# GitHubOfAndrew/TeAMOFlow

Measured on AMD Instinct MI355X. Metric: train_interactions_per_sec, higher is better.
Workload: dtype f32

## Files before the change

### include/tmf.h

```cpp
#ifndef TMF_H
#define TMF_H

#include <stddef.h>
#include <stdint.h>

#ifdef __cplusplus
extern "C" {
#endif

#define TMF_VERSION 203

#define TMF_OK 0
#define TMF_E_INVALID (-1)
#define TMF_E_LAUNCH (-2)
#define TMF_E_UNSUPPORTED (-3)

#define TMF_EPI_ADAM 0
#define TMF_EPI_GRAD 1

int tmf_version(void);
const char* tmf_last_error(void);

int tmf_padded_ld(int n_components);

int tmf_padded_ld_bf16(int n_components);

typedef struct tmf_adam {
    float alpha, one_minus_b1, one_minus_b2, eps;
} tmf_adam;
tmf_adam tmf_adam_fresh(float lr);

typedef struct tmf_segments {
    const int64_t* rowptr;
    const int32_t* seg_row;
    const int32_t* seg_chunk;
    const int32_t* seg_slab;
    int64_t nseg;
    int32_t chunk;
    int32_t row_mod;
} tmf_segments;

size_t tmf_csr_build_workspace_bytes(int64_t nnz);
int tmf_csr_build(const int64_t* indices, const float* values, int64_t nnz, int32_t n_users, int32_t n_items,
                  int64_t* rowptr_u, int32_t* col_u, float* val_u, int32_t* user_of, void* workspace,
                  size_t workspace_bytes, void* stream);
size_t tmf_stable_order_workspace_bytes(int64_t n);
int tmf_csc_perm(const int32_t* col_u, int64_t nnz, int32_t n_items, int64_t* rowptr_i, int64_t* perm,
                 void* workspace, size_t workspace_bytes, void* stream);
int tmf_stable_order_i32(const int32_t* keys, int64_t n, int64_t n_rows, int64_t* perm, int32_t* sorted_keys,
                         int64_t* rowptr, void* workspace, size_t workspace_bytes, void* stream);

size_t tmf_sort_samples_workspace_bytes(int32_t n_users, int32_t n_samples);
int tmf_sort_samples(const int32_t* R, int32_t n_users, int32_t n_samples, int32_t n_items, int32_t* R_sorted,
                     void* workspace, size_t workspace_bytes, void* stream);
int tmf_slice_offsets(const int32_t* ids, const int64_t* rowptr, int64_t stride, int32_t n_rows, int32_t n_items,
                      int32_t n_slices, int32_t* off, void* stream);
size_t tmf_wmrb_entry_lists_workspace_bytes(int64_t nnz, int32_t n_users, int32_t n_samples);
int tmf_wmrb_entry_lists(const int32_t* user_of, const int32_t* col_u, const float* val_u, int64_t nnz,
                         const int32_t* R_sorted, int32_t n_users, int32_t n_samples, int32_t n_items, int32_t user_chunks,
                         int32_t* ent_row, int32_t* ent_id, int64_t* rowptr_e, void* workspace, size_t workspace_bytes,
                         void* stream);

int tmf_mse_pass_f32(const tmf_segments* seg, const int32_t* other, const float* val,
                     const float* X_old, const float* Y_old, float* X_out, float* slab,
                     float* loss_part, int n_components, int epi, tmf_adam adam, void* stream);

int tmf_wsum_pass_f32(const tmf_segments* seg, const int32_t* ent_row, const int32_t* ent_w,
                      const float* wbuf, const float* T, const float* X_old, float* X_out,
                      float* slab, int n_components, int epi, tmf_adam adam, void* stream);

int tmf_wsum_rows4_rows_per_group(int n_components, int bf16);
size_t tmf_wsum_rows4_workspace_bytes(int32_t n_rows, int32_t n_blocks, int32_t rows_per_launch);
int tmf_wsum_rows4_f32(const int64_t* rowptr, int32_t n_rows, int32_t n_blocks, const int32_t* ent_row, const int32_t* ent_w,
                       const float* wbuf, const float* T, const float* X_old, float* X_out, int n_components, int epi,
                       tmf_adam adam, int32_t rows_per_launch, void* workspace, size_t workspace_bytes, void* stream);

size_t tmf_wsum_rows5_workspace_bytes(int32_t n_vrows, int32_t n_blocks, int32_t rows_per_launch);
int tmf_wsum_rows5_f32(const int64_t* rowptr, int32_t n_rows, int32_t n_blocks, const int32_t* ent_row, const int32_t* ent_w,
                       const float* wbuf, const float* T, const float* X_old, float* X_out, float* slab, const int32_t* vr_item,
                       const int32_t* vr_part, const int32_t* vr_nparts, const int32_t* vr_slot, int32_t n_vrows, int n_components,
                       int epi, tmf_adam adam, int32_t rows_per_launch, void* workspace, size_t workspace_bytes, void* stream);

int tmf_combine_rows_f32(const int32_t* long_rows, const int64_t* slab_beg, int64_t n_long,
                         const float* slab, const float* X_old, float* X_out, int n_components,
                         int epi, tmf_adam adam, void* stream);

int tmf_wmrb_user_pass_f32(const int64_t* rowptr, const int32_t* col, const float* val,
                           const int32_t* R, int32_t n_users, int32_t S, float c,
                           const float* U_old, const float* V_old, float* U_out, float* delta,
                           float* D, float* loss_part, float* pos_part,
                           int n_components, int epi, tmf_adam adam, void* stream);
int tmf_wmrb_user_pass_fits(int32_t n_samples, int n_components);

typedef struct tmf_slice_lists {
    const int32_t* R_sorted;
    const int32_t* slice_off;
    const int64_t* rowptr;
    const int32_t* col;
    const int32_t* pos_off;
    int32_t n_users, n_samples, n_slices;
    int32_t slice_begin, slice_count, item_base;
    int32_t flags;
    int32_t n_items;
} tmf_slice_lists;
#define TMF_SLICE_XCD_MAJOR 1
#define TMF_SLICE_N_ITEMS_STATED 2
int tmf_wmrb_scores3_f32(const tmf_slice_lists* lists, const void* U, const void* V, float* sp, float* p,
                         int n_components, void* stream);
int tmf_wmrb_scores3_bf16(const tmf_slice_lists* lists, const void* U, const void* V, float* sp, float* p,
                          int n_components, void* stream);
int tmf_wmrb_scores5_users_per_workgroup(void);
int tmf_wmrb_scores5_supported(int n_components, int bf16, int64_t n_items);
size_t tmf_wmrb_scores5_workspace_bytes(int64_t n_wg, int32_t n_windows, int wgs_per_launch);
int tmf_wmrb_scores5_f32(const int32_t* ids, const int32_t* outs, const int64_t* wg_ptr, int64_t n_wg, int64_t n_users,
                         int64_t n_items, const void* U, const void* V, float* sp, float* p, int n_components,
                         int wgs_per_launch, const int32_t* wstart, int32_t n_windows, int lag, void* workspace,
                         size_t workspace_bytes, void* stream);
int tmf_wmrb_scores5_bf16(const int32_t* ids, const int32_t* outs, const int64_t* wg_ptr, int64_t n_wg, int64_t n_users,
                          int64_t n_items, const void* U, const void* V, float* sp, float* p, int n_components,
                          int wgs_per_launch, const int32_t* wstart, int32_t n_windows, int lag, void* workspace,
                          size_t workspace_bytes, void* stream);
int tmf_wmrb_scores6_users_per_group(void);
int tmf_wmrb_scores6_supported(int n_components, int bf16, int64_t n_items);
int tmf_wmrb_scores6_f32(const int32_t* ids, const int32_t* outs, const int64_t* chunk_ptr, int64_t n_groups, int32_t n_slices,
                         int64_t n_users, int64_t n_items, const void* U, const void* V, float* sp, float* p, int n_components,
                         void* stream);
int tmf_wmrb_scores6_bf16(const int32_t* ids, const int32_t* outs, const int64_t* chunk_ptr, int64_t n_groups, int32_t n_slices,
                          int64_t n_users, int64_t n_items, const void* U, const void* V, float* sp, float* p, int n_components,
                          void* stream);
int tmf_wmrb_hinge2(const int64_t* rowptr, const float* val, const float* p, const float* sp, int32_t n_users,
                    int32_t n_samples, float c, float* delta, float* D, float* loss_part, void* stream);
int tmf_wmrb_hinge2_ordered(const int64_t* rowptr, const float* val, const float* p, const float* sp, int32_t n_users,
                            int32_t n_samples, float c, float* delta, float* D, float* loss_part, const int32_t* user_order,
                            void* stream);
int tmf_wmrb_gradu3_f32(const tmf_slice_lists* lists, const float* D, const float* delta, const void* V, float* part,
                        int per_slice_launches, int n_components, void* stream);
int tmf_wmrb_gradu3_bf16(const tmf_slice_lists* lists, const float* D, const float* delta, const void* V, float* part,
                         int per_slice_launches, int n_components, void* stream);
int tmf_wmrb_gradu4_supported(int n_components, int bf16);
size_t tmf_wmrb_gradu4_workspace_bytes(int32_t n_users, int32_t n_slices, int32_t users_per_launch);
int tmf_wmrb_gradu4_f32(const tmf_slice_lists* lists, const float* D, const float* delta, const void* V, const void* U_old,
                        void* U_out, int n_components, int epi, tmf_adam adam, int32_t users_per_launch, void* workspace,
                        size_t workspace_bytes, void* stream);
int tmf_wmrb_gradu4_bf16(const tmf_slice_lists* lists, const float* D, const float* delta, const void* V, const void* U_old,
                         void* U_out, int n_components, int epi, tmf_adam adam, int32_t users_per_launch, void* workspace,
                         size_t workspace_bytes, void* stream);
int tmf_wmrb_finish_f32(const float* part, int32_t n_slices, int32_t n_users, const void* U_old, void* U_out,
                        int n_components, int epi, tmf_adam adam, void* stream);
int tmf_wmrb_finish_bf16(const float* part, int32_t n_slices, int32_t n_users, const void* U_old, void* U_out,
                         int n_components, int epi, tmf_adam adam, void* stream);

int tmf_adam_fresh_rows_f32(float* W, const float* G, int64_t n_rows, int n_components,
                            tmf_adam adam, void* stream);

tmf_adam tmf_adam_step(float lr, int step);
int tmf_adam_state_rows_f32(float* W, const float* G, float* M, float* V, int64_t n_rows, int n_components,
                            tmf_adam adam, void* stream);

int tmf_sum_f32(const float* x, int64_t n, double* out, void* stream);

int tmf_gather_rows_cols_f32(const float* X, const int64_t* idx, float* out, int64_t rows,
                             int64_t cols, int64_t k, void* stream);

int tmf_predict_gemm_f32(const float* A, const float* B, float* C, int64_t m, int64_t n, int r,
                         int64_t lda, int64_t ldb, int64_t ldc, void* stream);

size_t tmf_topk_workspace_bytes(int64_t rows, int64_t cols, int k);
int tmf_topk_stable_f32(const float* X, int64_t rows, int64_t cols, int64_t ldx, int k,
                        int clamp_negatives, int32_t* out_idx, float* out_val, void* workspace,
                        size_t workspace_bytes, void* stream);

int tmf_mse_pass_bf16(const tmf_segments* seg, const int32_t* other, const float* val,
                      const void* X_old, const void* Y_old, void* X_out, float* slab,
                      float* loss_part, int n_components, int epi, tmf_adam adam, void* stream);
int tmf_wsum_pass_bf16(const tmf_segments* seg, const int32_t* ent_row, const int32_t* ent_w,
                       const float* wbuf, const void* T, const void* X_old, void* X_out,
                       float* slab, int n_components, int epi, tmf_adam adam, void* stream);
int tmf_wsum_rows4_bf16(const int64_t* rowptr, int32_t n_rows, int32_t n_blocks, const int32_t* ent_row, const int32_t* ent_w,
                        const float* wbuf, const void* T, const void* X_old, void* X_out, int n_components, int epi,
                        tmf_adam adam, int32_t rows_per_launch, void* workspace, size_t workspace_bytes, void* stream);
int tmf_wsum_rows5_bf16(const int64_t* rowptr, int32_t n_rows, int32_t n_blocks, const int32_t* ent_row, const int32_t* ent_w,
                        const float* wbuf, const void* T, const void* X_old, void* X_out, float* slab, const int32_t* vr_item,
                        const int32_t* vr_part, const int32_t* vr_nparts, const int32_t* vr_slot, int32_t n_vrows, int n_components,
                        int epi, tmf_adam adam, int32_t rows_per_launch, void* workspace, size_t workspace_bytes, void* stream);
int tmf_combine_rows_bf16(const int32_t* long_rows, const int64_t* slab_beg, int64_t n_long,
                          const float* slab, const void* X_old, void* X_out, int n_components,
                          int epi, tmf_adam adam, void* stream);
int tmf_wmrb_user_pass_bf16(const int64_t* rowptr, const int32_t* col, const float* val,
                            const int32_t* R, int32_t n_users, int32_t S, float c,
                            const void* U_old, const void* V_old, void* U_out, float* delta,
                            float* D, float* loss_part, float* pos_part,
                            int n_components, int epi, tmf_adam adam, void* stream);
int tmf_adam_fresh_rows_bf16(void* W, const float* G, int64_t n_rows, int n_components,
                             tmf_adam adam, void* stream);

int tmf_predict_topk_f32(const float* A, const float* B, int64_t m, int64_t n, int r, int64_t lda,
                         int64_t ldb, int k, int clamp_negatives, int32_t* out_idx, float* out_val,
                         void* stream);

int tmf_predict_topk_bf16(const void* A, const void* B, int64_t m, int64_t n, int r, int64_t lda,
                          int64_t ldb, int k, int clamp_negatives, int32_t* out_idx, float* out_val,
                          void* stream);

int tmf_predict_topk_split_supported(int r, int k);
size_t tmf_predict_topk_split_workspace_bytes(int64_t n, int r);
int tmf_predict_topk_split_f32(const float* A, const float* B, int64_t m, int64_t n, int r, int64_t lda,
                               int64_t ldb, int k, int clamp_negatives, int32_t* out_idx, float* out_val,
                               void* workspace, size_t workspace_bytes, void* stream);
int tmf_predict_topk_half2_supported(int r, int k);
size_t tmf_predict_topk_half2_workspace_bytes(int64_t n, int r);
int tmf_predict_topk_half2_f32(const float* A, const float* B, int64_t m, int64_t n, int r, int64_t lda,
                               int64_t ldb, int k, int clamp_negatives, int32_t* out_idx, float* out_val,
                               void* workspace, size_t workspace_bytes, void* stream);

typedef struct tmf_exclusion {
    const int64_t* rowptr;
    const int32_t* cols;
    int64_t item_base;
} tmf_exclusion;

int tmf_predict_topk_exclude_f32(const float* A, const float* B, int64_t m, int64_t n, int r, int64_t lda,
                                 int64_t ldb, int k, int clamp_negatives, const tmf_exclusion* exclude,
                                 int32_t* out_idx, float* out_val, void* stream);
int tmf_predict_topk_exclude_bf16(const void* A, const void* B, int64_t m, int64_t n, int r, int64_t lda,
                                  int64_t ldb, int k, int clamp_negatives, const tmf_exclusion* exclude,
                                  int32_t* out_idx, float* out_val, void* stream);
int tmf_predict_topk_split_exclude_f32(const float* A, const float* B, int64_t m, int64_t n, int r, int64_t lda,
                                       int64_t ldb, int k, int clamp_negatives, const tmf_exclusion* exclude,
                                       int32_t* out_idx, float* out_val, void* workspace, size_t workspace_bytes, void* stream);
int tmf_predict_topk_half2_exclude_f32(const float* A, const float* B, int64_t m, int64_t n, int r, int64_t lda,
                                       int64_t ldb, int k, int clamp_negatives, const tmf_exclusion* exclude,
                                       int32_t* out_idx, float* out_val, void* workspace, size_t workspace_bytes, void* stream);
int tmf_topk_stable_exclude_f32(float* X, int64_t rows, int64_t cols, int64_t ldx, int k, int clamp_negatives,
                                const tmf_exclusion* exclude, int32_t* out_idx, float* out_val, void* workspace,
                                size_t workspace_bytes, void* stream);

#define TMF_RANK_ROW_PAIRS 16
typedef struct tmf_rank_rows {
    const int32_t* user;
    const int64_t* begin;
    const int32_t* count;
    int64_t n_rows;
} tmf_rank_rows;

int tmf_pair_scores_f32(const float* A, const float* B, int r, int64_t lda, int64_t ldb, const int32_t* pair_user,
                        const int32_t* pair_item, int64_t n_pairs, float* out, void* stream);
int tmf_pair_scores_split(const float* A, const float* B, int r, int64_t lda, int64_t ldb, const int32_t* pair_user,
                          const int32_t* pair_item, int64_t n_pairs, float* out, void* stream);

int tmf_item_ranks_f32_supported(int r);
int tmf_item_ranks_split_supported(int r);
size_t tmf_item_ranks_split_workspace_bytes(int64_t n, int r);
int tmf_item_ranks_f32(const float* A, const float* B, int64_t n, int r, int64_t lda, int64_t ldb, const tmf_rank_rows* rows,
                       const int32_t* pos_item, const float* pos_score, const tmf_exclusion* exclude, int32_t* out_rank,
                       void* stream);
int tmf_item_ranks_split(const float* A, const float* B, int64_t n, int r, int64_t lda, int64_t ldb, const tmf_rank_rows* rows,
                         const int32_t* pos_item, const float* pos_score, const tmf_exclusion* exclude, int32_t* out_rank,
                         void* workspace, size_t workspace_bytes, void* stream);

int tmf_rank_count_rows_f32(float* X, int64_t rows, int64_t cols, int64_t ldx, int64_t user_base, const tmf_rank_rows* vrows,
                            const int32_t* pos_item, const tmf_exclusion* exclude, int32_t* out_rank, void* stream);

int tmf_dcg_idcg_f32(const int64_t* rowptr, const int32_t* cols, const float* gain, int64_t m, int64_t n_items, const int32_t* top,
                     int64_t ldt, int k, const float* den, const int64_t* n_zero, float* dcg, float* idcg, void* stream);

#ifdef __cplusplus
}
#endif
#endif
```

### teamoflow_amd/_engine.py

```python
import ctypes
import os

import torch

from . import _lib

DEFAULT_CHUNK = 1024
PART_BUDGET = int(os.environ.get('TMF_PART_BUDGET', 8 << 30))


def _excl_cumsum(x):
    out = torch.zeros(x.numel() + 1, dtype=torch.int64, device=x.device)
    torch.cumsum(x, 0, out=out[1:])
    return out


def take_interactions(indices, values, keep, user_offset=0, item_offset=0):
    u = indices[:, 0][keep] - user_offset
    j = indices[:, 1][keep] - item_offset
    return torch.stack([u, j], dim=1), values[keep]


def stable_order(keys, n_rows):
    n = keys.numel()
    if keys.is_cuda and n < 2 ** 31 and n_rows < 2 ** 31:
        lib = _lib.get()
        k32 = keys.to(torch.int32).contiguous()
        perm = torch.empty(n, dtype=torch.int64, device=keys.device)
        rowptr = torch.empty(n_rows + 1, dtype=torch.int64, device=keys.device)
        ws = torch.empty(lib.tmf_stable_order_workspace_bytes(n), dtype=torch.uint8, device=keys.device)
        _lib.check(lib.tmf_stable_order_i32(_lib.ptr(k32), n, n_rows, _lib.ptr(perm), None, _lib.ptr(rowptr), _lib.ptr(ws),
                                            ws.numel(), _lib.stream_ptr()), lib)
        return perm, rowptr
    perm = torch.sort(keys, stable=True)[1]
    return perm, _excl_cumsum(torch.bincount(keys.to(torch.int64), minlength=n_rows))


class SegmentTable:

    def __init__(self, rowptr, chunk=DEFAULT_CHUNK, out_row=None, n_out=None, row_mod=0):
        dev = rowptr.device
        rows = rowptr.numel() - 1
        lens = rowptr[1:] - rowptr[:-1]
        nch = torch.clamp((lens + (chunk - 1)) // chunk, min=1)
        nseg = int(nch.sum())
        seg_first = _excl_cumsum(nch)
        ar = torch.arange(rows, device=dev)
        seg_row = torch.repeat_interleave(ar, nch, output_size=nseg)
        seg_chunk = torch.arange(nseg, device=dev) - seg_first[seg_row]
        if out_row is None:
            multi = nch > 1
            slab_beg = _excl_cumsum(nch * multi)
            seg_slab = torch.where(multi[seg_row], slab_beg[seg_row] + seg_chunk, torch.full_like(seg_chunk, -1))
            long_rows = torch.nonzero(multi).flatten()
            self.n_slab = int(slab_beg[-1])
            self.long_slab_beg = torch.cat([slab_beg[long_rows], slab_beg[-1:]]).contiguous()
        else:
            seg_out = out_row[seg_row]
            order = torch.sort(seg_out, stable=True)[1]
            seg_slab = torch.empty(nseg, dtype=torch.int64, device=dev)
            seg_slab[order] = torch.arange(nseg, device=dev)
            long_rows = torch.arange(n_out, device=dev)
            self.n_slab = nseg
            self.long_slab_beg = _excl_cumsum(torch.bincount(seg_out, minlength=n_out))
        self.rows, self.chunk, self.nseg, self.row_mod = rows, int(chunk), nseg, int(row_mod)
        self.rowptr = rowptr.contiguous()
        self.seg_row = seg_row.to(torch.int32)
        self.seg_chunk = seg_chunk.to(torch.int32)
        self.seg_slab = seg_slab.to(torch.int32)
        self.long_rows = long_rows.to(torch.int32)
        self.n_long = int(long_rows.numel())
        self._c = None

    @classmethod
    def of_rows(cls, rowptr, rows, out_row, n_out, chunk=DEFAULT_CHUNK):
        self = cls.__new__(cls)
        dev = rowptr.device
        lens = rowptr[rows + 1] - rowptr[rows]
        nch = torch.clamp((lens + (chunk - 1)) // chunk, min=1)
        nseg = int(nch.sum())
        seg_first = _excl_cumsum(nch)
        sel = torch.repeat_interleave(torch.arange(rows.numel(), device=dev), nch, output_size=nseg)
        seg_chunk = torch.arange(nseg, device=dev) - seg_first[sel]
        seg_out = out_row[sel]
        order = torch.sort(seg_out, stable=True)[1]
        seg_slab = torch.empty(nseg, dtype=torch.int64, device=dev)
        seg_slab[order] = torch.arange(nseg, device=dev)
        self.n_slab = nseg
        self.long_slab_beg = _excl_cumsum(torch.bincount(seg_out, minlength=n_out))
        self.rows, self.chunk, self.nseg, self.row_mod = int(rows.numel()), int(chunk), nseg, 0
        self.rowptr = rowptr
        self.seg_row = rows[sel].to(torch.int32)
        self.seg_chunk = seg_chunk.to(torch.int32)
        self.seg_slab = seg_slab.to(torch.int32)
        self.long_rows = torch.arange(n_out, device=dev, dtype=torch.int32)
        self.n_long = int(n_out)
        self._c = None
        return self

    def cstruct(self):
        if self._c is None:
            self._c = _lib.Segments(self.rowptr.data_ptr(), self.seg_row.data_ptr(), self.seg_chunk.data_ptr(),
                                    self.seg_slab.data_ptr(), self.nseg, self.chunk, self.row_mod)
        return ctypes.byref(self._c)


class InteractionPlan:

    def __init__(self, indices, values, n_users, n_items, chunk=DEFAULT_CHUNK, user_chunks=1, csc=True):
        dev = indices.device
        u = indices[:, 0].contiguous()
        j = indices[:, 1].contiguous()
        nnz = u.numel()
        if nnz:
            lo_u, hi_u, lo_j, hi_j = int(u.min()), int(u.max()), int(j.min()), int(j.max())
            if lo_u < 0 or hi_u >= n_users or lo_j < 0 or hi_j >= n_items:
                raise IndexError(f'interaction indices outside dense_shape: users [{lo_u}, {hi_u}] of {n_users}, '
                                 f'items [{lo_j}, {hi_j}] of {n_items}')
        values = values.to(torch.float32).contiguous()
        self.nnz, self.n_users, self.n_items = nnz, n_users, n_items
        if indices.is_cuda and nnz < 2 ** 31:
            lib = _lib.get()
            idx64 = indices.to(torch.int64).contiguous()
            self.rowptr_u = torch.empty(n_users + 1, dtype=torch.int64, device=dev)
            self.col_u = torch.empty(nnz, dtype=torch.int32, device=dev)
            self.val_u = torch.empty(nnz, dtype=torch.float32, device=dev)
            self.user_of = torch.empty(nnz, dtype=torch.int32, device=dev)
            ws = torch.empty(lib.tmf_csr_build_workspace_bytes(nnz), dtype=torch.uint8, device=dev)
            _lib.check(lib.tmf_csr_build(_lib.ptr(idx64), _lib.ptr(values), nnz, n_users, n_items, _lib.ptr(self.rowptr_u),
                                         _lib.ptr(self.col_u), _lib.ptr(self.val_u), _lib.ptr(self.user_of), _lib.ptr(ws),
                                         ws.numel(), _lib.stream_ptr()), lib)
            del ws, idx64
        else:
            key = u.to(torch.int64) * n_items + j.to(torch.int64)
            if nnz > 1 and not bool((key[1:] >= key[:-1]).all()):
                perm = torch.sort(key, stable=True)[1]
                u, j, values = u[perm], j[perm], values[perm]
            self.rowptr_u = _excl_cumsum(torch.bincount(u, minlength=n_users))
            self.col_u = j.to(torch.int32)
            self.val_u = values.contiguous()
            self.user_of = u.to(torch.int32)
        self.seg_u = SegmentTable(self.rowptr_u, chunk)
        C = max(1, int(user_chunks))
        self.user_chunks = C
        self.seg_i = self.rowptr_i = self.row_i = self.val_i = None
        if csc:
            if C > 1:
                upc = -(-n_users // C)
                key = (self.user_of.to(torch.int64) // upc) * n_items + self.col_u.to(torch.int64)
            else:
                key = self.col_u
            perm_c, self.rowptr_i = stable_order(key, C * n_items)
            self.row_i = self.user_of[perm_c].contiguous()
            self.val_i = self.val_u[perm_c].contiguous()
            if C > 1:
                out_row = torch.arange(C * n_items, device=dev) % n_items
                self.seg_i = SegmentTable(self.rowptr_i, chunk, out_row=out_row, n_out=n_items, row_mod=n_items)
            else:
                self.seg_i = SegmentTable(self.rowptr_i, chunk)
        self.n_pos = int((self.val_u > 0).sum())

    @property
    def user_ids(self):
        return self.user_of.to(torch.int64)


def _slab_budget():
    env = os.environ.get('TMF_SLAB_BUDGET')
    if env:
        return int(env)
    total = torch.cuda.get_device_properties(torch.cuda.current_device()).total_memory if torch.cuda.is_available() else 32 << 30
    return int(min(64 << 30, total // 4))




def default_user_chunks(n_users, ld, target_bytes=3 << 20, n_items=None):
    env = os.environ.get('TMF_USER_CHUNKS')
    if env:
        return max(1, int(env))
    c = -(-n_users * ld * 4 // target_bytes)
    if n_items:
        c = min(c, max(1, _slab_budget() // (n_items * ld * 4)))
    return int(min(max(c, 1), 256)) if c > 1 else 1


def mse_user_chunks():
    env = os.environ.get('TMF_USER_CHUNKS')
    return max(1, int(env)) if env else 1


def default_item_slices(n_items, ld, n_samples=None, target_bytes=4 << 20, elem_size=4):
    env = os.environ.get('TMF_ITEM_SLICES')
    if env:
        return max(1, int(env))
    if n_items * ld * elem_size <= 2 * target_bytes:
        return 1
    return int(min(-(-n_items * ld * elem_size // target_bytes), 64))


def slices_xcd_major(n_slices):
    env = os.environ.get('TMF_SLICE_XCD')
    if env in ('0', '1'):
        return env == '1'
    return XCD_MAJOR_DEFAULT and n_slices >= 8


XCD_MAJOR_DEFAULT = False
SLICED_MIN_HINGE_TERMS = 1 << 16
SLICED_MIN_SCORES = 1 << 21


def choose_wmrb_user_pass(n_users, n_items, ld, n_samples, n_positives, n_components, elem_size=4):
    ns = default_item_slices(n_items, ld, elem_size=elem_size)
    if ns > 1 or not fused_user_pass_fits(n_samples, n_components) or os.environ.get('TMF_FORCE_SLICED') == '1':
        return ns, True
    if os.environ.get('TMF_ITEM_SLICES') or os.environ.get('TMF_FORCE_FUSED') == '1':
        return ns, False
    if (n_positives / max(n_users, 1)) * n_samples >= SLICED_MIN_HINGE_TERMS and n_users * n_samples >= SLICED_MIN_SCORES:
        groups = -(-n_users // 16)
        return int(max(min(max(round(1400 / groups), 1), 8), -(-n_items * ld * elem_size // (4 << 20)))), True
    return 1, False


def rows4_wanted(n_components, dtype=torch.float32, plan=None, R=None, n_users=None, n_items=None):
    env = os.environ.get('TMF_ROWS4')
    if env == '0':
        return False
    if not _lib.load_library().tmf_wsum_rows4_rows_per_group(int(n_components), int(dtype is torch.bfloat16)):
        return False
    if env == '1':
        return True
    if plan is not None:
        n_users = plan.n_users if n_users is None else n_users
        n_items = plan.n_items if n_items is None else n_items
    if not n_users or not n_items:
        return False
    ld = _lib.padded_ld(n_components, dtype)
    row_bytes = ld * (2 if dtype is torch.bfloat16 else 4)
    blocks_wanted = -(-int(n_users) * row_bytes // ROWS5_BLOCK_BYTES)
    blocks_slab_allows = max(1, _slab_budget() // (int(n_items) * ld * 4))
    return blocks_wanted > 2 * blocks_slab_allows


ROWS5_TARGET_OVER_MEDIAN = 1.15
ROWS5_BLOCK_BYTES = 4 << 20


def rows5_user_chunks(n_users, n_components, dtype=torch.float32):
    env = os.environ.get('TMF_USER_CHUNKS')
    if env:
        return max(1, int(env))
    row_bytes = _lib.padded_ld(n_components, dtype) * (2 if dtype is torch.bfloat16 else 4)
    return int(min(max(1, -(-int(n_users) * row_bytes // ROWS5_BLOCK_BYTES)), 256))


class VirtualRows:

    def __init__(self, rowptr_e, n_blocks, n_rows, target=None):
        dev = rowptr_e.device
        lens = (rowptr_e[1:] - rowptr_e[:-1]).view(n_blocks, n_rows).sum(0)
        mean = float(lens.to(torch.float64).mean()) if n_rows else 0.0
        median = float(lens.to(torch.float64).median()) if n_rows else 0.0
        env = os.environ.get('TMF_ROWS5_TARGET')
        self.target = int(env) if env else (int(target) if target else max(1, int(max(ROWS5_TARGET_OVER_MEDIAN * median, mean)) + 1))
        parts = torch.clamp((lens + (self.target - 1)) // self.target, min=1)
        first = _excl_cumsum(parts)
        nv = int(first[-1])
        item = torch.repeat_interleave(torch.arange(n_rows, device=dev), parts, output_size=nv)
        part = torch.arange(nv, device=dev) - first[item]
        multi = parts > 1
        slab_beg = _excl_cumsum(parts * multi)
        slot = torch.where(multi[item], slab_beg[item] + part, torch.full_like(part, -1))
        i32 = torch.int32
        self.n_vrows, self.n_slab = nv, int(slab_beg[-1])
        self.item = torch.cat([item, torch.tensor([n_rows], device=dev)]).to(i32).contiguous()
        self.part = torch.cat([part, torch.zeros(1, dtype=part.dtype, device=dev)]).to(i32).contiguous()
        self.nparts = torch.cat([parts[item], torch.ones(1, dtype=parts.dtype, device=dev)]).to(i32).contiguous()
        self.slot = slot.to(i32).contiguous()
        long_rows = torch.nonzero(multi).flatten()
        self.long_rows = long_rows.to(i32).contiguous()
        self.long_slab_beg = torch.cat([slab_beg[long_rows], slab_beg[-1:]]).contiguous()
        self.n_long = int(long_rows.numel())
        self.max_parts = int(parts.max()) if n_rows else 0


def fused_user_pass_fits(n_samples, n_components):
    return bool(_lib.load_library().tmf_wmrb_user_pass_fits(int(n_samples), min(int(n_components), 1024)))


HINGE_CHUNK = 255


def hinge_user_order(rowptr_u):
    if os.environ.get('TMF_HINGE_ORDER', '1') == '0':
        return None
    deg = rowptr_u[1:] - rowptr_u[:-1]
    passes = (deg + (HINGE_CHUNK - 1)) // HINGE_CHUNK
    if passes.numel() == 0 or int(passes.max()) <= 1:
        return None
    return torch.argsort(passes, descending=True, stable=True).to(torch.int32)


class WmrbPlan:

    def __init__(self, plan, R, chunk=DEFAULT_CHUNK, user_chunks=1, item_slices=1, n_components=128, sliced=None, item_lists=True,
                 xcd_major=None, rows4=False):
        dev = R.device
        m, S = R.shape
        nnz, n = plan.nnz, plan.n_items
        self.S, self.n_slices = S, max(1, int(item_slices))
        self.xcd_major = slices_xcd_major(self.n_slices) if xcd_major is None else bool(xcd_major)
        self.sliced = bool(sliced) if sliced is not None else (self.n_slices > 1 or not fused_user_pass_fits(S, n_components))
        C = self.user_chunks = max(1, int(user_chunks))
        E = nnz + m * S
        if E >= 2 ** 31:
            raise ValueError(f'interactions + n_users * n_samples = {E} >= 2^31 on one GPU: split the users over more GPUs')
        self.R_model = R
        native = R.is_cuda
        lib = _lib.get() if native else None
        i32 = ctypes.c_int32
        self.slice_off = self.pos_off = None
        if self.sliced:
            ns = self.n_slices
            if native:
                Rs = torch.empty_like(R)
                ws = torch.empty(lib.tmf_sort_samples_workspace_bytes(m, S), dtype=torch.uint8, device=dev)
                _lib.check(lib.tmf_sort_samples(_lib.ptr(R), i32(m), i32(S), i32(n), _lib.ptr(Rs), _lib.ptr(ws), ws.numel(),
                                                _lib.stream_ptr()), lib)
                del ws
                self.slice_off = torch.empty(m, ns + 1, dtype=torch.int32, device=dev)
                self.pos_off = torch.empty(m, ns + 1, dtype=torch.int32, device=dev)
                _lib.check(lib.tmf_slice_offsets(_lib.ptr(Rs), None, S, i32(m), i32(n), i32(ns), _lib.ptr(self.slice_off),
                                                 _lib.stream_ptr()), lib)
                _lib.check(lib.tmf_slice_offsets(_lib.ptr(plan.col_u), _lib.ptr(plan.rowptr_u), 0, i32(m), i32(n), i32(ns),
                                                 _lib.ptr(self.pos_off), _lib.stream_ptr()), lib)
            else:
                Rs = torch.sort(R.to(torch.int64), dim=1, stable=True)[0].to(torch.int32).contiguous()
                width = -(-n // ns)
                bnd = torch.arange(ns + 1, dtype=torch.int64) * width
                self.slice_off = torch.searchsorted(Rs.to(torch.int64), bnd[None, :].expand(m, -1).contiguous()).to(torch.int32)
                self.slice_off[:, -1] = S
                key = plan.user_of.to(torch.int64) * (ns * width + 1) + plan.col_u.to(torch.int64)
                q = torch.arange(m, dtype=torch.int64)[:, None] * (ns * width + 1) + bnd[None, :]
                self.pos_off = (torch.searchsorted(key, q.reshape(-1)).reshape(m, ns + 1) - plan.rowptr_u[:-1, None]).to(torch.int32)
                self.pos_off[:, -1] = (plan.rowptr_u[1:] - plan.rowptr_u[:-1]).to(torch.int32)
            R = Rs
        self.R = R.contiguous()
        self.ent_row = torch.empty(E, dtype=torch.int32, device=dev)
        rowptr = torch.empty(C * n + 2, dtype=torch.int64, device=dev)
        if native:
            ent_id = torch.empty(E, dtype=torch.int32, device=dev)
            ws = torch.empty(lib.tmf_wmrb_entry_lists_workspace_bytes(nnz, m, S), dtype=torch.uint8, device=dev)
            _lib.check(lib.tmf_wmrb_entry_lists(_lib.ptr(plan.user_of), _lib.ptr(plan.col_u), _lib.ptr(plan.val_u), nnz,
                                                _lib.ptr(self.R), i32(m), i32(S), i32(n), i32(C), _lib.ptr(self.ent_row),
                                                _lib.ptr(ent_id), _lib.ptr(rowptr), _lib.ptr(ws), ws.numel(),
                                                _lib.stream_ptr()), lib)
            del ws
        else:
            upc = max(1, -(-m // C))
            ku = plan.user_of.to(torch.int64)
            kp = torch.where(plan.val_u > 0, (ku // upc) * n + plan.col_u.to(torch.int64), torch.full_like(ku, C * n))
            ks = (torch.arange(m, dtype=torch.int64) // upc).repeat_interleave(S) * n + self.R.reshape(-1).to(torch.int64)
            keys = torch.cat([kp, ks])
            ent_id = torch.sort(keys, stable=True)[1]
            rowptr = _excl_cumsum(torch.bincount(keys, minlength=C * n + 1))
            owner = torch.cat([ku, torch.arange(m, dtype=torch.int64).repeat_interleave(S)])
            self.ent_row = owner[ent_id].to(torch.int32)
            ent_id = ent_id.to(torch.int32)
        self.rowptr_e = rowptr[:C * n + 1].contiguous()
        self.ent_w = ent_id
        self.rows4 = bool(rows4)
        self.vrows = VirtualRows(self.rowptr_e, C, n) if self.rows4 and os.environ.get('TMF_ROWS5', '1') != '0' else None
        if not item_lists or self.rows4:
            self.seg_e = None
        elif C > 1:
            out_row = torch.arange(C * n, device=dev) % n
            self.seg_e = SegmentTable(self.rowptr_e, chunk, out_row=out_row, n_out=n)
        else:
            self.seg_e = SegmentTable(self.rowptr_e, chunk)
        self.wbuf = torch.zeros(E, dtype=torch.float32, device=dev)
        self.delta = self.wbuf[:nnz]
        self.hinge_order = hinge_user_order(plan.rowptr_u)
        self.D = self.wbuf[nnz:].view(m, S)
        self._lists = None
        self.s5 = None

    def lists(self, plan):
        if self._lists is None:
            m, S = self.R.shape
            self._lists = _lib.SliceLists(self.R.data_ptr(), self.slice_off.data_ptr(), plan.rowptr_u.data_ptr(),
                                          plan.col_u.data_ptr(), self.pos_off.data_ptr(), m, S, self.n_slices, 0, 0, 0,
                                          (_lib.SLICE_XCD_MAJOR if self.xcd_major else 0) | _lib.SLICE_N_ITEMS_STATED, int(plan.n_items))
        return ctypes.byref(self._lists)

    def window_lists(self, plan, slice_begin, slice_count, item_base):
        m, S = self.R.shape
        return _lib.SliceLists(self.R.data_ptr(), self.slice_off.data_ptr(), plan.rowptr_u.data_ptr(), plan.col_u.data_ptr(),
                               self.pos_off.data_ptr(), m, S, self.n_slices, slice_begin, slice_count, item_base,
                               _lib.SLICE_N_ITEMS_STATED, int(plan.n_items))

    def D_in_model_order(self):
        if not self.sliced:
            return self.D
        perm = torch.sort(self.R_model.to(torch.int64), dim=1, stable=True)[1]
        out = torch.empty_like(self.D)
        out.scatter_(1, perm, self.D)
        return out


def row_stationary_wanted(n_users, n_items, n_samples, nnz, n_components, dtype=torch.float32, sliced=True):
    env = os.environ.get('TMF_ROW_STATIONARY')
    if env == '0' or not sliced:
        return False
    if not _lib.load_library().tmf_wmrb_gradu4_supported(int(n_components), int(dtype is torch.bfloat16)):
        return False
    return env == '1' or short_visits(n_users, n_items, n_samples, nnz, n_components, dtype)


def wmrb_plan_for(plan, R, n_components, dtype=torch.float32, n_items=None):
    m = plan.n_users
    n = plan.n_items if n_items is None else n_items
    bf16 = dtype is torch.bfloat16
    ld_store = _lib.padded_ld(n_components, dtype)
    ns, sliced = choose_wmrb_user_pass(m, n, ld_store, int(R.shape[1]), plan.n_pos, n_components, elem_size=2 if bf16 else 4)
    rs = row_stationary_wanted(m, n, int(R.shape[1]), plan.nnz, n_components, dtype, sliced)
    if rs and not os.environ.get('TMF_ITEM_SLICES'):
        ns = int(max(1, -(-n * ld_store * (2 if bf16 else 4) // GRADU4_SLICE_BYTES)))
    rows4 = rows4_wanted(n_components, dtype, plan, R)
    C = rows5_user_chunks(m, n_components, dtype) if rows4 else default_user_chunks(m, _lib.padded_ld(n_components), n_items=plan.n_items)
    return WmrbPlan(plan, R, user_chunks=C, item_slices=ns, n_components=n_components, sliced=sliced, rows4=rows4)


def scores6_wanted(plan, wplan, n_components, dtype=torch.float32):
    env = os.environ.get('TMF_SCORES6')
    if env == '0' or wplan is None or not wplan.sliced or not plan.col_u.is_cuda or os.environ.get('TMF_SCORES5') == '1':
        return False
    m, S = wplan.R.shape
    if m * S >= 2 ** 31 or plan.nnz >= 2 ** 31:
        return False
    if not _lib.load_library().tmf_wmrb_scores6_supported(int(n_components), int(dtype is torch.bfloat16), int(plan.n_items)):
        return False
    if env == '1':
        return True
    return SCORES6_DEFAULT and short_visits(m, plan.n_items, S, plan.nnz, n_components, dtype)


def short_visits(n_users, n_items, n_samples, nnz, n_components, dtype=torch.float32):
    row_bytes = _lib.padded_ld(n_components, dtype) * (2 if dtype is torch.bfloat16 else 4)
    table = n_items * row_bytes
    if table < 8 * VISIT_SLICE_BYTES:
        return False
    return (n_samples + nnz / max(n_users, 1)) * VISIT_SLICE_BYTES / table <= SCORES6_MAX_VISIT


SCORES6_SLICE_BYTES = 6 << 20
VISIT_SLICE_BYTES = 4 << 20
GRADU4_SLICE_BYTES = 3200000
SCORES6_MAX_VISIT = 24
SCORES6_DEFAULT = True


class Scores6Plan:

    PAD = -2 ** 31

    def __init__(self, plan, wplan, n_components, dtype=torch.float32, slice_bytes=None):
        lib = _lib.load_library()
        dev = plan.col_u.device
        self.key = (int(n_components), dtype)
        UG = int(lib.tmf_wmrb_scores6_users_per_group())
        m, S = wplan.R.shape
        nnz, n = plan.nnz, plan.n_items
        E = nnz + m * S
        self.n_groups = ng = -(-m // UG)
        row_bytes = _lib.padded_ld(n_components, dtype) * (2 if dtype is torch.bfloat16 else 4)
        slice_bytes = int(os.environ.get('TMF_S6_SLICE_BYTES', slice_bytes or SCORES6_SLICE_BYTES))
        ns = int(min(max(1, -(-n * row_bytes // slice_bytes)), max(1, (2 ** 31 - 1) // max(ng, 1))))
        width = -(-n // ns)
        self.n_slices = ns = -(-n // width)
        i32 = torch.int32
        uo = plan.user_of
        rows = torch.arange(m, device=dev, dtype=i32)
        keys = torch.empty(E, dtype=i32, device=dev)
        keys[:nnz] = (plan.col_u // width) * ng + uo // UG
        keys[nnz:].view(m, S).copy_((wplan.R // width) * ng + (rows // UG)[:, None])
        perm, rowptr = stable_order(keys, ns * ng)
        del keys
        packed = torch.empty(E, dtype=i32, device=dev)
        packed[:nnz] = ((uo % UG) << 24) | plan.col_u
        packed[nnz:].view(m, S).copy_(((rows % UG) << 24)[:, None] | wplan.R)
        ids_sorted = packed[perm]
        del packed
        outs = torch.empty(E, dtype=i32, device=dev)
        outs[:nnz] = -1 - torch.arange(nnz, device=dev, dtype=i32)
        outs[nnz:] = torch.arange(m * S, device=dev, dtype=i32)
        outs_sorted = outs[perm]
        del outs, perm
        cnt = rowptr[1:] - rowptr[:-1]
        ptr8 = _excl_cumsum((cnt + 7) // 8 * 8)
        E8 = int(ptr8[-1])
        self.ids = torch.empty(E8 + 8, dtype=i32, device=dev)
        self.outs = torch.full((E8 + 8,), self.PAD, dtype=i32, device=dev)
        self.ids[E8:] = 0
        step = 1 << 27
        for q0 in range(0, E8, step):
            q = torch.arange(q0, min(q0 + step, E8), device=dev, dtype=torch.int64)
            ch = torch.searchsorted(ptr8, q, right=True) - 1
            r = q - ptr8[ch]
            c = cnt[ch]
            src = rowptr[ch] + torch.minimum(r, c - 1)
            self.ids[q0:q0 + q.numel()] = ids_sorted[src]
            self.outs[q0:q0 + q.numel()] = torch.where(r < c, outs_sorted[src], torch.full_like(src, self.PAD).to(i32))
            del q, ch, r, c, src
        self.chunk_ptr = ptr8
        self.n_entries, self.n_padded = E, E8


def scores5_wanted(plan, wplan, n_components, dtype=torch.float32):
    if os.environ.get('TMF_SCORES5') != '1' or wplan is None or not wplan.sliced or not plan.col_u.is_cuda:
        return False
    m, S = wplan.R.shape
    if m * S >= 2 ** 31 or plan.nnz >= 2 ** 31:
        return False
    return bool(_lib.load_library().tmf_wmrb_scores5_supported(int(n_components), int(dtype is torch.bfloat16), int(plan.n_items)))


class Scores5Plan:

    PAD = -2 ** 31

    def __init__(self, plan, wplan, n_components, dtype=torch.float32, slice_bytes=None):
        lib = _lib.get()
        dev = plan.col_u.device
        self.key = (int(n_components), dtype)
        UB = int(lib.tmf_wmrb_scores5_users_per_workgroup())
        m, S = wplan.R.shape
        nnz, n = plan.nnz, plan.n_items
        E = nnz + m * S
        self.n_wg = n_wg = -(-m // UB)
        row_bytes = _lib.padded_ld(n_components, dtype) * (2 if dtype is torch.bfloat16 else 4)
        slice_bytes = int(os.environ.get('TMF_S5_SLICE_BYTES', slice_bytes or (512 << 10)))
        ns = int(min(max(1, -(-n * row_bytes // slice_bytes)), 4096, max(1, (2 ** 31 - 1) // max(n_wg, 1))))
        width = -(-n // ns)
        self.n_slices = ns
        i32 = torch.int32
        uo = plan.user_of
        rows = torch.arange(m, device=dev, dtype=i32)
        keys = torch.empty(E, dtype=i32, device=dev)
        keys[:nnz] = (uo // UB) * ns + plan.col_u // width
        keys[nnz:].view(m, S).copy_(((rows // UB) * ns)[:, None] + wplan.R // width)
        perm, rowptr = stable_order(keys, n_wg * ns)
        del keys
        packed = torch.empty(E, dtype=i32, device=dev)
        packed[:nnz] = ((uo % UB) << 24) | plan.col_u
        packed[nnz:].view(m, S).copy_(((rows % UB) << 24)[:, None] | wplan.R)
        ids_sorted = packed[perm]
        del packed
        outs = torch.empty(E, dtype=i32, device=dev)
        outs[:nnz] = -1 - torch.arange(nnz, device=dev, dtype=i32)
        outs[nnz:] = torch.arange(m * S, device=dev, dtype=i32)
        outs_sorted = outs[perm]
        del outs, perm
        wg_ptr = rowptr[::ns].contiguous()
        cnt = wg_ptr[1:] - wg_ptr[:-1]
        wg_ptr8 = _excl_cumsum((cnt + 7) // 8 * 8)
        E8 = int(wg_ptr8[-1])
        self.ids = torch.empty(E8 + 8, dtype=i32, device=dev)
        self.outs = torch.full((E8 + 8,), self.PAD, dtype=i32, device=dev)
        self.ids[E8:] = 0
        step = 1 << 27
        for q0 in range(0, E8, step):
            q = torch.arange(q0, min(q0 + step, E8), device=dev, dtype=torch.int64)
            wg = torch.searchsorted(wg_ptr8, q, right=True) - 1
            r = q - wg_ptr8[wg]
            c = cnt[wg]
            src = wg_ptr[wg] + torch.minimum(r, c - 1)
            self.ids[q0:q0 + q.numel()] = ids_sorted[src]
            self.outs[q0:q0 + q.numel()] = torch.where(r < c, outs_sorted[src], torch.full_like(src, self.PAD).to(i32))
            del q, wg, r, c, src
        self.wg_ptr = wg_ptr8
        self.n_entries, self.n_padded = E, E8
        every = max(1, int(os.environ.get('TMF_S5_PACE_EVERY', 32)), -(-ns // 4000))
        firsts = list(range(0, ns, every))
        off = rowptr[:n_wg * ns].view(n_wg, ns)[:, firsts] - wg_ptr[:-1, None]
        self.n_windows = nwin = len(firsts) + 1
        self.wstart = torch.zeros(n_wg, nwin + 1, dtype=i32, device=dev)
        self.wstart[:, 1:nwin] = ((off + 7) // 8).to(i32)
        self.wstart[:, nwin] = ((wg_ptr8[1:] - wg_ptr8[:-1]) // 8).to(i32)
        self.lag = int(os.environ.get('TMF_S5_LAG', 0))
        self.wgs_per_launch = int(os.environ.get('TMF_S5_WGS', 0))
        self.paced = os.environ.get('TMF_S5_PACE', '1') != '0' and ns > 1
        nb = lib.tmf_wmrb_scores5_workspace_bytes(n_wg, nwin, self.wgs_per_launch) if self.paced else 0
        self.sync = torch.zeros(max(nb // 4, 1), dtype=i32, device=dev)


class TrainState:

    def __init__(self, U0, V0, plan, n_components, wplan=None, dtype=torch.float32, V_tables=None, scratch=None):
        dev = plan.col_u.device
        self.r = int(n_components)
        if dtype not in (torch.float32, torch.bfloat16):
            raise ValueError('factor tables are stored as float32 or bfloat16')
        self.dtype = dtype
        self.sfx = '_bf16' if dtype is torch.bfloat16 else '_f32'
        self.ld = _lib.padded_ld(self.r, dtype)
        self.U = self._pad(U0, dev)
        self.U_nxt = torch.empty_like(self.U)
        if V_tables is None:
            self.V = self._pad(V0, dev)
            self.V_nxt = torch.empty_like(self.V)
        else:
            self.V, self.V_nxt = V_tables
        self.plan, self.wplan = plan, wplan
        need = dict(slab=max(plan.seg_u.n_slab, plan.seg_i.n_slab if plan.seg_i else 0,
                             wplan.seg_e.n_slab if wplan is not None and wplan.seg_e is not None else 0,
                             wplan.vrows.n_slab if wplan is not None and getattr(wplan, 'vrows', None) is not None else 0, 1) * self.ld,
                    loss_part=max(plan.seg_u.nseg, plan.n_users, 1))
        self.row_stationary = False
        if wplan is not None and wplan.sliced:
            m, S = wplan.R.shape
            self.row_stationary = row_stationary_wanted(m, plan.n_items, S, plan.nnz, self.r, dtype)
            self.users_per_launch = int(os.environ.get('TMF_G4_USERS', 32768))
            if self.row_stationary:
                nb = _lib.load_library().tmf_wmrb_gradu4_workspace_bytes(m, wplan.n_slices, self.users_per_launch)
                self.g4_sync = torch.zeros(max(nb // 4, 1), dtype=torch.int32, device=dev)
            ns = wplan.n_slices
            if ns * m * self.ld * 4 <= PART_BUDGET:
                self.part_layers, self.gradu_launches = ns, 0
            elif wplan.xcd_major:
                self.part_layers, self.gradu_launches = min(8, ns), 3
            else:
                self.part_layers, self.gradu_launches = 1, 1
            need.update(sp=m * S, pk=max(plan.nnz, 1), part=self.part_layers * max(m, 1) * self.ld)
            wplan.s6 = getattr(wplan, 's6', None)
            if scores6_wanted(plan, wplan, self.r, dtype):
                if wplan.s6 is None or wplan.s6.key != (self.r, dtype):
                    wplan.s6 = Scores6Plan(plan, wplan, self.r, dtype)
            else:
                wplan.s6 = None
            if wplan.seg_e is not None and scores5_wanted(plan, wplan, self.r, dtype):
                if getattr(wplan, 's5', None) is None or wplan.s5.key != (self.r, dtype):
                    wplan.s5 = Scores5Plan(plan, wplan, self.r, dtype)
            else:
                wplan.s5 = None
        if wplan is not None and wplan.rows4:
            L = _lib.load_library()
            per_group = L.tmf_wsum_rows4_rows_per_group(self.r, int(dtype is torch.bfloat16))
            if not per_group:
                raise ValueError('the row-stationary item pass needs rows of at least 16 lanes')
            cus = torch.cuda.get_device_properties(dev).multi_processor_count if torch.cuda.is_available() else 256
            self.rows4_per_launch = int(os.environ.get('TMF_ROWS4_PER_LAUNCH', 2 * cus * per_group))
            n_work = wplan.vrows.n_vrows if wplan.vrows is not None else plan.n_items
            nb = L.tmf_wsum_rows4_workspace_bytes(n_work, wplan.user_chunks, self.rows4_per_launch)
            self.rows4_sync = torch.zeros(max(nb // 4, 1), dtype=torch.int32, device=dev)
        self._need = need
        if scratch is None:
            self._bind({k: torch.zeros(v, dtype=torch.float32, device=dev) if k == 'loss_part'
                        else torch.empty(v, dtype=torch.float32, device=dev) for k, v in need.items()})
        else:
            scratch.setdefault('states', []).append(self)

    def _bind(self, bufs):
        need = self._need
        self.slab = bufs['slab'][:need['slab']].view(-1, self.ld)
        self.loss_part = bufs['loss_part'][:need['loss_part']]
        if 'sp' in need:
            m, S = self.wplan.R.shape
            self.sp = bufs['sp'][:need['sp']].view(m, S)
            self.pk = bufs['pk'][:need['pk']]
            self.part = bufs['part'][:need['part']].view(-1, self.ld)

    def _pad(self, W, dev):
        W = torch.as_tensor(W).detach().to(device=dev, dtype=torch.float32)
        out = torch.zeros(W.shape[0], self.ld, dtype=self.dtype, device=dev)
        out[:, :self.r] = W
        return out

    def swap(self):
        self.U, self.U_nxt = self.U_nxt, self.U
        self.V, self.V_nxt = self.V_nxt, self.V


def share_scratch(scratch, dev):
    states = scratch.get('states', [])
    sizes = {}
    for st in states:
        for k, v in st._need.items():
            sizes[k] = max(sizes.get(k, 0), v)
    bufs = {k: torch.zeros(v, dtype=torch.float32, device=dev) for k, v in sizes.items()}
    for st in states:
        st._bind(bufs)
    return bufs


class KernelTimer:

    def __init__(self):
        self.spans = {}

    def start(self, name):
        ev = torch.cuda.Event(enable_timing=True)
        ev.record()
        self.spans.setdefault(name, []).append([ev, None])

    def stop(self, name):
        ev = torch.cuda.Event(enable_timing=True)
        ev.record()
        self.spans[name][-1][1] = ev

    def mean_ms(self, name):
        v = [a.elapsed_time(b) for a, b in self.spans.get(name, []) if b is not None]
        return sum(v) / len(v) if v else float('nan')


def _row_pass_finish(lib, seg, slab, X_old, X_out, r, epi, adam, stream, sfx='_f32'):
    if seg.n_long:
        _lib.check(getattr(lib, 'tmf_combine_rows' + sfx)(_lib.ptr(seg.long_rows), _lib.ptr(seg.long_slab_beg), seg.n_long,
                                            _lib.ptr(slab), _lib.ptr(X_old), _lib.ptr(X_out), r, epi, adam, stream), lib)


def epoch_mse(st, adam, loss_out, item_epi=_lib.EPI_ADAM, item_out=None, prof=None, user_epi=_lib.EPI_ADAM, user_out=None):
    lib, p, r = _lib.get(), st.plan, st.r
    s = _lib.stream_ptr()
    U_out = st.U_nxt if user_out is None else user_out
    if prof:
        prof.start('mse_user_pass')
    mse_pass = getattr(lib, 'tmf_mse_pass' + st.sfx)
    _lib.check(mse_pass(p.seg_u.cstruct(), _lib.ptr(p.col_u), _lib.ptr(p.val_u), _lib.ptr(st.U),
                                    _lib.ptr(st.V), _lib.ptr(U_out), _lib.ptr(st.slab), _lib.ptr(st.loss_part),
                                    r, user_epi, adam, s), lib)
    if prof:
        prof.stop('mse_user_pass')
    _row_pass_finish(lib, p.seg_u, st.slab, st.U, U_out, r, user_epi, adam, s, st.sfx)
    _lib.check(lib.tmf_sum_f32(_lib.ptr(st.loss_part), p.seg_u.nseg, _lib.ptr(loss_out), s), lib)
    V_out = st.V_nxt if item_out is None else item_out
    if prof:
        prof.start('mse_item_pass')
    _lib.check(mse_pass(p.seg_i.cstruct(), _lib.ptr(p.row_i), _lib.ptr(p.val_i), _lib.ptr(st.V),
                                    _lib.ptr(st.U), _lib.ptr(V_out), _lib.ptr(st.slab), None, r, item_epi, adam, s), lib)
    if prof:
        prof.stop('mse_item_pass')
    _row_pass_finish(lib, p.seg_i, st.slab, st.V, V_out, r, item_epi, adam, s, st.sfx)


def _wmrb_user_pass_sliced(lib, st, adam, c, prof=None, user_epi=_lib.EPI_ADAM, U_out=None):
    p, w, r = st.plan, st.wplan, st.r
    i32 = ctypes.c_int32
    m, S, ns = p.n_users, w.S, w.n_slices
    s = _lib.stream_ptr()
    lists = w.lists(p)

    def timed(name, rc_fn):
        if prof:
            prof.start(name)
        _lib.check(rc_fn(), lib)
        if prof:
            prof.stop(name)
    s5, s6 = getattr(w, 's5', None), getattr(w, 's6', None)
    if s6 is not None:
        timed('wmrb_scores', lambda: getattr(lib, 'tmf_wmrb_scores6' + st.sfx)(
            _lib.ptr(s6.ids), _lib.ptr(s6.outs), _lib.ptr(s6.chunk_ptr), s6.n_groups, i32(s6.n_slices), m, p.n_items, _lib.ptr(st.U),
            _lib.ptr(st.V), _lib.ptr(st.sp), _lib.ptr(st.pk), r, s))
    elif s5 is not None:
        timed('wmrb_scores', lambda: getattr(lib, 'tmf_wmrb_scores5' + st.sfx)(
            _lib.ptr(s5.ids), _lib.ptr(s5.outs), _lib.ptr(s5.wg_ptr), s5.n_wg, m, p.n_items, _lib.ptr(st.U), _lib.ptr(st.V),
            _lib.ptr(st.sp), _lib.ptr(st.pk), r, s5.wgs_per_launch, _lib.ptr(s5.wstart) if s5.paced else None, i32(s5.n_windows),
            s5.lag, _lib.ptr(s5.sync) if s5.paced else None, s5.sync.numel() * 4, s))
    else:
        timed('wmrb_scores', lambda: getattr(lib, 'tmf_wmrb_scores3' + st.sfx)(lists, _lib.ptr(st.U), _lib.ptr(st.V), _lib.ptr(st.sp),
                                                                                _lib.ptr(st.pk), r, s))
    timed('wmrb_hinge', lambda: lib.tmf_wmrb_hinge2_ordered(_lib.ptr(p.rowptr_u), _lib.ptr(p.val_u), _lib.ptr(st.pk), _lib.ptr(st.sp),
                                                            i32(m), i32(S), c, _lib.ptr(w.delta), _lib.ptr(w.D), _lib.ptr(st.loss_part),
                                                            _lib.ptr(w.hinge_order), s))
    if st.row_stationary:
        timed('wmrb_gradu', lambda: getattr(lib, 'tmf_wmrb_gradu4' + st.sfx)(
            lists, _lib.ptr(w.D), _lib.ptr(w.delta), _lib.ptr(st.V), _lib.ptr(st.U), _lib.ptr(st.U_nxt if U_out is None else U_out),
            r, user_epi, adam, i32(st.users_per_launch), _lib.ptr(st.g4_sync), st.g4_sync.numel() * 4, s))
        return
    timed('wmrb_gradu', lambda: getattr(lib, 'tmf_wmrb_gradu3' + st.sfx)(
        lists, _lib.ptr(w.D), _lib.ptr(w.delta), _lib.ptr(st.V), _lib.ptr(st.part),
        st.gradu_launches, r, s))
    timed('wmrb_finish', lambda: getattr(lib, 'tmf_wmrb_finish' + st.sfx)(_lib.ptr(st.part), i32(st.part_layers), i32(m),
                                                                          _lib.ptr(st.U), _lib.ptr(st.U_nxt if U_out is None else U_out),
                                                                          r, user_epi, adam, s))


def epoch_wmrb(st, adam, c, loss_out, item_epi=_lib.EPI_ADAM, item_out=None, prof=None, user_epi=_lib.EPI_ADAM, user_out=None):
    lib, p, w, r = _lib.get(), st.plan, st.wplan, st.r
    s = _lib.stream_ptr()
    if prof:
        prof.start('wmrb_user_pass')
    if w.sliced:
        _wmrb_user_pass_sliced(lib, st, adam, c, prof, user_epi, user_out)
    else:
        _lib.check(getattr(lib, 'tmf_wmrb_user_pass' + st.sfx)(_lib.ptr(p.rowptr_u), _lib.ptr(p.col_u), _lib.ptr(p.val_u), _lib.ptr(w.R),
                                              p.n_users, w.S, c, _lib.ptr(st.U), _lib.ptr(st.V),
                                              _lib.ptr(st.U_nxt if user_out is None else user_out),
                                              _lib.ptr(w.delta), _lib.ptr(w.D), _lib.ptr(st.loss_part), None,
                                              r, user_epi, adam, s), lib)
    if prof:
        prof.stop('wmrb_user_pass')
    _lib.check(lib.tmf_sum_f32(_lib.ptr(st.loss_part), p.n_users, _lib.ptr(loss_out), s), lib)
    V_out = st.V_nxt if item_out is None else item_out
    if w.rows4:
        if prof:
            prof.start('wmrb_item_pass')
        i32 = ctypes.c_int32
        if w.vrows is not None:
            v = w.vrows
            _lib.check(getattr(lib, 'tmf_wsum_rows5' + st.sfx)(_lib.ptr(w.rowptr_e), i32(p.n_items), i32(w.user_chunks), _lib.ptr(w.ent_row),
                                                               _lib.ptr(w.ent_w), _lib.ptr(w.wbuf), _lib.ptr(st.U), _lib.ptr(st.V), _lib.ptr(V_out),
                                                               _lib.ptr(st.slab), _lib.ptr(v.item), _lib.ptr(v.part), _lib.ptr(v.nparts),
                                                               _lib.ptr(v.slot), i32(v.n_vrows), r, item_epi, adam, i32(st.rows4_per_launch),
                                                               _lib.ptr(st.rows4_sync), st.rows4_sync.numel() * 4, s), lib)
        else:
            _lib.check(getattr(lib, 'tmf_wsum_rows4' + st.sfx)(_lib.ptr(w.rowptr_e), i32(p.n_items), i32(w.user_chunks),
                                                               _lib.ptr(w.ent_row), _lib.ptr(w.ent_w), _lib.ptr(w.wbuf), _lib.ptr(st.U),
                                                               _lib.ptr(st.V), _lib.ptr(V_out), r, item_epi, adam,
                                                               i32(st.rows4_per_launch), _lib.ptr(st.rows4_sync),
                                                               st.rows4_sync.numel() * 4, s), lib)
        if prof:
            prof.stop('wmrb_item_pass')
        if w.vrows is not None and w.vrows.n_long:
            if prof:
                prof.start('wmrb_combine')
            v = w.vrows
            _lib.check(getattr(lib, 'tmf_combine_rows' + st.sfx)(_lib.ptr(v.long_rows), _lib.ptr(v.long_slab_beg), v.n_long, _lib.ptr(st.slab),
                                                                 _lib.ptr(st.V), _lib.ptr(V_out), r, item_epi, adam, s), lib)
            if prof:
                prof.stop('wmrb_combine')
        return
    if prof:
        prof.start('wmrb_item_pass')
    _lib.check(getattr(lib, 'tmf_wsum_pass' + st.sfx)(w.seg_e.cstruct(), _lib.ptr(w.ent_row), _lib.ptr(w.ent_w), _lib.ptr(w.wbuf),
                                     _lib.ptr(st.U), _lib.ptr(st.V), _lib.ptr(V_out), _lib.ptr(st.slab), r, item_epi,
                                     adam, s), lib)
    if prof:
        prof.stop('wmrb_item_pass')
    if prof:
        prof.start('wmrb_combine')
    _row_pass_finish(lib, w.seg_e, st.slab, st.V, V_out, r, item_epi, adam, s, st.sfx)
    if prof:
        prof.stop('wmrb_combine')


def adam_constants(lr):
    return _lib.load_library().tmf_adam_fresh(float(lr))
```

### teamoflow_amd/_lib.py

```python
import ctypes
import os
import subprocess

import torch

_HERE = os.path.dirname(os.path.abspath(__file__))
LIB_PATH = os.environ.get('TMF_LIB', os.path.join(_HERE, 'libtmf.so'))
CSRC = os.path.join(_HERE, 'csrc')

EPI_ADAM, EPI_GRAD = 0, 1


class EngineUnavailable(RuntimeError):
    pass


class EngineError(RuntimeError):
    pass


class Adam(ctypes.Structure):
    _fields_ = [('alpha', ctypes.c_float), ('one_minus_b1', ctypes.c_float), ('one_minus_b2', ctypes.c_float),
                ('eps', ctypes.c_float)]


class SliceLists(ctypes.Structure):
    _fields_ = [('R_sorted', ctypes.c_void_p), ('slice_off', ctypes.c_void_p), ('rowptr', ctypes.c_void_p),
                ('col', ctypes.c_void_p), ('pos_off', ctypes.c_void_p), ('n_users', ctypes.c_int32),
                ('n_samples', ctypes.c_int32), ('n_slices', ctypes.c_int32), ('slice_begin', ctypes.c_int32),
                ('slice_count', ctypes.c_int32), ('item_base', ctypes.c_int32), ('flags', ctypes.c_int32),
                ('n_items', ctypes.c_int32)]


class Segments(ctypes.Structure):
    _fields_ = [('rowptr', ctypes.c_void_p), ('seg_row', ctypes.c_void_p), ('seg_chunk', ctypes.c_void_p),
                ('seg_slab', ctypes.c_void_p), ('nseg', ctypes.c_int64), ('chunk', ctypes.c_int32),
                ('row_mod', ctypes.c_int32)]


class Exclusion(ctypes.Structure):
    _fields_ = [('rowptr', ctypes.c_void_p), ('cols', ctypes.c_void_p), ('item_base', ctypes.c_int64)]


class RankRows(ctypes.Structure):
    _fields_ = [('user', ctypes.c_void_p), ('begin', ctypes.c_void_p), ('count', ctypes.c_void_p), ('n_rows', ctypes.c_int64)]


_P, _I, _L, _F = ctypes.c_void_p, ctypes.c_int, ctypes.c_int64, ctypes.c_float
_EX = ctypes.POINTER(Exclusion)
_RR = ctypes.POINTER(RankRows)
_SEG = ctypes.POINTER(Segments)
_SL = ctypes.POINTER(SliceLists)
_I32, _SZ = ctypes.c_int32, ctypes.c_size_t

SIGNATURES = {}
_BASE_SIGNATURES = {
    'tmf_version': (_I, []),
    'tmf_last_error': (ctypes.c_char_p, []),
    'tmf_padded_ld': (_I, [_I]),
    'tmf_padded_ld_bf16': (_I, [_I]),
    'tmf_adam_fresh': (Adam, [_F]),
    'tmf_csr_build_workspace_bytes': (_SZ, [_L]),
    'tmf_csr_build': (_I, [_P, _P, _L, _I32, _I32, _P, _P, _P, _P, _P, _SZ, _P]),
    'tmf_stable_order_workspace_bytes': (_SZ, [_L]),
    'tmf_csc_perm': (_I, [_P, _L, _I32, _P, _P, _P, _SZ, _P]),
    'tmf_stable_order_i32': (_I, [_P, _L, _L, _P, _P, _P, _P, _SZ, _P]),
    'tmf_sort_samples_workspace_bytes': (_SZ, [_I32, _I32]),
    'tmf_sort_samples': (_I, [_P, _I32, _I32, _I32, _P, _P, _SZ, _P]),
    'tmf_slice_offsets': (_I, [_P, _P, _L, _I32, _I32, _I32, _P, _P]),
    'tmf_wmrb_entry_lists_workspace_bytes': (_SZ, [_L, _I32, _I32]),
    'tmf_wmrb_entry_lists': (_I, [_P, _P, _P, _L, _P, _I32, _I32, _I32, _I32, _P, _P, _P, _P, _SZ, _P]),
    'tmf_mse_pass_f32': (_I, [_SEG, _P, _P, _P, _P, _P, _P, _P, _I, _I, Adam, _P]),
    'tmf_wsum_pass_f32': (_I, [_SEG, _P, _P, _P, _P, _P, _P, _P, _I, _I, Adam, _P]),
    'tmf_wsum_rows4_rows_per_group': (_I, [_I, _I]),
    'tmf_wsum_rows4_workspace_bytes': (_SZ, [_I32, _I32, _I32]),
    'tmf_wsum_rows4_f32': (_I, [_P, _I32, _I32, _P, _P, _P, _P, _P, _P, _I, _I, Adam, _I32, _P, _SZ, _P]),
    'tmf_wsum_rows5_workspace_bytes': (_SZ, [_I32, _I32, _I32]),
    'tmf_wsum_rows5_f32': (_I, [_P, _I32, _I32, _P, _P, _P, _P, _P, _P, _P, _P, _P, _P, _P, _I32, _I, _I, Adam, _I32, _P, _SZ, _P]),
    'tmf_combine_rows_f32': (_I, [_P, _P, _L, _P, _P, _P, _I, _I, Adam, _P]),
    'tmf_wmrb_user_pass_f32': (_I, [_P, _P, _P, _P, _I32, _I32, _F, _P, _P, _P, _P, _P, _P, _P, _I, _I, Adam, _P]),
    'tmf_wmrb_user_pass_fits': (_I, [_I32, _I]),
    'tmf_wmrb_scores3_f32': (_I, [_SL, _P, _P, _P, _P, _I, _P]),
    'tmf_wmrb_scores6_users_per_group': (_I, []),
    'tmf_wmrb_scores6_supported': (_I, [_I, _I, _L]),
    'tmf_wmrb_scores6_f32': (_I, [_P, _P, _P, _L, _I32, _L, _L, _P, _P, _P, _P, _I, _P]),
    'tmf_wmrb_scores5_users_per_workgroup': (_I, []),
    'tmf_wmrb_scores5_supported': (_I, [_I, _I, _L]),
    'tmf_wmrb_scores5_workspace_bytes': (_SZ, [_L, _I32, _I]),
    'tmf_wmrb_scores5_f32': (_I, [_P, _P, _P, _L, _L, _L, _P, _P, _P, _P, _I, _I, _P, _I32, _I, _P, _SZ, _P]),
    'tmf_wmrb_hinge2': (_I, [_P, _P, _P, _P, _I32, _I32, _F, _P, _P, _P, _P]),
    'tmf_wmrb_hinge2_ordered': (_I, [_P, _P, _P, _P, _I32, _I32, _F, _P, _P, _P, _P, _P]),
    'tmf_wmrb_gradu3_f32': (_I, [_SL, _P, _P, _P, _P, _I, _I, _P]),
    'tmf_wmrb_gradu4_supported': (_I, [_I, _I]),
    'tmf_wmrb_gradu4_workspace_bytes': (_SZ, [_I32, _I32, _I32]),
    'tmf_wmrb_gradu4_f32': (_I, [_SL, _P, _P, _P, _P, _P, _I, _I, Adam, _I32, _P, _SZ, _P]),
    'tmf_wmrb_finish_f32': (_I, [_P, _I32, _I32, _P, _P, _I, _I, Adam, _P]),
    'tmf_adam_fresh_rows_f32': (_I, [_P, _P, _L, _I, Adam, _P]),
    'tmf_adam_step': (Adam, [_F, _I]),
    'tmf_adam_state_rows_f32': (_I, [_P, _P, _P, _P, _L, _I, Adam, _P]),
    'tmf_mse_pass_bf16': (_I, [_SEG, _P, _P, _P, _P, _P, _P, _P, _I, _I, Adam, _P]),
    'tmf_wsum_rows4_bf16': (_I, [_P, _I32, _I32, _P, _P, _P, _P, _P, _P, _I, _I, Adam, _I32, _P, _SZ, _P]),
    'tmf_wsum_rows5_bf16': (_I, [_P, _I32, _I32, _P, _P, _P, _P, _P, _P, _P, _P, _P, _P, _P, _I32, _I, _I, Adam, _I32, _P, _SZ, _P]),
    'tmf_wsum_pass_bf16': (_I, [_SEG, _P, _P, _P, _P, _P, _P, _P, _I, _I, Adam, _P]),
    'tmf_combine_rows_bf16': (_I, [_P, _P, _L, _P, _P, _P, _I, _I, Adam, _P]),
    'tmf_wmrb_user_pass_bf16': (_I, [_P, _P, _P, _P, _I32, _I32, _F, _P, _P, _P, _P, _P, _P, _P, _I, _I, Adam, _P]),
    'tmf_adam_fresh_rows_bf16': (_I, [_P, _P, _L, _I, Adam, _P]),
    'tmf_sum_f32': (_I, [_P, _L, _P, _P]),
    'tmf_gather_rows_cols_f32': (_I, [_P, _P, _P, _L, _L, _L, _P]),
    'tmf_predict_gemm_f32': (_I, [_P, _P, _P, _L, _L, _I, _L, _L, _L, _P]),
    'tmf_topk_workspace_bytes': (_SZ, [_L, _L, _I]),
    'tmf_topk_stable_f32': (_I, [_P, _L, _L, _L, _I, _I, _P, _P, _P, _SZ, _P]),
    'tmf_predict_topk_f32': (_I, [_P, _P, _L, _L, _I, _L, _L, _I, _I, _P, _P, _P]),
    'tmf_predict_topk_bf16': (_I, [_P, _P, _L, _L, _I, _L, _L, _I, _I, _P, _P, _P]),
    'tmf_predict_topk_split_supported': (_I, [_I, _I]),
    'tmf_predict_topk_split_workspace_bytes': (_SZ, [_L, _I]),
    'tmf_predict_topk_split_f32': (_I, [_P, _P, _L, _L, _I, _L, _L, _I, _I, _P, _P, _P, _SZ, _P]),
    'tmf_predict_topk_half2_supported': (_I, [_I, _I]),
    'tmf_predict_topk_half2_workspace_bytes': (_SZ, [_L, _I]),
    'tmf_predict_topk_half2_f32': (_I, [_P, _P, _L, _L, _I, _L, _L, _I, _I, _P, _P, _P, _SZ, _P]),
    'tmf_predict_topk_exclude_f32': (_I, [_P, _P, _L, _L, _I, _L, _L, _I, _I, _EX, _P, _P, _P]),
    'tmf_predict_topk_exclude_bf16': (_I, [_P, _P, _L, _L, _I, _L, _L, _I, _I, _EX, _P, _P, _P]),
    'tmf_predict_topk_split_exclude_f32': (_I, [_P, _P, _L, _L, _I, _L, _L, _I, _I, _EX, _P, _P, _P, _SZ, _P]),
    'tmf_predict_topk_half2_exclude_f32': (_I, [_P, _P, _L, _L, _I, _L, _L, _I, _I, _EX, _P, _P, _P, _SZ, _P]),
    'tmf_topk_stable_exclude_f32': (_I, [_P, _L, _L, _L, _I, _I, _EX, _P, _P, _P, _SZ, _P]),
    'tmf_pair_scores_f32': (_I, [_P, _P, _I, _L, _L, _P, _P, _L, _P, _P]),
    'tmf_pair_scores_split': (_I, [_P, _P, _I, _L, _L, _P, _P, _L, _P, _P]),
    'tmf_item_ranks_f32_supported': (_I, [_I]),
    'tmf_item_ranks_split_supported': (_I, [_I]),
    'tmf_item_ranks_split_workspace_bytes': (_SZ, [_L, _I]),
    'tmf_item_ranks_f32': (_I, [_P, _P, _L, _I, _L, _L, _RR, _P, _P, _EX, _P, _P]),
    'tmf_item_ranks_split': (_I, [_P, _P, _L, _I, _L, _L, _RR, _P, _P, _EX, _P, _P, _SZ, _P]),
    'tmf_rank_count_rows_f32': (_I, [_P, _L, _L, _L, _L, _RR, _P, _EX, _P, _P]),
    'tmf_dcg_idcg_f32': (_I, [_P, _P, _P, _L, _L, _P, _L, _I, _P, _P, _P, _P, _P]),
}

SIGNATURES.update(_BASE_SIGNATURES)
for _name in ('tmf_wmrb_scores3', 'tmf_wmrb_scores5', 'tmf_wmrb_scores6', 'tmf_wmrb_gradu3', 'tmf_wmrb_gradu4', 'tmf_wmrb_finish'):
    SIGNATURES[_name + '_bf16'] = SIGNATURES[_name + '_f32']

_lib = None
MIN_LIB_VERSION = 203
SLICE_XCD_MAJOR, SLICE_N_ITEMS_STATED = 1, 2


def build(force=False, verbose=False):
    if force:
        subprocess.run(['make', '-C', CSRC, 'clean'], check=True, capture_output=not verbose)
    subprocess.run(['make', '-C', CSRC, '-j4'], check=True, capture_output=not verbose)
    return LIB_PATH


def load_library():
    global _lib
    if _lib is not None:
        return _lib
    if not os.path.exists(LIB_PATH):
        raise EngineUnavailable(f'{LIB_PATH} not found - run `python -c "import __graft_entry__ as g; g.build()"` '
                                f'or `make -C {CSRC}`')
    lib = ctypes.CDLL(LIB_PATH)
    older = os.environ.get('TMF_LIB_OLDER') == '1'
    try:
        lib.tmf_version.restype, lib.tmf_version.argtypes = SIGNATURES['tmf_version']
        version = lib.tmf_version()
    except AttributeError:
        version = 0
    if version < MIN_LIB_VERSION and not older:
        raise EngineUnavailable(f'{LIB_PATH} is version {version}, this package needs {MIN_LIB_VERSION} or newer (struct layouts and '
                                f'entry points changed) - rebuild it: `make -C {CSRC}`')
    for name, (res, args) in SIGNATURES.items():
        try:
            fn = getattr(lib, name)
        except AttributeError:
            if older:
                continue
            raise EngineUnavailable(f'{LIB_PATH} (version {version}) lacks {name} - rebuild it: `make -C {CSRC}`') from None
        fn.restype, fn.argtypes = res, args
    _lib = lib
    return lib


def get():
    if not torch.cuda.is_available():
        raise EngineUnavailable('teamoflow_amd needs an MI355X: torch.cuda.is_available() is False and the '
                                'engine has no CPU fallback')
    return load_library()


def stream_ptr():
    return ctypes.c_void_p(torch.cuda.current_stream().cuda_stream)


def ptr(t):
    if t is None:
        return None
    return ctypes.c_void_p(t.data_ptr())


def check(rc, lib=None):
    if rc != 0:
        lib = lib or load_library()
        raise EngineError(f'libtmf error {rc}: {lib.tmf_last_error().decode()}')


def padded_ld(n_components, dtype=None):
    r = int(n_components)
    if r < 1 or r > 1024:
        raise ValueError(f'n_components={r} outside the supported range [1, 1024]')
    if dtype is torch.bfloat16:
        if r > 512:
            return 1024
        lanes, g = (r + 7) // 8, 1
        while g < lanes:
            g *= 2
        return 8 * g
    if r <= 256:
        lanes, g = (r + 3) // 4, 1
        while g < lanes:
            g *= 2
        return 4 * g
    nv = (r + 255) // 256
    if nv == 3:
        nv = 4
    return 256 * nv
```

### teamoflow_amd/csrc/tmf_hinge.hip

```cpp
#include <math.h>

#include "tmf_common.h"

namespace tmf {

constexpr int HK = 256;
constexpr int HCHUNK = HK - 1;
constexpr int HPAD = HK + HK / 32;
constexpr int HSPL = 8;
constexpr int HWAVES = 1;

struct HingeLds {
    unsigned long long keys[HK];
    float ts[HPAD];
    float pw[HPAD];
    unsigned int cnt[HK];
    unsigned char ord[HK];
};

__device__ __forceinline__ unsigned int orderable(float t) {
    const unsigned int u = __float_as_uint(t);
    return u ^ ((u >> 31) ? 0xffffffffu : 0x80000000u);
}

__device__ __forceinline__ int pad_slot(int i) { return i + (i >> 5); }

template <int STEP>
__device__ __forceinline__ void search_step(const float* __restrict__ ts, const float (&x)[HSPL], int (&pp)[HSPL]) {
    constexpr int SP = STEP + (STEP >> 5);
    constexpr int OFF = (STEP >= 32) ? SP - 2 : STEP - 1;
    float tv[HSPL];
#pragma unroll
    for (int j = 0; j < HSPL; ++j) tv[j] = ts[pp[j] + OFF];
#pragma unroll
    for (int j = 0; j < HSPL; ++j) pp[j] += (tv[j] <= x[j]) ? SP : 0;
}

__device__ __forceinline__ void search_tile(const float* __restrict__ ts, const float (&x)[HSPL], int (&rho)[HSPL], int nfin) {
    int pp[HSPL];
#pragma unroll
    for (int j = 0; j < HSPL; ++j) pp[j] = 0;
    if (nfin >= 128) search_step<128>(ts, x, pp);
    if (nfin >= 64) search_step<64>(ts, x, pp);
    if (nfin >= 32) search_step<32>(ts, x, pp);
    if (nfin >= 16) search_step<16>(ts, x, pp);
    search_step<8>(ts, x, pp);
    search_step<4>(ts, x, pp);
    search_step<2>(ts, x, pp);
    search_step<1>(ts, x, pp);
#pragma unroll
    for (int j = 0; j < HSPL; ++j) {
        const int r = pp[j] - pp[j] / 33;
        rho[j] = r < nfin ? r : nfin;
    }
}

__device__ __forceinline__ void load_tile(const float* __restrict__ spu, int s0, int S, int lane, float (&x)[HSPL]) {
#pragma unroll
    for (int j = 0; j < HSPL; ++j) {
        const int s = s0 + lane + 64 * j;
        x[j] = (s < S) ? spu[s] : __builtin_nanf("");
    }
}

__global__ __launch_bounds__(64 * HWAVES) void k_wmrb_hinge2(
    const int64_t* __restrict__ rowptr, const float* __restrict__ val, const float* __restrict__ p,
    const float* __restrict__ sp, int S, int fixbits, float c, int64_t n_users, float* __restrict__ delta,
    float* __restrict__ D, float* __restrict__ loss_part, const int32_t* __restrict__ order) {
    __shared__ HingeLds lds_all[HWAVES];
    const int lane = threadIdx.x & 63, wave = threadIdx.x >> 6;
    const int64_t slot = (int64_t)blockIdx.x * HWAVES + wave;
    if (slot >= n_users) return;
    const int64_t u = order ? (int64_t)order[slot] : slot;
    HingeLds& L = lds_all[wave];
    const int64_t rb = rowptr[u], re = rowptr[u + 1];
    const float* spu = sp + u * (int64_t)S;
    float* Du = D + u * (int64_t)S;
    const int ntiles = (S + 64 * HSPL - 1) / (64 * HSPL);

    float lsum = 0.f;
    bool wrote = false;
    for (int64_t cb = rb; cb < re; cb += HCHUNK) {
        const int len = (int)((re - cb < HCHUNK) ? (re - cb) : HCHUNK);
        float tq[4];
        unsigned long long kq[4];
        int nfin = 0;
#pragma unroll
        for (int q = 0; q < 4; ++q) {
            const int i = lane + 64 * q;
            float t = INFINITY;
            if (i < len) {
                const float a = val[cb + i];
                if (a > 0.f) t = -(1.0f - p[cb + i]);
            }
            tq[q] = t;
            kq[q] = ((unsigned long long)orderable(t) << 32) | (unsigned int)i;
            nfin += __popcll(__ballot(t < INFINITY));
            if (i < len) L.keys[i] = kq[q];
        }
        if (nfin == 0) {
            for (int i = lane; i < len; i += 64) delta[cb + i] = 0.f;
            continue;
        }
        wave_lds_sync();
        int rank[4] = {0, 0, 0, 0};
        if (len <= 64) {
            for (int j = 0; j < len; ++j) rank[0] += (L.keys[j] < kq[0]) ? 1 : 0;
        } else if (len <= 128) {
            for (int j = 0; j < len; ++j) {
                const unsigned long long kj = L.keys[j];
                rank[0] += (kj < kq[0]) ? 1 : 0;
                rank[1] += (kj < kq[1]) ? 1 : 0;
            }
        } else {
            for (int j = 0; j < len; ++j) {
                const unsigned long long kj = L.keys[j];
#pragma unroll
                for (int q = 0; q < 4; ++q) rank[q] += (kj < kq[q]) ? 1 : 0;
            }
        }
#pragma unroll
        for (int q = 0; q < 4; ++q) {
            const int i = lane + 64 * q;
            if (i < len) {
                L.ts[pad_slot(rank[q])] = tq[q];
                L.ord[rank[q]] = (unsigned char)i;
            } else if (i < HK) {
                L.ts[pad_slot(i)] = INFINITY;
            }
        }
        wave_lds_sync();
        float town[4];
        int oown[4];
#pragma unroll
        for (int q = 0; q < 4; ++q) {
            const int pos = 4 * lane + q;
            town[q] = L.ts[pad_slot(pos)];
            oown[q] = (pos < len) ? (int)L.ord[pos] : -1;
            L.cnt[pos] = 0u;
            L.keys[pos] = 0ull;
        }
        const float B = fmaxf(fabsf(L.ts[0]), fabsf(L.ts[pad_slot(nfin - 1)]));
        int eB = 0;
        (void)frexpf(B, &eB);
        if (!(B < INFINITY)) eB = 128;
        const double to_fix = ldexp(1.0, fixbits - eB), from_fix = ldexp(1.0, eB - fixbits);
        wave_lds_sync();
        int ctop = 0;
        double stop = 0.0;
        unsigned int rpk[4];
        for (int tp = 0; tp < ntiles; tp += 2) {
#pragma unroll
            for (int h = 0; h < 2; ++h) {
                const int tile = tp + h;
                if (tile >= ntiles) break;
                float x[HSPL];
                int rho[HSPL];
                load_tile(spu, tile * 64 * HSPL, S, lane, x);
                search_tile(L.ts, x, rho, nfin);
#pragma unroll
                for (int j = 0; j < HSPL; ++j) {
                    if (rho[j] == nfin) {
                        ctop += 1;
                        stop += (double)x[j];
                    } else if (rho[j] != 0 && fabsf(x[j]) <= B) {
                        atomicAdd(&L.cnt[rho[j]], 1u);
                        atomicAdd(&L.keys[rho[j]], (unsigned long long)__double2ll_rn((double)x[j] * to_fix));
                    }
                }
                if (tp == 0) {
                    rpk[2 * h] = (unsigned)rho[0] | ((unsigned)rho[1] << 8) | ((unsigned)rho[2] << 16) | ((unsigned)rho[3] << 24);
                    rpk[2 * h + 1] = (unsigned)rho[4] | ((unsigned)rho[5] << 8) | ((unsigned)rho[6] << 16) | ((unsigned)rho[7] << 24);
                }
            }
        }
#pragma unroll
        for (int off = 32; off >= 1; off >>= 1) {
            ctop += __shfl_xor(ctop, off, 64);
            stop += __shfl_xor(stop, off, 64);
        }
        wave_lds_sync();
        int csuf[4];
        long long fsuf[4];
        {
            int crun = 0;
            long long frun = 0;
#pragma unroll
            for (int q = 3; q >= 0; --q) {
                const int b = 4 * lane + q + 1;
                if (b < HK) {
                    crun += (int)L.cnt[b];
                    frun += (long long)L.keys[b];
                }
                csuf[q] = crun;
                fsuf[q] = frun;
            }
            int cinc = crun;
            long long finc = frun;
#pragma unroll
            for (int off = 1; off < 64; off <<= 1) {
                const int co = __shfl_down(cinc, off, 64);
                const long long fo = __shfl_down(finc, off, 64);
                if (lane + off < 64) {
                    cinc += co;
                    finc += fo;
                }
            }
            const int cex = cinc - crun;
            const long long fex = finc - frun;
#pragma unroll
            for (int q = 0; q < 4; ++q) {
                csuf[q] += cex;
                fsuf[q] += fex;
            }
        }
        float wown[4];
#pragma unroll
        for (int q = 0; q < 4; ++q) {
            const int pos = 4 * lane + q;
            float w = 0.f, d = 0.f;
            if (pos < nfin) {
                const int cn = csuf[q] + ctop;
                const float c1 = -town[q];
                double hs = (double)cn * (double)c1 + ((double)fsuf[q] * from_fix + stop);
                hs = hs > 0.0 ? hs : 0.0;
                const float M = c * (float)hs;
                lsum += logf(1.0f + M);
                w = c * __frcp_rn(1.0f + M);
                d = -(w * (float)cn);
            }
            wown[q] = w;
            if (oown[q] >= 0) delta[cb + oown[q]] = d;
        }
        {
            const float l0 = wown[0], l1 = l0 + wown[1], l2 = l1 + wown[2], l3 = l2 + wown[3];
            float inc = l3;
#pragma unroll
            for (int off = 1; off < 64; off <<= 1) {
                const float o = __shfl_up(inc, off, 64);
                if (lane >= off) inc += o;
            }
            const float ex = __shfl_up(inc, 1, 64);
            const float base = (lane == 0) ? 0.f : ex;
            L.pw[pad_slot(4 * lane)] = base;
            L.pw[pad_slot(4 * lane + 1)] = base + l0;
            L.pw[pad_slot(4 * lane + 2)] = base + l1;
            L.pw[pad_slot(4 * lane + 3)] = base + l2;
        }
        wave_lds_sync();
        for (int tp = 0; tp < ntiles; tp += 2) {
#pragma unroll
            for (int h = 0; h < 2; ++h) {
                const int tile = tp + h;
                if (tile >= ntiles) break;
                int rho[HSPL];
                if (ntiles <= 2) {
#pragma unroll
                    for (int j = 0; j < HSPL; ++j) rho[j] = (int)((rpk[2 * h + (j >> 2)] >> (8 * (j & 3))) & 0xffu);
                } else {
                    float x[HSPL];
                    load_tile(spu, tile * 64 * HSPL, S, lane, x);
                    search_tile(L.ts, x, rho, nfin);
                }
#pragma unroll
                for (int j = 0; j < HSPL; ++j) {
                    const int s = tile * 64 * HSPL + lane + 64 * j;
                    if (s < S) {
                        const float dv = L.pw[pad_slot(rho[j])];
                        if (wrote) Du[s] += dv;
                        else Du[s] = dv;
                    }
                }
            }
        }
        wrote = true;
        wave_lds_sync();
    }
    if (!wrote)
        for (int s = lane; s < S; s += 64) Du[s] = 0.f;
#pragma unroll
    for (int off = 32; off >= 1; off >>= 1) lsum += __shfl_xor(lsum, off, 64);
    if (lane == 0 && loss_part) loss_part[u] = lsum;
}

}

using namespace tmf;

extern "C" int tmf_wmrb_hinge2(const int64_t* rowptr, const float* val, const float* p, const float* sp, int32_t n_users,
                               int32_t S, float c, float* delta, float* D, float* loss_part, void* stream) {
    return tmf_wmrb_hinge2_ordered(rowptr, val, p, sp, n_users, S, c, delta, D, loss_part, nullptr, stream);
}

extern "C" int tmf_wmrb_hinge2_ordered(const int64_t* rowptr, const float* val, const float* p, const float* sp, int32_t n_users,
                                       int32_t S, float c, float* delta, float* D, float* loss_part, const int32_t* user_order,
                                       void* stream) {
    if (n_users == 0) return TMF_OK;
    TMF_REQUIRE(rowptr && sp && D && n_users > 0 && S > 0, "wmrb_hinge2: bad arguments");
    int lg = 0;
    while (((int64_t)1 << lg) < (int64_t)S) ++lg;
    const int fixbits = 62 - lg;
    const unsigned blocks = (unsigned)(((int64_t)n_users + HWAVES - 1) / HWAVES);
    hipLaunchKernelGGL(k_wmrb_hinge2, dim3(blocks), dim3(64 * HWAVES), 0, (hipStream_t)stream, rowptr, val, p, sp, (int)S, fixbits,
                       c, (int64_t)n_users, delta, D, loss_part, user_order);
    return check_launch("tmf_wmrb_hinge2");
}
```

### teamoflow_amd/csrc/tmf_wmrb.hip

```cpp
#include <math.h>
#include <stdlib.h>

#include <type_traits>

#include "tmf_common.h"

namespace tmf {

constexpr int kThreads = 256;
constexpr int kWaves = kThreads / 64;
constexpr int kPosChunk = 512;
constexpr int kUnrollW = 4;
#ifndef TMF_G4_UNROLL
#define TMF_G4_UNROLL 4
#endif
constexpr int kG4Unroll = TMF_G4_UNROLL;

__host__ __device__ inline int round4(int x) { return (x + 3) & ~3; }

__host__ __device__ inline int sp_padded(int S) {
    const int nf4 = (S + 3) / 4;
    const int per = ((nf4 + 2 * kWaves - 1) / (2 * kWaves) + 1) & ~1;
    return 4 * 2 * kWaves * per;
}

__device__ __forceinline__ void count_ge0_x4(int& c0, int& c1, float x0, float x1, float x2, float x3) {
    unsigned long long m0, m1, m2, m3;
    asm("v_cmp_le_f32_e64 %2, 0, %6\n\t"
        "v_cmp_le_f32_e64 %3, 0, %7\n\t"
        "v_cmp_le_f32_e64 %4, 0, %8\n\t"
        "v_cmp_le_f32_e64 %5, 0, %9\n\t"
        "v_addc_co_u32_e64 %0, %2, 0, %0, %2\n\t"
        "v_addc_co_u32_e64 %1, %3, 0, %1, %3\n\t"
        "v_addc_co_u32_e64 %0, %4, 0, %0, %4\n\t"
        "v_addc_co_u32_e64 %1, %5, 0, %1, %5"
        : "+v"(c0), "+v"(c1), "=&s"(m0), "=&s"(m1), "=&s"(m2), "=&s"(m3)
        : "v"(x0), "v"(x1), "v"(x2), "v"(x3));
}

__device__ __forceinline__ float4 select_ge_x4(float sps, const float4 c, const float4 w) {
    unsigned long long m0, m1, m2, m3;
    float4 r;
    asm("v_cmp_ge_f32_e64 %4, %8, -%9\n\t"
        "v_cmp_ge_f32_e64 %5, %8, -%10\n\t"
        "v_cmp_ge_f32_e64 %6, %8, -%11\n\t"
        "v_cmp_ge_f32_e64 %7, %8, -%12\n\t"
        "v_cndmask_b32_e64 %0, 0, %13, %4\n\t"
        "v_cndmask_b32_e64 %1, 0, %14, %5\n\t"
        "v_cndmask_b32_e64 %2, 0, %15, %6\n\t"
        "v_cndmask_b32_e64 %3, 0, %16, %7"
        : "=&v"(r.x), "=&v"(r.y), "=&v"(r.z), "=&v"(r.w), "=&s"(m0), "=&s"(m1), "=&s"(m2), "=&s"(m3)
        : "v"(sps), "v"(c.x), "v"(c.y), "v"(c.z), "v"(c.w), "v"(w.x), "v"(w.y), "v"(w.z), "v"(w.w));
    return r;
}

template <int G, int NV, typename T>
__device__ __forceinline__ void wmrb_user_body(
    const int64_t u, char* smem_raw,
    const int64_t* __restrict__ rowptr, const int32_t* __restrict__ col, const float* __restrict__ val,
    const int32_t* __restrict__ R, int S, float c,
    const T* __restrict__ U_old,
    const T* __restrict__ V_old, void* __restrict__ U_out, float* __restrict__ delta,
    float* __restrict__ Dg, float* __restrict__ loss_part, float* __restrict__ pos_part, int epi,
    tmf_adam adam) {
    constexpr int NG = 64 / G;
    constexpr int NGB = NG * kWaves;
    constexpr int LD = 4 * G * NV;
    const int S4 = round4(S), SP = sp_padded(S);
    float* sp = reinterpret_cast<float*>(smem_raw);
    float* Dl = sp + SP;
    float* c1 = Dl + S4;
    float* wl = c1 + kPosChunk;
    float* dl = wl + kPosChunk;
    int* ci = reinterpret_cast<int*>(dl + kPosChunk);
    int* Rl = ci + kPosChunk;
    float* pm = reinterpret_cast<float*>(Rl + S4);
    int* pc = reinterpret_cast<int*>(pm + kWaves * 64);
    float* red = reinterpret_cast<float*>(pc + kWaves * 64);

    const int tid = threadIdx.x, lane = tid & 63, wave = tid >> 6;
    const int g = lane & (G - 1), grp = lane / G, gid = wave * NG + grp;
    const int64_t rb = rowptr[u], re = rowptr[u + 1];
    const int32_t* Ru = R + u * (int64_t)S;

    int mine = 0;
    for (int64_t k = rb + tid; k < re; k += kThreads) mine |= (val[k] > 0.f);
    const int anypos = __syncthreads_or(mine);

    Frag<NV> acc;
    zero<NV>(acc);
    float lsum = 0.f, npos = 0.f;

    if (!anypos) {
        for (int64_t k = rb + tid; k < re; k += kThreads) delta[k] = 0.f;
        for (int s = tid; s < S; s += kThreads) Dg[u * (int64_t)S + s] = 0.f;
    } else {
        Frag<NV> x;
        load_row<G, NV>(x, U_old, u, g);
        for (int s = tid; s < S; s += kThreads) Rl[s] = Ru[s];
        __syncthreads();
        const int32_t* Ri = Rl;
        for (int s0 = gid; s0 < S; s0 += NGB * kUnrollW) {
            Raw<NV, T> raw[kUnrollW];
#pragma unroll
            for (int t = 0; t < kUnrollW; ++t) {
                const int s = s0 + t * NGB;
                load_raw<G, NV>(raw[t], V_old, Ri[s < S ? s : 0], g);
            }
#pragma unroll
            for (int t = 0; t < kUnrollW; ++t) {
                const int s = s0 + t * NGB;
                Frag<NV> y;
                to_frag<NV>(y, raw[t]);
                const float d = group_allsum<G>(dot_partial<NV>(x, y));
                if (g == 0 && s < S) sp[s] = d;
            }
        }
        for (int s = tid; s < SP; s += kThreads) {
            if (s < S) Dl[s] = 0.f;
            else sp[s] = -INFINITY;
        }
        __syncthreads();

        for (int64_t cb = rb; cb < re; cb += kPosChunk) {
            const int len = (int)((re - cb < kPosChunk) ? (re - cb) : kPosChunk);
            const int len4 = round4(len);
            for (int kk = tid; kk < len; kk += kThreads) ci[kk] = (val[cb + kk] > 0.f) ? col[cb + kk] : -1;
            __syncthreads();
            for (int k0 = gid; k0 < len; k0 += NGB * kUnrollW) {
                Raw<NV, T> raw[kUnrollW];
                bool pos[kUnrollW];
#pragma unroll
                for (int t = 0; t < kUnrollW; ++t) {
                    const int kk = k0 + t * NGB;
                    const int item = (kk < len) ? ci[kk] : -1;
                    pos[t] = item >= 0;
                    load_raw<G, NV>(raw[t], V_old, pos[t] ? item : 0, g);
                }
#pragma unroll
                for (int t = 0; t < kUnrollW; ++t) {
                    const int kk = k0 + t * NGB;
                    Frag<NV> y;
                    to_frag<NV>(y, raw[t]);
                    const float p = group_allsum<G>(dot_partial<NV>(x, y));
                    if (g == 0 && kk < len) c1[kk] = pos[t] ? (1.0f - p) : -INFINITY;
                }
            }
            for (int kk = len + tid; kk < len4; kk += kThreads) {
                c1[kk] = -INFINITY;
                wl[kk] = 0.f;
            }
            __syncthreads();
            {
                constexpr int kSG = 2 * kWaves;
                const int per_sg = SP / (4 * kSG);
                const int sg = wave * 2 + (lane >> 5), l32 = lane & 31;
                const float4* sp4 = reinterpret_cast<const float4*>(sp) + sg * per_sg;
                for (int kb = 0; kb < len; kb += 32) {
                    const int kk = kb + l32;
                    const float c1v = (kk < len) ? c1[kk] : -INFINITY;
                    float m0 = 0.f, m1 = 0.f, m2 = 0.f, m3 = 0.f;
                    int cnt = 0, cnt2 = 0;
#pragma unroll 2
                    for (int f = 0; f < per_sg; f += 2) {
                        const float4 q = sp4[f];
                        const float4 q2 = sp4[f + 1];
                        const float x0 = c1v + q.x, x1 = c1v + q.y, x2 = c1v + q.z, x3 = c1v + q.w;
                        const float x4 = c1v + q2.x, x5 = c1v + q2.y, x6 = c1v + q2.z, x7 = c1v + q2.w;
                        m0 += fmaxf(x0, 0.f);
                        m1 += fmaxf(x1, 0.f);
                        m2 += fmaxf(x2, 0.f);
                        m3 += fmaxf(x3, 0.f);
                        m0 += fmaxf(x4, 0.f);
                        m1 += fmaxf(x5, 0.f);
                        m2 += fmaxf(x6, 0.f);
                        m3 += fmaxf(x7, 0.f);
                        count_ge0_x4(cnt, cnt2, x0, x1, x2, x3);
                        count_ge0_x4(cnt, cnt2, x4, x5, x6, x7);
                    }
                    cnt += cnt2;
                    pm[sg * 32 + l32] = (m0 + m1) + (m2 + m3);
                    pc[sg * 32 + l32] = cnt;
                    __syncthreads();
                    if (tid < 32 && kk < len) {
                        float w = 0.f, d = 0.f;
                        if (c1v != -INFINITY) {
                            float Ms = 0.f;
                            int cn = 0;
#pragma unroll
                            for (int h = 0; h < kSG; ++h) {
                                Ms += pm[h * 32 + tid];
                                cn += pc[h * 32 + tid];
                            }
                            const float M = c * Ms;
                            lsum += logf(1.0f + M);
                            npos += 1.f;
                            w = c * __frcp_rn(1.0f + M);
                            d = -(w * (float)cn);
                        }
                        wl[kk] = w;
                        dl[kk] = d;
                        delta[cb + kk] = d;
                    }
                    __syncthreads();
                }
            }
            for (int s = tid; s < S; s += kThreads) {
                const float sps = sp[s];
                float d0 = 0.f, d1 = 0.f;
                const float4* c4 = reinterpret_cast<const float4*>(c1);
                const float4* w4 = reinterpret_cast<const float4*>(wl);
#pragma unroll 4
                for (int q = 0; q < len4 / 4; ++q) {
                    const float4 r = select_ge_x4(sps, c4[q], w4[q]);
                    d0 += r.x;
                    d1 += r.y;
                    d0 += r.z;
                    d1 += r.w;
                }
                Dl[s] += d0 + d1;
            }
            for (int k0 = gid; k0 < len; k0 += NGB * kUnrollW) {
                Raw<NV, T> raw[kUnrollW];
                float d[kUnrollW];
#pragma unroll
                for (int t = 0; t < kUnrollW; ++t) {
                    const int kk = k0 + t * NGB;
                    d[t] = (kk < len) ? dl[kk] : 0.f;
                    load_raw<G, NV>(raw[t], V_old, d[t] != 0.f ? ci[kk] : 0, g);
                }
#pragma unroll
                for (int t = 0; t < kUnrollW; ++t) {
                    Frag<NV> y;
                    to_frag<NV>(y, raw[t]);
                    axpy<NV>(acc, d[t], y);
                }
            }
            __syncthreads();
        }
        for (int s0 = gid; s0 < S; s0 += NGB * kUnrollW) {
            Raw<NV, T> raw[kUnrollW];
            float d[kUnrollW];
#pragma unroll
            for (int t = 0; t < kUnrollW; ++t) {
                const int s = s0 + t * NGB;
                d[t] = (s < S) ? Dl[s] : 0.f;
                load_raw<G, NV>(raw[t], V_old, d[t] != 0.f ? Ri[s] : 0, g);
            }
#pragma unroll
            for (int t = 0; t < kUnrollW; ++t) {
                Frag<NV> y;
                to_frag<NV>(y, raw[t]);
                axpy<NV>(acc, d[t], y);
            }
        }
        for (int s = tid; s < S; s += kThreads) __builtin_nontemporal_store(Dl[s], Dg + u * (int64_t)S + s);
    }

    across_groups_sum<G, NV>(acc);
#pragma unroll
    for (int off = 32; off >= 1; off >>= 1) {
        lsum += __shfl_xor(lsum, off, 64);
        npos += __shfl_xor(npos, off, 64);
    }
    __syncthreads();
    if (grp == 0) {
#pragma unroll
        for (int v = 0; v < NV; ++v) reinterpret_cast<float4*>(red + wave * LD)[g + G * v] = acc.v[v];
    }
    if (lane == 0) {
        red[kWaves * LD + wave] = lsum;
        red[kWaves * LD + kWaves + wave] = npos;
    }
    __syncthreads();
    if (wave == 0 && grp == 0) {
        Frag<NV> tot;
#pragma unroll
        for (int v = 0; v < NV; ++v) tot.v[v] = reinterpret_cast<const float4*>(red)[g + G * v];
        for (int w = 1; w < kWaves; ++w) {
            Frag<NV> part;
#pragma unroll
            for (int v = 0; v < NV; ++v) part.v[v] = reinterpret_cast<const float4*>(red + w * LD)[g + G * v];
            add<NV>(tot, part);
        }
        row_epilogue<G, NV, T>(tot, U_old, U_out, u, g, epi, adam);
    }
    if (tid == 0) {
        const float* t = red + kWaves * LD;
        if (loss_part) loss_part[u] = (t[0] + t[1]) + (t[2] + t[3]);
        if (pos_part) pos_part[u] = (t[4] + t[5]) + (t[6] + t[7]);
    }
}

template <int G, int NV, typename T>
__global__ __launch_bounds__(kThreads) void k_wmrb_user(
    const int64_t* __restrict__ rowptr, const int32_t* __restrict__ col, const float* __restrict__ val,
    const int32_t* __restrict__ R, int S, float c,
    const T* __restrict__ U_old, const T* __restrict__ V_old, void* __restrict__ U_out, float* __restrict__ delta,
    float* __restrict__ Dg, float* __restrict__ loss_part, float* __restrict__ pos_part, int epi, tmf_adam adam) {
    extern __shared__ __attribute__((aligned(16))) char smem_raw[];
    wmrb_user_body<G, NV, T>(blockIdx.x, smem_raw, rowptr, col, val, R, S, c, U_old, V_old, U_out, delta, Dg, loss_part,
                             pos_part, epi, adam);
}

static size_t wmrb_user_lds(int S, int ld) {
    return sizeof(float) * ((size_t)sp_padded(S) + round4(S) + 4 * kPosChunk + (size_t)round4(S) + 2 * kWaves * 64 +
                            (size_t)kWaves * ld + 2 * kWaves);
}

template <int G, int NV, typename T>
static int launch_wmrb_user(const int64_t* rowptr, const int32_t* col, const float* val, const int32_t* R,
                            int32_t n_users, int32_t S, float c, const T* U_old, const T* V_old,
                            void* U_out, float* delta, float* D, float* loss_part, float* pos_part, int epi,
                            tmf_adam adam, hipStream_t stream) {
    const size_t lds = wmrb_user_lds(S, 4 * G * NV);
    if (lds > 160 * 1024) {
        set_error("wmrb_user_pass: n_samples=%d does not fit LDS (%zu bytes); use the sliced pass (tmf_wmrb_scores3 ...)", S, lds);
        return TMF_E_UNSUPPORTED;
    }
    static LdsGrant grant;
    if (int rc = grant_dynamic_lds(reinterpret_cast<const void*>(&k_wmrb_user<G, NV, T>), lds, grant)) return rc;
    TMF_REQUIRE_LAUNCH(n_users, kThreads, "wmrb_user_pass");
    hipLaunchKernelGGL((k_wmrb_user<G, NV, T>), dim3((unsigned)n_users), dim3(kThreads), lds, stream, rowptr, col,
                       val, R, (int)S, c, U_old, V_old, U_out, delta, D, loss_part, pos_part, epi, adam);
    return check_launch("tmf_wmrb_user_pass");
}

#ifndef TMF_STREAM_NT
#define TMF_STREAM_NT 1
#endif
constexpr bool kStreamNT = TMF_STREAM_NT;
constexpr int kSliceUsers = 16;
constexpr int kLongRange = 48;

template <int G>
struct Stage {
    static constexpr int tile = 8 * G;
};

template <int G>
__device__ __forceinline__ int* slice_stage(char* smem_raw, int gid) {
    return reinterpret_cast<int*>(smem_raw) + gid * 2 * Stage<G>::tile;
}

template <int G, int NV, typename T, bool GRADU>
__device__ __forceinline__ void slice_list(int* ids, float* dst, const int32_t* __restrict__ list, int beg, int end,
                                           const T* __restrict__ V, const Frag<NV>& x, Frag<NV>& acc,
                                           float* __restrict__ out, const float* __restrict__ wts, int g, int safe) {
    constexpr int kStageTile = Stage<G>::tile;
    for (int t0 = beg; t0 < end; t0 += kStageTile) {
        const int cnt = (end - t0 < kStageTile) ? end - t0 : kStageTile;
        for (int e = g; e < cnt; e += G) {
            ids[e] = kStreamNT ? __builtin_nontemporal_load(list + t0 + e) : list[t0 + e];
            if (GRADU) dst[e] = kStreamNT ? __builtin_nontemporal_load(wts + t0 + e) : wts[t0 + e];
        }
        wave_lds_sync();
        float keep = 0.f;
        for (int e0 = 0; e0 < cnt; e0 += kUnrollW) {
            Raw<NV, T> raw[kUnrollW];
            float d[kUnrollW];
            static_assert(kUnrollW == 4, "vector LDS reads assume four entries per step");
            const int4 id4 = *reinterpret_cast<const int4*>(ids + e0);
            const float4 w4 = GRADU ? *reinterpret_cast<const float4*>(dst + e0) : make_float4(0.f, 0.f, 0.f, 0.f);
            const int idv[4] = {id4.x, id4.y, id4.z, id4.w};
            const float wv[4] = {w4.x, w4.y, w4.z, w4.w};
#pragma unroll
            for (int t = 0; t < kUnrollW; ++t) {
                const int e = e0 + t;
                bool want = e < cnt;
                d[t] = 0.f;
                if (GRADU && want) { d[t] = wv[t]; want = d[t] != 0.f; }
                load_raw<G, NV>(raw[t], V, want ? idv[t] : safe, g);
            }
#pragma unroll
            for (int t = 0; t < kUnrollW; ++t) {
                Frag<NV> y;
                to_frag<NV>(y, raw[t]);
                if (GRADU) {
                    axpy<NV>(acc, d[t], y);
                } else {
                    const int e = e0 + t;
                    const float pr = group_allsum<G>(dot_partial<NV>(x, y));
                    if (g == (e & (G - 1))) keep = pr;
                    if (e < cnt && ((e & (G - 1)) == G - 1 || e == cnt - 1)) {
                        if (g <= (e & (G - 1))) __builtin_nontemporal_store(keep, out + t0 + (e & ~(G - 1)) + g);
                    }
                }
            }
        }
    }
}

template <int NV, typename T>
__device__ __forceinline__ void slice_scores_lean(int* ids, const int32_t* __restrict__ list, int beg, int end, const T* __restrict__ V,
                                                  const Raw<NV, T>& x, float* __restrict__ out, int g, int lane, int safe) {
    constexpr int G = 32, kStageTile = Stage<G>::tile;
    const uint32_t loff = 16u * (uint32_t)g;
    const int my_entry = Reduce4x32::entry_of_lane(lane);
    const int my_step = lane & 7, my_slot = 4 * my_step + my_entry;
    for (int t0 = beg; t0 < end; t0 += kStageTile) {
        const int cnt = (end - t0 < kStageTile) ? end - t0 : kStageTile;
        const int cnt4 = (cnt + 3) & ~3;
        for (int e = g; e < cnt4; e += G) ids[e] = e < cnt ? (kStreamNT ? __builtin_nontemporal_load(list + t0 + e) : list[t0 + e]) : safe;
        wave_lds_sync();
        float keep = 0.f;
        for (int e0 = 0; e0 < cnt4; e0 += 4) {
            const int4 id4 = *reinterpret_cast<const int4*>(ids + e0);
            Raw<NV, T> y[4];
            load_raw32<G, NV>(y[0], V, (uint32_t)id4.x, loff);
            load_raw32<G, NV>(y[1], V, (uint32_t)id4.y, loff);
            load_raw32<G, NV>(y[2], V, (uint32_t)id4.z, loff);
            load_raw32<G, NV>(y[3], V, (uint32_t)id4.w, loff);
            float pr[4];
#pragma unroll
            for (int t = 0; t < 4; ++t) pr[t] = dot_raw<NV>(x, y[t]);
            const float sc = Reduce4x32::run(pr, lane);
            const int step = (e0 >> 2) & 7;
            keep = (step == my_step) ? sc : keep;
            if (step == 7 || e0 + 4 >= cnt4) {
                const int at = (e0 & ~31) + my_slot;
                if (at < cnt) __builtin_nontemporal_store(keep, out + t0 + at);
            }
        }
    }
}

struct SliceLists {
    const int32_t* R;
    const int32_t* off;
    const int64_t* rowptr;
    const int32_t* col;
    const int32_t* poff;
    int n_slices, S;
    int64_t n_users, n_groups;
    int upg;
    int sl0, nsl;
    int item_base;
    int xcd;
    int lean;
};

__device__ __forceinline__ bool slice_of_block(const SliceLists& a, int64_t b, int64_t& sl, int64_t& grp) {
    if (!a.xcd) {
        sl = a.sl0 + b / a.n_groups;
        grp = b % a.n_groups;
        return true;
    }
    const int64_t x = b & 7, j = b >> 3;
    sl = a.sl0 + 8 * (j / a.n_groups) + x;
    grp = j % a.n_groups;
    return sl < a.sl0 + a.nsl;
}

template <int G, int NV, typename T>
__device__ __forceinline__ const T* window_base(const T* V, int item_base) {
    return V - (int64_t)item_base * (4 * G * NV);
}

template <int G, int NV, typename T, int WAVES>
__global__ __launch_bounds__(64 * WAVES) void k_wmrb_scores3(SliceLists a, const T* __restrict__ U, const T* __restrict__ V,
                                                           float* __restrict__ sp, float* __restrict__ p) {
    extern __shared__ __attribute__((aligned(16))) char smem_raw[];
    constexpr int NG = 64 / G, NGB = NG * WAVES;
    const int tid = threadIdx.x, lane = tid & 63, wave = tid >> 6;
    const int g = lane & (G - 1), gid = wave * NG + lane / G;
    int* ids = slice_stage<G>(smem_raw, gid);
    float* dst = reinterpret_cast<float*>(ids + Stage<G>::tile);
    int64_t sl, grp;
    if (!slice_of_block(a, blockIdx.x, sl, grp)) return;
    const int64_t ubeg = grp * a.upg;
    const int64_t uend = (ubeg + a.upg < a.n_users) ? ubeg + a.upg : a.n_users;
    V = window_base<G, NV, T>(V, a.item_base);
    if constexpr (G == 32 && sizeof(Raw<NV, T>) <= 16) {
        if (a.lean) {
            for (int64_t u = ubeg + gid; u < uend; u += NGB) {
                const int64_t o = u * (a.n_slices + 1) + sl;
                const int nb = a.off[o], ne = a.off[o + 1], pb = a.poff[o], pe = a.poff[o + 1];
                if (nb == ne && pb == pe) continue;
                Raw<NV, T> x;
                {
                    const char* xp = reinterpret_cast<const char*>(U) + u * (int64_t)RowBytes<G, NV, T>::value + 16 * g;
                    if constexpr (std::is_same<T, float>::value) {
#pragma unroll
                        for (int v = 0; v < NV; ++v) x.v[v] = load_f4_nt(reinterpret_cast<const float*>(xp + 16 * G * v));
                    } else {
#pragma unroll
                        for (int pv = 0; pv < NV / 2; ++pv) x.v[pv] = __builtin_nontemporal_load(reinterpret_cast<const bf16x8*>(xp + 16 * G * pv));
                    }
                }
                slice_scores_lean<NV, T>(ids, a.R + u * (int64_t)a.S, nb, ne, V, x, sp + u * (int64_t)a.S, g, lane, a.item_base);
                const int64_t rb = a.rowptr[u];
                slice_scores_lean<NV, T>(ids, a.col + rb, pb, pe, V, x, p + rb, g, lane, a.item_base);
            }
            return;
        }
    }
    for (int64_t u = ubeg + gid; u < uend; u += NGB) {
        const int64_t o = u * (a.n_slices + 1) + sl;
        const int nb = a.off[o], ne = a.off[o + 1], pb = a.poff[o], pe = a.poff[o + 1];
        if (nb == ne && pb == pe) continue;
        Frag<NV> x, none;
        load_row_nt<G, NV>(x, U, u, g);
        slice_list<G, NV, T, false>(ids, dst, a.R + u * (int64_t)a.S, nb, ne, V, x, none, sp + u * (int64_t)a.S, nullptr, g,
                                    a.item_base);
        const int64_t rb = a.rowptr[u];
        slice_list<G, NV, T, false>(ids, dst, a.col + rb, pb, pe, V, x, none, p + rb, nullptr, g, a.item_base);
    }
}

template <int G, int NV, typename T, int WAVES>
__global__ __launch_bounds__(64 * WAVES) void k_wmrb_gradu3(SliceLists a, const T* __restrict__ V, const float* __restrict__ D,
                                                          const float* __restrict__ delta, float* __restrict__ part,
                                                          int slice_first, int accumulate) {
    extern __shared__ __attribute__((aligned(16))) char smem_raw[];
    constexpr int NG = 64 / G, NGB = NG * WAVES;
    const int tid = threadIdx.x, lane = tid & 63, wave = tid >> 6;
    const int g = lane & (G - 1), gid = wave * NG + lane / G;
    int* ids = slice_stage<G>(smem_raw, gid);
    float* dst = reinterpret_cast<float*>(ids + Stage<G>::tile);
    int64_t sl, grp, layer = 0;
    if (slice_first < 0) {
        if (!slice_of_block(a, blockIdx.x, sl, grp)) return;
    } else if (accumulate >= 3) {
        layer = blockIdx.x & 7;
        sl = slice_first + layer;
        grp = blockIdx.x >> 3;
        if (sl >= a.sl0 + a.nsl) return;
        accumulate -= 2;
    } else {
        sl = slice_first;
        grp = blockIdx.x;
    }
    V = window_base<G, NV, T>(V, a.item_base);
    const int64_t ubeg = grp * a.upg;
    const int64_t uend = (ubeg + a.upg < a.n_users) ? ubeg + a.upg : a.n_users;
    for (int64_t u = ubeg + gid; u < uend; u += NGB) {
        const int64_t o = u * (a.n_slices + 1) + sl;
        const int nb = a.off[o], ne = a.off[o + 1], pb = a.poff[o], pe = a.poff[o + 1];
        Frag<NV> acc, none;
        zero<NV>(acc);
        const int64_t us = u * (int64_t)a.S, rb = a.rowptr[u];
        slice_list<G, NV, T, true>(ids, dst, a.R + us, nb, ne, V, none, acc, nullptr, D + us, g, a.item_base);
        slice_list<G, NV, T, true>(ids, dst, a.col + rb, pb, pe, V, none, acc, nullptr, delta + rb, g, a.item_base);
        if (accumulate == 0) {
            store_row_f32<G, NV, T>(acc, part, sl * a.n_users + u, g);
        } else {
            const int64_t prow = layer * a.n_users + u;
            if (accumulate == 2) {
                Frag<NV> prev;
                load_row_f32<G, NV, T>(prev, part, prow, g);
                add<NV>(prev, acc);
                acc = prev;
            }
            store_row_f32<G, NV, T>(acc, part, prow, g);
        }
    }
}

template <int G>
struct Stage4 {
    static constexpr int cap = G < 16 ? G : 16;
};

template <int G, int NV, typename T, int K, int WAVES>
__global__ __launch_bounds__(64 * WAVES, WAVES / 2) void k_wmrb_gradu4(
    SliceLists a, const T* __restrict__ V, const float* __restrict__ D,
                                                          const float* __restrict__ delta, const T* __restrict__ U_old,
                                                          void* __restrict__ U_out, int epi, tmf_adam adam, int64_t user_begin,
                                                          int64_t user_end, int* __restrict__ sync, int lag) {
    extern __shared__ __attribute__((aligned(16))) char smem_raw[];
    constexpr int NG = 64 / G, NGB = NG * WAVES, CAP = Stage4<G>::cap, WIN = G - 1, UG = (CAP >= 8) ? kG4Unroll : kUnrollW;
    const int tid = threadIdx.x, lane = tid & 63, wave = tid >> 6;
    const int g = lane & (G - 1), gid = wave * NG + lane / G;
    int* stage = reinterpret_cast<int*>(smem_raw) + gid * (2 * K * 2 * CAP);
    V = window_base<G, NV, T>(V, a.item_base);
    const int64_t u0 = user_begin + ((int64_t)blockIdx.x * NGB + gid) * K;
    const int sl_end = a.sl0 + a.nsl;
    Frag<NV> acc[K];
    int us[K], rb[K];
    bool live[K];
    int ocn[K], ocp[K];
    int c_tot[K];
#pragma unroll
    for (int k = 0; k < K; ++k) {
        zero<NV>(acc[k]);
        live[k] = u0 + k < user_end;
        const int64_t u = live[k] ? u0 + k : user_begin;
        us[k] = (int)(u * (int64_t)a.S);
        rb[k] = (int)a.rowptr[u];
    }
    int base = a.sl0;
    auto refill = [&](int b) {
        base = b;
#pragma unroll
        for (int k = 0; k < K; ++k) {
            const int64_t u = live[k] ? u0 + k : user_begin;
            const int64_t o = u * (a.n_slices + 1) + ((b + g <= a.n_slices) ? b + g : a.n_slices);
            ocn[k] = a.off[o];
            ocp[k] = a.poff[o];
        }
    };
    int n_tot[K], n_id[K];
    float n_w[K];
    auto fetch = [&](int sl) {
#pragma unroll
        for (int k = 0; k < K; ++k) {
            const int nb = group_read<G>(ocn[k], sl - base), ne = group_read<G>(ocn[k], sl + 1 - base);
            const int pb = group_read<G>(ocp[k], sl - base), pe = group_read<G>(ocp[k], sl + 1 - base);
            const int cn = live[k] ? ne - nb : 0;
            n_tot[k] = live[k] ? cn + (pe - pb) : 0;
            const bool neg = g < cn, any = g < n_tot[k] && g < CAP;
            const int at = neg ? us[k] + nb + g : rb[k] + pb + (g - cn);
            n_id[k] = any ? (neg ? a.R : a.col)[at] : a.item_base;
            n_w[k] = any ? (neg ? D : delta)[at] : 0.f;
        }
    };
    auto commit = [&](int buf) {
#pragma unroll
        for (int k = 0; k < K; ++k) {
            int* ids = stage + (buf * K + k) * 2 * CAP;
            if (g < CAP) {
                ids[g] = n_id[k];
                reinterpret_cast<float*>(ids + CAP)[g] = n_w[k];
            }
            c_tot[k] = n_tot[k];
        }
        wave_lds_sync();
    };
    refill(a.sl0);
    fetch(a.sl0);
    commit(0);
    for (int sl = a.sl0; sl < sl_end; ++sl) {
        const int buf = (sl - a.sl0) & 1;
        const bool more = sl + 1 < sl_end;
        if (more) {
            if (sl + 2 - base > WIN) refill(sl + 1);
            fetch(sl + 1);
        }
#pragma unroll
        for (int k = 0; k < K; ++k) {
            const int* ids = stage + (buf * K + k) * 2 * CAP;
            const float* ws = reinterpret_cast<const float*>(ids + CAP);
            const int cnt = c_tot[k] < CAP ? c_tot[k] : CAP;
            for (int e0 = 0; e0 < cnt; e0 += UG) {
                static_assert(((UG == 4 || UG == 8) && CAP % UG == 0) || CAP < 4, "vector LDS reads assume four or eight entries per step");
                Raw<NV, T> raw[UG];
                float d[UG];
                int idv[UG];
                if constexpr (CAP >= 4) {
#pragma unroll
                    for (int q = 0; q < UG / 4; ++q) {
                        const int4 id4 = *reinterpret_cast<const int4*>(ids + e0 + 4 * q);
                        const float4 w4 = *reinterpret_cast<const float4*>(ws + e0 + 4 * q);
                        idv[4 * q] = id4.x; idv[4 * q + 1] = id4.y; idv[4 * q + 2] = id4.z; idv[4 * q + 3] = id4.w;
                        d[4 * q] = w4.x; d[4 * q + 1] = w4.y; d[4 * q + 2] = w4.z; d[4 * q + 3] = w4.w;
                    }
                } else {
#pragma unroll
                    for (int t = 0; t < UG; ++t) {
                        idv[t] = (e0 + t < CAP) ? ids[e0 + t] : a.item_base;
                        d[t] = (e0 + t < CAP) ? ws[e0 + t] : 0.f;
                    }
                }
#pragma unroll
                for (int t = 0; t < UG; ++t) {
                    const bool want = e0 + t < cnt && d[t] != 0.f;
                    if (!want) d[t] = 0.f;
                    load_raw<G, NV>(raw[t], V, want ? idv[t] : a.item_base, g);
                }
#pragma unroll
                for (int t = 0; t < UG; ++t) {
                    Frag<NV> y;
                    to_frag<NV>(y, raw[t]);
                    axpy<NV>(acc[k], d[t], y);
                }
            }
            if (c_tot[k] > CAP) {
                const int64_t o = (u0 + k) * (a.n_slices + 1) + sl;
                const int nb = a.off[o], cn = a.off[o + 1] - nb, pb = a.poff[o];
                for (int e = CAP; e < c_tot[k]; ++e) {
                    const bool neg = e < cn;
                    const int at = neg ? us[k] + nb + e : rb[k] + pb + (e - cn);
                    const float w = (neg ? D : delta)[at];
                    if (w != 0.f) {
                        Frag<NV> y;
                        load_row<G, NV>(y, V, (neg ? a.R : a.col)[at], g);
                        axpy<NV>(acc[k], w, y);
                    }
                }
            }
        }
        if (more) commit(buf ^ 1);
        if (sync != nullptr && tid == 0) step_rendezvous(sync, sl - a.sl0, lag, (int)gridDim.x);
        __syncthreads();
    }
#pragma unroll
    for (int k = 0; k < K; ++k)
        if (live[k]) row_epilogue<G, NV, T>(acc[k], U_old, U_out, u0 + k, g, epi, adam);
}

template <int G, int NV, typename T>
__global__ __launch_bounds__(kThreads) void k_wmrb_finish(const float* part, int n_slices, int64_t n_users,
                                                          const T* __restrict__ U_old, void* U_out, int epi,
                                                          tmf_adam adam) {
    constexpr int NG = 64 / G, NGB = NG * kWaves;
    const int lane = threadIdx.x & 63, g = lane & (G - 1);
    const int64_t u = (int64_t)blockIdx.x * NGB + (threadIdx.x >> 6) * NG + lane / G;
    if (u >= n_users) return;
    Frag<NV> acc;
    load_row_f32<G, NV, T, TMF_NT_FIN>(acc, part, u, g);
    for (int sl = 1; sl < n_slices; ++sl) {
        Frag<NV> y;
        load_row_f32<G, NV, T, TMF_NT_FIN>(y, part, sl * n_users + u, g);
        add<NV>(acc, y);
    }
    row_epilogue<G, NV, T>(acc, U_old, U_out, u, g, epi, adam);
}

}

using namespace tmf;

template <typename T>
static int wmrb_user_pass_impl(const int64_t* rowptr, const int32_t* col, const float* val, const int32_t* R,
                               int32_t n_users, int32_t S, float c, const void* U_old, const void* V_old, void* U_out,
                               float* delta, float* D, float* loss_part, float* pos_part, int n_components, int epi,
                               tmf_adam adam, void* stream) {
    if (n_users == 0) return TMF_OK;
    TMF_REQUIRE(n_users > 0 && S > 0, "wmrb_user_pass: n_users=%d S=%d", n_users, S);
    TMF_REQUIRE(rowptr && R && U_old && V_old && U_out && D, "wmrb_user_pass: null pointer");
    TMF_REQUIRE(epi == TMF_EPI_ADAM || epi == TMF_EPI_GRAD, "wmrb_user_pass: bad epilogue %d", epi);
    const RowGeom geom = row_geom_of<T>(n_components);
#define CALL(G_, NV_)                                                                                                  \
    return launch_wmrb_user<G_, NV_, T>(rowptr, col, val, R, n_users, S, c, (const T*)U_old, (const T*)V_old, U_out, \
                                        delta, D, loss_part, pos_part, epi, adam, (hipStream_t)stream)
    TMF_DISPATCH(T, geom, CALL);
#undef CALL
    return TMF_OK;
}

extern "C" int tmf_wmrb_gradu4_supported(int n_components, int bf16) {
    const RowGeom geom = bf16 ? row_geom_bf16(n_components) : row_geom(n_components);
    return geom.ld != 0 && geom.G >= 8;
}

extern "C" int tmf_wmrb_user_pass_fits(int32_t S, int n_components) {
    const RowGeom geom = row_geom(n_components);
    return geom.ld != 0 && S > 0 && wmrb_user_lds(S, geom.ld) <= 160 * 1024;
}

extern "C" int tmf_wmrb_user_pass_f32(const int64_t* rowptr, const int32_t* col, const float* val,
                                      const int32_t* R, int32_t n_users, int32_t S, float c,
                                      const float* U_old, const float* V_old, float* U_out, float* delta,
                                      float* D, float* loss_part, float* pos_part,
                                      int n_components, int epi, tmf_adam adam, void* stream) {
    return wmrb_user_pass_impl<float>(rowptr, col, val, R, n_users, S, c, U_old, V_old, U_out, delta, D, loss_part,
                                      pos_part, n_components, epi, adam, stream);
}
extern "C" int tmf_wmrb_user_pass_bf16(const int64_t* rowptr, const int32_t* col, const float* val,
                                       const int32_t* R, int32_t n_users, int32_t S, float c,
                                       const void* U_old, const void* V_old, void* U_out, float* delta,
                                       float* D, float* loss_part, float* pos_part,
                                       int n_components, int epi, tmf_adam adam, void* stream) {
    return wmrb_user_pass_impl<__bf16>(rowptr, col, val, R, n_users, S, c, U_old, V_old, U_out, delta, D, loss_part,
                                       pos_part, n_components, epi, adam, stream);
}

static int check_lists(const tmf_slice_lists* l, SliceLists& a, const char* what, int lanes_per_row, int waves, size_t row_bytes = 0) {
    TMF_REQUIRE(l != nullptr, "%s: lists is null", what);
    TMF_REQUIRE(l->n_users >= 0 && l->n_slices > 0 && l->n_samples > 0, "%s: n_users=%d n_slices=%d n_samples=%d", what,
                l->n_users, l->n_slices, l->n_samples);
    TMF_REQUIRE(l->n_users == 0 || (l->R_sorted && l->slice_off && l->rowptr && l->pos_off), "%s: null list array", what);
    const int lane_groups = (64 / (lanes_per_row > 0 ? lanes_per_row : 64)) * waves;
    int upg = kSliceUsers > lane_groups ? kSliceUsers : lane_groups;
    if (const char* env = getenv("TMF_SLICE_USERS")) {
        const int v = atoi(env);
        if (v >= 16 && v <= 1024 && (v & (v - 1)) == 0) upg = v;
    }
    const int64_t groups = ((int64_t)l->n_users + upg - 1) / upg;
    const int sl0 = l->slice_begin, nsl = l->slice_count > 0 ? l->slice_count : l->n_slices - sl0;
    TMF_REQUIRE(sl0 >= 0 && nsl > 0 && sl0 + nsl <= l->n_slices && l->item_base >= 0, "%s: window [%d, +%d) of %d slices, item_base=%d",
                what, sl0, l->slice_count, l->n_slices, l->item_base);
    int xcd = (l->flags & TMF_SLICE_XCD_MAJOR) != 0;
    if (const char* env = getenv("TMF_SLICE_XCD")) xcd = env[0] == '1';
    int lean = (l->flags & TMF_SLICE_N_ITEMS_STATED) && l->n_items > 0 && row_bytes > 0 && (int64_t)l->n_items * (int64_t)row_bytes < ((int64_t)1 << 32);
    if (const char* env = getenv("TMF_LEAN")) lean = lean && env[0] != '0';
    a = SliceLists{l->R_sorted, l->slice_off, l->rowptr, l->col, l->pos_off, l->n_slices, l->n_samples, l->n_users, groups,
                   upg, sl0, nsl, l->item_base, xcd, lean};
    return TMF_OK;
}

namespace tmf {
__global__ __launch_bounds__(256) void k_check_ids(const int32_t* __restrict__ R, int64_t n_neg, const int32_t* __restrict__ col,
                                                   const int64_t* __restrict__ rowptr, int64_t n_users, int n_items, int* __restrict__ bad) {
    const int64_t nnz = col ? rowptr[n_users] : 0;
    for (int64_t i = (int64_t)blockIdx.x * blockDim.x + threadIdx.x; i < n_neg + nnz; i += (int64_t)gridDim.x * blockDim.x) {
        const int id = i < n_neg ? R[i] : col[i - n_neg];
        if (id < 0 || id >= n_items) atomicAdd(bad, 1);
    }
}
}
static int check_ids_debug(const tmf_slice_lists* l, hipStream_t stream) {
    const char* env = getenv("TMF_CHECK_IDS");
    if (!(env && env[0] == '1') || !(l->flags & TMF_SLICE_N_ITEMS_STATED) || l->n_users == 0) return TMF_OK;
    int* bad = nullptr;
    int host = 0;
    if (hipMalloc(&bad, sizeof(int)) != hipSuccess || hipMemsetAsync(bad, 0, sizeof(int), stream) != hipSuccess) {
        set_error("TMF_CHECK_IDS: could not allocate the flag");
        return TMF_E_LAUNCH;
    }
    hipLaunchKernelGGL(tmf::k_check_ids, dim3(1024), dim3(256), 0, stream, l->R_sorted, (int64_t)l->n_users * l->n_samples, l->col,
                       l->rowptr, (int64_t)l->n_users, (int)l->n_items, bad);
    const bool ok = hipMemcpyAsync(&host, bad, sizeof(int), hipMemcpyDeviceToHost, stream) == hipSuccess &&
                    hipStreamSynchronize(stream) == hipSuccess;
    (void)hipFree(bad);
    if (!ok) { set_error("TMF_CHECK_IDS: the check itself failed"); return TMF_E_LAUNCH; }
    TMF_REQUIRE(host == 0, "tmf_slice_lists: %d ids of R_sorted / col are outside [0, n_items = %d)", host, l->n_items);
    return TMF_OK;
}

static unsigned slice_grid(const SliceLists& a) {
    return (unsigned)(a.xcd ? a.n_groups * 8 * ((a.nsl + 7) / 8) : a.n_groups * a.nsl);
}

static size_t slice_lds(const RowGeom& geom, int waves) {
    return (size_t)(64 / (geom.G ? geom.G : 1)) * waves * 2 * 8 * geom.G * sizeof(int);
}

static int slice_waves(const tmf_slice_lists* l, int lanes_per_row) {
    if (const char* env = getenv("TMF_SLICE_WAVES")) {
        const int v = atoi(env);
        if (v == 4 || v == 8) return v;
    }
    return (l && l->n_slices > 0 && l->n_samples / l->n_slices >= kLongRange && lanes_per_row >= 32) ? 8 : 4;
}

template <typename T>
static int wmrb_scores3_impl(const tmf_slice_lists* lists, const void* U, const void* V, float* sp, float* p,
                             int n_components, void* stream) {
    SliceLists a;
    const RowGeom geom = row_geom_of<T>(n_components);
    const int waves = slice_waves(lists, geom.G);
    if (int rc = check_lists(lists, a, "wmrb_scores3", geom.G, waves, (size_t)geom.ld * sizeof(T))) return rc;
    if (a.n_users == 0) return TMF_OK;
    if (int rc = check_ids_debug(lists, (hipStream_t)stream)) return rc;
    TMF_REQUIRE(U && V && sp && (p || lists->col == nullptr), "wmrb_scores3: null pointer");
    const size_t lds = slice_lds(geom, waves);
    const int unit = a.xcd ? 8 : 1;
    const int64_t per_unit = a.n_groups * unit * 64 * waves;
    const int max_units = (int)((((int64_t)1 << 32) - 1) / per_unit);
    TMF_REQUIRE(max_units >= 1, "wmrb_scores3: %lld user groups exceed one launch", (long long)a.n_groups);
    const int first = a.sl0, last = a.sl0 + a.nsl;
    for (int s0 = first; s0 < last; s0 += max_units * unit) {
        a.sl0 = s0;
        a.nsl = (last - s0 < max_units * unit) ? last - s0 : max_units * unit;
#define CALLW(G_, NV_, W_)                                                                                             \
    hipLaunchKernelGGL((k_wmrb_scores3<G_, NV_, T, W_>), dim3(slice_grid(a)), dim3(64 * W_), lds, \
                       (hipStream_t)stream, a, (const T*)U, (const T*)V, sp, p)
#define CALL4(G_, NV_) CALLW(G_, NV_, 4)
#define CALL8(G_, NV_) CALLW(G_, NV_, 8)
        if (waves == 8) { TMF_DISPATCH(T, geom, CALL8); } else { TMF_DISPATCH(T, geom, CALL4); }
#undef CALL4
#undef CALL8
#undef CALLW
    }
    return check_launch("tmf_wmrb_scores3");
}

template <typename T>
static int wmrb_gradu3_impl(const tmf_slice_lists* lists, const float* D, const float* delta, const void* V, float* part,
                            int per_slice_launches, int n_components, void* stream) {
    SliceLists a;
    const RowGeom geom = row_geom_of<T>(n_components);
    const int waves = slice_waves(lists, geom.G);
    if (int rc = check_lists(lists, a, "wmrb_gradu3", geom.G, waves)) return rc;
    if (a.n_users == 0) return TMF_OK;
    TMF_REQUIRE(D && V && part && (delta || lists->col == nullptr), "wmrb_gradu3: null pointer");
    const size_t lds = slice_lds(geom, waves);
    TMF_REQUIRE(per_slice_launches >= 0 && per_slice_launches <= 3, "wmrb_gradu3: per_slice_launches=%d", per_slice_launches);
    if (per_slice_launches == 3) {
        TMF_REQUIRE_LAUNCH(a.n_groups * 8, 64 * waves, "wmrb_gradu3 (rounds of eight slices)");
        for (int sl = a.sl0; sl < a.sl0 + a.nsl; sl += 8) {
            const int accumulate = (sl == a.sl0) ? 3 : 4;
#define CALLW(G_, NV_, W_)                                                                                                       \
    hipLaunchKernelGGL((k_wmrb_gradu3<G_, NV_, T, W_>), dim3((unsigned)(a.n_groups * 8)), dim3(64 * W_), lds, (hipStream_t)stream, a, \
                       (const T*)V, D, delta, part, sl, accumulate)
#define CALL4(G_, NV_) CALLW(G_, NV_, 4)
#define CALL8(G_, NV_) CALLW(G_, NV_, 8)
            if (waves == 8) { TMF_DISPATCH(T, geom, CALL8); } else { TMF_DISPATCH(T, geom, CALL4); }
#undef CALL4
#undef CALL8
#undef CALLW
        }
        return check_launch("tmf_wmrb_gradu3");
    }
    if (per_slice_launches) {
        TMF_REQUIRE_LAUNCH(a.n_groups, 64 * waves, "wmrb_gradu3 (one launch per slice)");
        for (int sl = a.sl0; sl < a.sl0 + a.nsl; ++sl) {
            const int accumulate = (sl == a.sl0 && per_slice_launches == 1) ? 1 : 2;
#define CALLW(G_, NV_, W_)                                                                                                   \
    hipLaunchKernelGGL((k_wmrb_gradu3<G_, NV_, T, W_>), dim3((unsigned)a.n_groups), dim3(64 * W_), lds, (hipStream_t)stream, a, \
                       (const T*)V, D, delta, part, sl, accumulate)
#define CALL4(G_, NV_) CALLW(G_, NV_, 4)
#define CALL8(G_, NV_) CALLW(G_, NV_, 8)
            if (waves == 8) { TMF_DISPATCH(T, geom, CALL8); } else { TMF_DISPATCH(T, geom, CALL4); }
#undef CALL4
#undef CALL8
#undef CALLW
        }
        return check_launch("tmf_wmrb_gradu3");
    }
    const int unit = a.xcd ? 8 : 1;
    const int64_t per_unit = a.n_groups * unit * 64 * waves;
    const int max_units = (int)((((int64_t)1 << 32) - 1) / per_unit);
    TMF_REQUIRE(max_units >= 1, "wmrb_gradu3: %lld user groups exceed one launch", (long long)a.n_groups);
    const int first = a.sl0, last = a.sl0 + a.nsl;
    for (int s0 = first; s0 < last; s0 += max_units * unit) {
        a.sl0 = s0;
        a.nsl = (last - s0 < max_units * unit) ? last - s0 : max_units * unit;
#define CALLW(G_, NV_, W_)                                                                                   \
    hipLaunchKernelGGL((k_wmrb_gradu3<G_, NV_, T, W_>), dim3(slice_grid(a)), dim3(64 * W_), lds, \
                       (hipStream_t)stream, a, (const T*)V, D, delta, part, -1, 0)
#define CALL4(G_, NV_) CALLW(G_, NV_, 4)
#define CALL8(G_, NV_) CALLW(G_, NV_, 8)
        if (waves == 8) { TMF_DISPATCH(T, geom, CALL8); } else { TMF_DISPATCH(T, geom, CALL4); }
#undef CALL4
#undef CALL8
#undef CALLW
    }
    return check_launch("tmf_wmrb_gradu3");
}

static size_t gradu4_workspace(int64_t n_users, int n_slices, int64_t users_per_launch) {
    const int64_t launches = users_per_launch > 0 ? (n_users + users_per_launch - 1) / users_per_launch : 0;
    return rendezvous_bytes(launches, n_slices);
}

extern "C" size_t tmf_wmrb_gradu4_workspace_bytes(int32_t n_users, int32_t n_slices, int32_t users_per_launch) {
    return gradu4_workspace(n_users, n_slices, users_per_launch);
}

template <typename T>
static int wmrb_gradu4_impl(const tmf_slice_lists* lists, const float* D, const float* delta, const void* V, const void* U_old,
                            void* U_out, int n_components, int epi, tmf_adam adam, int32_t users_per_launch, void* workspace,
                            size_t workspace_bytes, void* stream) {
    SliceLists a;
    const RowGeom geom = row_geom_of<T>(n_components);
    constexpr int W4 = 8;
    if (int rc = check_lists(lists, a, "wmrb_gradu4", geom.G, W4)) return rc;
    if (a.n_users == 0) return TMF_OK;
    TMF_REQUIRE(D && V && U_out && (delta || lists->col == nullptr) && (epi == TMF_EPI_GRAD || U_old), "wmrb_gradu4: null pointer");
    TMF_REQUIRE(epi == TMF_EPI_ADAM || epi == TMF_EPI_GRAD, "wmrb_gradu4: bad epilogue %d", epi);
    TMF_REQUIRE(users_per_launch > 0, "wmrb_gradu4: users_per_launch=%d", users_per_launch);
    if (geom.G < 8) {
        set_error("wmrb_gradu4: rows of %d lanes are too narrow for the row-stationary form; use tmf_wmrb_gradu3 + tmf_wmrb_finish", geom.G);
        return TMF_E_UNSUPPORTED;
    }
#ifndef TMF_G4_K
#define TMF_G4_K 4
#endif
    constexpr int K4 = TMF_G4_K;
    const int cap = geom.G < 16 ? geom.G : 16;
    const size_t lds = (size_t)(64 / geom.G) * W4 * 2 * K4 * 2 * cap * sizeof(int);
    const int64_t per_block = (int64_t)(64 / geom.G) * W4 * K4;
    int* sync = nullptr;
    if (workspace != nullptr) {
        const size_t need = gradu4_workspace(a.n_users, a.nsl, users_per_launch);
        TMF_REQUIRE(workspace_bytes >= need, "wmrb_gradu4: workspace of %zu bytes, %zu needed", workspace_bytes, need);
        if (hipMemsetAsync(workspace, 0, need, (hipStream_t)stream) != hipSuccess) { set_error("wmrb_gradu4: hipMemsetAsync failed"); return TMF_E_LAUNCH; }
        sync = static_cast<int*>(workspace);
    }
    int lag = 1;
    if (const char* env = getenv("TMF_G4_LAG")) lag = atoi(env);
    if (getenv("TMF_DEBUG")) {
        int nb = -1, dev = 0, cus = 0;
        (void)hipGetDevice(&dev);
        (void)hipDeviceGetAttribute(&cus, hipDeviceAttributeMultiprocessorCount, dev);
#define CALL(G_, NV_) (void)hipOccupancyMaxActiveBlocksPerMultiprocessor(&nb, k_wmrb_gradu4<G_, NV_, T, K4, W4>, 64 * W4, lds)
        TMF_DISPATCH(T, geom, CALL);
#undef CALL
        fprintf(stderr, "[tmf] gradu4: %d workgroups per CU x %d CUs resident, %lld users per workgroup, lds %zu, lag %d\n", nb, cus,
                (long long)per_block, lds, lag);
    }
    for (int64_t b = 0, launch = 0; b < a.n_users; b += users_per_launch, ++launch) {
        const int64_t e = (b + users_per_launch < a.n_users) ? b + users_per_launch : a.n_users;
        const unsigned blocks = (unsigned)((e - b + per_block - 1) / per_block);
        int* sy = (sync && lag >= 0) ? sync + launch * a.nsl * 8 * kSyncStride : nullptr;
#define CALL(G_, NV_)                                                                                                         \
    hipLaunchKernelGGL((k_wmrb_gradu4<G_, NV_, T, K4, W4>), dim3(blocks), dim3(64 * W4), lds, (hipStream_t)stream, a, (const T*)V, \
                       D, delta, (const T*)U_old, U_out, epi, adam, b, e, sy, lag)
        TMF_DISPATCH(T, geom, CALL);
#undef CALL
    }
    return check_launch("tmf_wmrb_gradu4");
}


namespace tmf {
constexpr int kS5Users = 256;
constexpr int kS5Waves = 15;
constexpr int kS5Pad = INT32_MIN;
constexpr int kS5MaxWindows = 4096;
constexpr int kS5Stride = 16;

struct S5Pace {
    const int32_t* wst;
    int* cnt;
    int nw, lag;
};

template <int NV, typename T>
__global__ __launch_bounds__(64 * (kS5Waves + 1)) void k_wmrb_scores5(const int32_t* __restrict__ ids, const int32_t* __restrict__ outs,
                                                                     const int64_t* __restrict__ wg_ptr, int64_t wg0, int64_t n_users,
                                                                     const T* __restrict__ U, const T* __restrict__ V,
                                                                     float* __restrict__ sp, float* __restrict__ p, S5Pace pace) {
    constexpr int G = 32, NGB = 2 * kS5Waves;
    constexpr uint32_t RB = RowBytes<G, NV, T>::value;
    extern __shared__ __attribute__((aligned(16))) char smem_raw[];
    __shared__ int s_win[kS5Waves];
    __shared__ int s_gate;
    int* wst = reinterpret_cast<int*>(smem_raw + (size_t)kS5Users * RB);
    const int tid = threadIdx.x, lane = tid & 63, wave = tid >> 6, g = lane & (G - 1), gid = tid / G;
    const int64_t wg = wg0 + blockIdx.x;
    const int64_t ubeg = wg * kS5Users;
    const int nu = (int)((n_users - ubeg < kS5Users) ? n_users - ubeg : kS5Users);
    const bool paced = pace.cnt != nullptr;
    {
        const tmf_f4* src = reinterpret_cast<const tmf_f4*>(reinterpret_cast<const char*>(U) + ubeg * (int64_t)RB);
        tmf_f4* dst = reinterpret_cast<tmf_f4*>(smem_raw);
        for (int i = tid; i < nu * (int)(RB / 16); i += 64 * (kS5Waves + 1)) dst[i] = __builtin_nontemporal_load(src + i);
        if (paced)
            for (int i = tid; i <= pace.nw; i += 64 * (kS5Waves + 1)) wst[i] = pace.wst[wg * (pace.nw + 1) + i];
        if (tid < kS5Waves) s_win[tid] = 0;
        if (tid == 0) s_gate = paced ? pace.lag : INT32_MAX;
    }
    __syncthreads();
    if (wave == kS5Waves) {
        if (!paced) return;
        const int x = blockIdx.x & 7, peers = ((int)gridDim.x - x + 7) / 8;
        int* cnt = pace.cnt + (size_t)x * pace.nw * kS5Stride;
        int published = 0, gate = pace.lag, idle = 0;
        bool open = false;
        for (;;) {
            int mn = (lane < kS5Waves) ? __hip_atomic_load(&s_win[lane], __ATOMIC_RELAXED, __HIP_MEMORY_SCOPE_WORKGROUP) : INT32_MAX;
#pragma unroll
            for (int o = 8; o >= 1; o >>= 1) mn = min(mn, __shfl_xor(mn, o, 64));
            mn = __builtin_amdgcn_readfirstlane(mn);
            const bool done = mn == INT32_MAX;
            const int target = done ? pace.nw : mn;
            if (lane == 0)
                for (int w = published; w < target; ++w) __hip_atomic_fetch_add(cnt + (size_t)w * kS5Stride, 1, __ATOMIC_RELAXED, __HIP_MEMORY_SCOPE_AGENT);
            if (target > published) published = target;
            if (done) return;
            if (!open && gate < pace.nw - 1) {
                int c = (lane == 0) ? __hip_atomic_load(cnt + (size_t)(gate - pace.lag) * kS5Stride, __ATOMIC_RELAXED, __HIP_MEMORY_SCOPE_AGENT) : 0;
                c = __builtin_amdgcn_readfirstlane(c);
                if (c >= peers) {
                    ++gate;
                    idle = 0;
                    if (lane == 0) __hip_atomic_store(&s_gate, gate, __ATOMIC_RELAXED, __HIP_MEMORY_SCOPE_WORKGROUP);
                    continue;
                }
                if (++idle > 4000) {
                    open = true;
                    if (lane == 0) __hip_atomic_store(&s_gate, INT32_MAX, __ATOMIC_RELAXED, __HIP_MEMORY_SCOPE_WORKGROUP);
                }
            }
            __builtin_amdgcn_s_sleep(4);
        }
    }
    const int64_t beg = wg_ptr[wg], end = wg_ptr[wg + 1];
    const int steps = (int)((end - beg) >> 3);
    const uint32_t loff = 16u * (uint32_t)g;
    const int my_entry = Reduce8x32::entry_of_lane(lane);
    const bool owner = Reduce8x32::owner(lane);
    const int4* id4 = reinterpret_cast<const int4*>(ids + beg);
    const int32_t* out8 = outs + beg + my_entry;
    const int mine = steps > gid ? (steps - gid + NGB - 1) / NGB : 0;
    const int rounds = __builtin_amdgcn_readfirstlane(mine);
    if (rounds > 0) {
        const int last = mine > 0 ? gid + NGB * (mine - 1) : 0;
        struct Ids {
            int4 a, b;
            int o;
        };
        auto fetch = [&](int i) {
            const int st = gid + NGB * i;
            const int sc = st <= last ? st : last;
            Ids r{id4[2 * sc], id4[2 * sc + 1], out8[8 * sc]};
            if (i >= mine) r.o = kS5Pad;
            return r;
        };
        int cur_w = 0, next_b = paced ? wst[1] : INT32_MAX;
        auto pace_to = [&](int i) {
            if (!paced || i >= rounds || cur_w >= pace.nw - 1) return;
            const int st_w = __builtin_amdgcn_readfirstlane(gid + NGB * i);
            if (st_w < next_b) return;
            do {
                ++cur_w;
                next_b = wst[cur_w + 1];
            } while (st_w >= next_b && cur_w < pace.nw - 1);
            if (lane == 0) __hip_atomic_store(&s_win[wave], cur_w, __ATOMIC_RELAXED, __HIP_MEMORY_SCOPE_WORKGROUP);
            for (int spin = 0; spin < 20000; ++spin) {
                if (__hip_atomic_load(&s_gate, __ATOMIC_RELAXED, __HIP_MEMORY_SCOPE_WORKGROUP) >= cur_w) break;
                __builtin_amdgcn_s_sleep(2);
            }
        };
        auto gather = [&](Raw<NV, T> (&y)[8], const Ids& d) {
            const int idv[8] = {d.a.x, d.a.y, d.a.z, d.a.w, d.b.x, d.b.y, d.b.z, d.b.w};
#pragma unroll
            for (int t = 0; t < 8; ++t) load_raw32<G, NV>(y[t], V, (uint32_t)idv[t] & 0xffffffu, loff);
        };
        auto finish = [&](const Raw<NV, T> (&y)[8], const Ids& d) {
            const int idv[8] = {d.a.x, d.a.y, d.a.z, d.a.w, d.b.x, d.b.y, d.b.z, d.b.w};
            float pr[8];
#pragma unroll
            for (int t = 0; t < 8; ++t) {
                Raw<NV, T> x;
                const char* xr = smem_raw + ((uint32_t)idv[t] >> 24) * RB + loff;
                if constexpr (std::is_same<T, float>::value) {
#pragma unroll
                    for (int v = 0; v < NV; ++v) x.v[v] = *reinterpret_cast<const float4*>(xr + 16 * G * v);
                } else {
#pragma unroll
                    for (int pv = 0; pv < NV / 2; ++pv) x.v[pv] = *reinterpret_cast<const bf16x8*>(xr + 16 * G * pv);
                }
                pr[t] = dot_raw<NV>(x, y[t]);
            }
            const float sc = Reduce8x32::run(pr, lane);
            if (owner && d.o != kS5Pad) __builtin_nontemporal_store(sc, d.o >= 0 ? sp + d.o : p + ~d.o);
        };
        Raw<NV, T> yA[8], yB[8];
        Ids A = fetch(0);
        Ids B = fetch(1);
        pace_to(0);
        gather(yA, A);
        for (int i = 0; i < rounds; i += 2) {
            Ids C = fetch(i + 2);
            __builtin_amdgcn_sched_barrier(0);
            pace_to(i + 1);
            gather(yB, B);
            __builtin_amdgcn_sched_barrier(0);
            finish(yA, A);
            __builtin_amdgcn_sched_barrier(0);
            if (i + 1 >= rounds) break;
            Ids Dn = fetch(i + 3);
            __builtin_amdgcn_sched_barrier(0);
            pace_to(i + 2);
            gather(yA, C);
            __builtin_amdgcn_sched_barrier(0);
            finish(yB, B);
            __builtin_amdgcn_sched_barrier(0);
            A = C;
            B = Dn;
        }
    }
    if (lane == 0) __hip_atomic_store(&s_win[wave], INT32_MAX, __ATOMIC_RELAXED, __HIP_MEMORY_SCOPE_WORKGROUP);
}

}

namespace tmf {
#ifndef TMF_S6_USERS
#define TMF_S6_USERS 64
#endif
#ifndef TMF_S6_WAVES
#define TMF_S6_WAVES 8
#endif
#ifndef TMF_S6_ROUNDS
#define TMF_S6_ROUNDS 1
#endif
constexpr int kS6Users = TMF_S6_USERS;
constexpr int kS6Waves = TMF_S6_WAVES;

template <int NV, typename T>
__global__ __launch_bounds__(64 * kS6Waves) void k_wmrb_scores6(const int32_t* __restrict__ ids, const int32_t* __restrict__ outs,
                                                                const int64_t* __restrict__ chunk_ptr, int64_t chunk0, int64_t n_groups,
                                                                int64_t n_users, const T* __restrict__ U, const T* __restrict__ V,
                                                                float* __restrict__ sp, float* __restrict__ p) {
    constexpr int G = 32, NGB = 2 * kS6Waves;
    constexpr uint32_t RB = RowBytes<G, NV, T>::value;
    __shared__ __attribute__((aligned(16))) char smem_raw[kS6Users * RB];
    const int tid = threadIdx.x, lane = tid & 63, g = lane & (G - 1), gid = tid / G;
    const int64_t chunk = chunk0 + blockIdx.x;
    const int64_t beg = chunk_ptr[chunk], end = chunk_ptr[chunk + 1];
    if (beg == end) return;
    const int64_t ubeg = (chunk % n_groups) * kS6Users;
    const int nu = (int)((n_users - ubeg < kS6Users) ? n_users - ubeg : kS6Users);
    {
        const tmf_f4* src = reinterpret_cast<const tmf_f4*>(reinterpret_cast<const char*>(U) + ubeg * (int64_t)RB);
        tmf_f4* dst = reinterpret_cast<tmf_f4*>(smem_raw);
        for (int i = tid; i < nu * (int)(RB / 16); i += 64 * kS6Waves) dst[i] = __builtin_nontemporal_load(src + i);
    }
    __syncthreads();
    const int steps = (int)((end - beg) >> 3);
    const uint32_t loff = 16u * (uint32_t)g;
    const int my_entry = Reduce8x32::entry_of_lane(lane);
    const bool owner = Reduce8x32::owner(lane);
    const int4* id4 = reinterpret_cast<const int4*>(ids + beg);
    const int32_t* out8 = outs + beg + my_entry;
    const int mine = steps > gid ? (steps - gid + NGB - 1) / NGB : 0;
    const int rounds = __builtin_amdgcn_readfirstlane(mine);
    if (rounds == 0) return;
    const int last = mine > 0 ? gid + NGB * (mine - 1) : 0;
    struct Ids {
        int4 a, b;
        int o;
    };
    auto fetch = [&](int i) {
        const int st = gid + NGB * i;
        const int sc = st <= last ? st : last;
        Ids r{id4[2 * sc], id4[2 * sc + 1], out8[8 * sc]};
        if (i >= mine) r.o = kS5Pad;
        return r;
    };
    auto gather = [&](Raw<NV, T> (&y)[8], const Ids& d) {
        const int idv[8] = {d.a.x, d.a.y, d.a.z, d.a.w, d.b.x, d.b.y, d.b.z, d.b.w};
#pragma unroll
        for (int t = 0; t < 8; ++t) load_raw32<G, NV>(y[t], V, (uint32_t)idv[t] & 0xffffffu, loff);
    };
    auto finish = [&](const Raw<NV, T> (&y)[8], const Ids& d) {
        const int idv[8] = {d.a.x, d.a.y, d.a.z, d.a.w, d.b.x, d.b.y, d.b.z, d.b.w};
        float pr[8];
#pragma unroll
        for (int t = 0; t < 8; ++t) {
            Raw<NV, T> x;
            const char* xr = smem_raw + ((uint32_t)idv[t] >> 24) * RB + loff;
            if constexpr (std::is_same<T, float>::value) {
#pragma unroll
                for (int v = 0; v < NV; ++v) x.v[v] = *reinterpret_cast<const float4*>(xr + 16 * G * v);
            } else {
#pragma unroll
                for (int pv = 0; pv < NV / 2; ++pv) x.v[pv] = *reinterpret_cast<const bf16x8*>(xr + 16 * G * pv);
            }
            pr[t] = dot_raw<NV>(x, y[t]);
        }
        const float sc = Reduce8x32::run(pr, lane);
        if (owner && d.o != kS5Pad) __builtin_nontemporal_store(sc, d.o >= 0 ? sp + d.o : p + ~d.o);
    };
#if TMF_S6_ROUNDS == 1
    {
        Raw<NV, T> yA[8];
        Ids A = fetch(0);
        for (int i = 0; i < rounds; ++i) {
            Ids B = fetch(i + 1);
            __builtin_amdgcn_sched_barrier(0);
            gather(yA, A);
            __builtin_amdgcn_sched_barrier(0);
            finish(yA, A);
            A = B;
        }
        return;
    }
#endif
    Raw<NV, T> yA[8], yB[8];
    Ids A = fetch(0);
    Ids B = fetch(1);
    gather(yA, A);
    for (int i = 0; i < rounds; i += 2) {
        Ids C = fetch(i + 2);
        __builtin_amdgcn_sched_barrier(0);
        gather(yB, B);
        __builtin_amdgcn_sched_barrier(0);
        finish(yA, A);
        __builtin_amdgcn_sched_barrier(0);
        if (i + 1 >= rounds) break;
        Ids Dn = fetch(i + 3);
        __builtin_amdgcn_sched_barrier(0);
        gather(yA, C);
        __builtin_amdgcn_sched_barrier(0);
        finish(yB, B);
        __builtin_amdgcn_sched_barrier(0);
        A = C;
        B = Dn;
    }
}

}

static bool s6_supported(int n_components, int bf16, int64_t n_items) {
    const tmf::RowGeom geom = bf16 ? tmf::row_geom_bf16(n_components) : tmf::row_geom(n_components);
    const int64_t row_bytes = (int64_t)geom.ld * (bf16 ? 2 : 4);
    return geom.G == 32 && n_items > 0 && n_items < (1 << 24) && n_items * row_bytes < ((int64_t)1 << 32);
}

template <typename T>
static int wmrb_scores6_impl(const int32_t* ids, const int32_t* outs, const int64_t* chunk_ptr, int64_t n_groups, int32_t n_slices,
                             int64_t n_users, int64_t n_items, const void* U, const void* V, float* sp, float* p, int n_components,
                             void* stream) {
    if (n_users == 0 || n_slices == 0) return TMF_OK;
    const RowGeom geom = row_geom_of<T>(n_components);
    TMF_REQUIRE(ids && outs && chunk_ptr && U && V && sp && p, "wmrb_scores6: null pointer");
    TMF_REQUIRE(n_groups == (n_users + kS6Users - 1) / kS6Users && n_slices > 0, "wmrb_scores6: %lld groups for %lld users (%d per group), %d slices",
                (long long)n_groups, (long long)n_users, kS6Users, n_slices);
    if (!s6_supported(n_components, std::is_same<T, __bf16>::value, n_items)) {
        set_error("wmrb_scores6: needs rows of 32 lanes (fp32 65..128 / bf16 129..256 components) and fewer than 2^24 items in a table "
                  "below 4 GB (got %d components, %lld items)", n_components, (long long)n_items);
        return TMF_E_UNSUPPORTED;
    }
    const int64_t per_slice = n_groups * 64 * kS6Waves;
    const int max_slices = (int)((((int64_t)1 << 32) - 1) / per_slice);
    TMF_REQUIRE(max_slices >= 1, "wmrb_scores6: %lld user groups exceed one launch", (long long)n_groups);
    for (int s0 = 0; s0 < n_slices; s0 += max_slices) {
        const int nsl = (n_slices - s0 < max_slices) ? n_slices - s0 : max_slices;
        const unsigned blocks = (unsigned)(n_groups * nsl);
#define CALL(G_, NV_)                                                                                                       \
    {                                                                                                                       \
        if constexpr (G_ == 32) {                                                                                           \
            hipLaunchKernelGGL((k_wmrb_scores6<NV_, T>), dim3(blocks), dim3(64 * kS6Waves), 0, (hipStream_t)stream, ids, outs, \
                               chunk_ptr, (int64_t)s0 * n_groups, n_groups, n_users, (const T*)U, (const T*)V, sp, p);      \
        }                                                                                                                   \
    }
        TMF_DISPATCH(T, geom, CALL);
#undef CALL
    }
    return check_launch("tmf_wmrb_scores6");
}

static int s5_launches(int64_t n_wg, int wgs_per_launch) { return (int)((n_wg + wgs_per_launch - 1) / wgs_per_launch); }
static int s5_wgs_per_launch(int wgs_per_launch) {
    if (wgs_per_launch > 0) return wgs_per_launch;
    int dev = 0, cus = 256;
    if (hipGetDevice(&dev) == hipSuccess) (void)hipDeviceGetAttribute(&cus, hipDeviceAttributeMultiprocessorCount, dev);
    return cus > 0 ? cus : 256;
}

template <typename T>
static int wmrb_scores5_impl(const int32_t* ids, const int32_t* outs, const int64_t* wg_ptr, int64_t n_wg, int64_t n_users,
                             int64_t n_items, const void* U, const void* V, float* sp, float* p, int n_components,
                             int wgs_per_launch, const int32_t* wstart, int32_t n_windows, int lag, void* workspace,
                             size_t workspace_bytes, void* stream) {
    if (n_wg == 0 || n_users == 0) return TMF_OK;
    const RowGeom geom = row_geom_of<T>(n_components);
    TMF_REQUIRE(ids && outs && wg_ptr && U && V && sp && p, "wmrb_scores5: null pointer");
    TMF_REQUIRE(n_wg == (n_users + kS5Users - 1) / kS5Users, "wmrb_scores5: %lld workgroups for %lld users (%d per workgroup)",
                (long long)n_wg, (long long)n_users, kS5Users);
    const size_t row_bytes = (size_t)geom.ld * sizeof(T);
    if (geom.G != 32 || row_bytes * kS5Users > 128 * 1024 || n_items <= 0 || n_items >= (1 << 24) ||
        (int64_t)n_items * (int64_t)row_bytes >= ((int64_t)1 << 32)) {
        set_error("wmrb_scores5: needs rows of 32 lanes (fp32 65..128 / bf16 129..256 components) and fewer than 2^24 items "
                  "in a table below 4 GB (got %d components, %lld items)", n_components, (long long)n_items);
        return TMF_E_UNSUPPORTED;
    }
    wgs_per_launch = s5_wgs_per_launch(wgs_per_launch);
    const int launches = s5_launches(n_wg, wgs_per_launch);
    const bool paced = wstart != nullptr && workspace != nullptr && n_windows > 1;
    const size_t per_launch = (size_t)8 * (paced ? n_windows : 0) * kS5Stride * sizeof(int);
    if (paced) {
        TMF_REQUIRE(n_windows <= kS5MaxWindows && lag >= 0, "wmrb_scores5: %d windows (at most %d), lag %d", n_windows, kS5MaxWindows, lag);
        TMF_REQUIRE(workspace_bytes >= per_launch * launches, "wmrb_scores5: workspace of %zu bytes needed, got %zu", per_launch * launches,
                    workspace_bytes);
        if (hipMemsetAsync(workspace, 0, per_launch * launches, (hipStream_t)stream) != hipSuccess) {
            set_error("wmrb_scores5: hipMemsetAsync failed");
            return TMF_E_LAUNCH;
        }
    }
    const size_t lds = row_bytes * kS5Users + (paced ? (size_t)(n_windows + 1) * sizeof(int) : 0);
#define CALL(G_, NV_)                                                                                                       \
    {                                                                                                                       \
        if constexpr (G_ == 32) {                                                                                           \
            static LdsGrant grant;                                                                                          \
            if (int rc = grant_dynamic_lds(reinterpret_cast<const void*>(&k_wmrb_scores5<NV_, T>), lds, grant)) return rc;  \
            for (int l = 0; l < launches; ++l) {                                                                            \
                const int64_t w0 = (int64_t)l * wgs_per_launch;                                                             \
                const unsigned blocks = (unsigned)((n_wg - w0 < wgs_per_launch) ? n_wg - w0 : wgs_per_launch);              \
                const S5Pace pace{wstart, paced ? reinterpret_cast<int*>(static_cast<char*>(workspace) + per_launch * l) : nullptr, \
                                  n_windows, lag};                                                                          \
                hipLaunchKernelGGL((k_wmrb_scores5<NV_, T>), dim3(blocks), dim3(64 * (kS5Waves + 1)), lds, (hipStream_t)stream, \
                                   ids, outs, wg_ptr, w0, n_users, (const T*)U, (const T*)V, sp, p, pace);                  \
            }                                                                                                               \
        }                                                                                                                   \
    }
    TMF_DISPATCH(T, geom, CALL);
#undef CALL
    return check_launch("tmf_wmrb_scores5");
}

template <typename T>
static int wmrb_finish_impl(const float* part, int32_t n_slices, int32_t n_users, const void* U_old, void* U_out,
                            int n_components, int epi, tmf_adam adam, void* stream) {
    if (n_users == 0) return TMF_OK;
    TMF_REQUIRE(part && U_out && n_slices > 0 && (epi == TMF_EPI_GRAD || U_old), "wmrb_finish: bad arguments");
    TMF_REQUIRE(epi == TMF_EPI_ADAM || epi == TMF_EPI_GRAD, "wmrb_finish: bad epilogue %d", epi);
    const RowGeom geom = row_geom_of<T>(n_components);
#define CALL(G_, NV_)                                                                                                  \
    {                                                                                                                  \
        constexpr int per_block = (64 / G_) * kWaves;                                                                  \
        hipLaunchKernelGGL((k_wmrb_finish<G_, NV_, T>), dim3((unsigned)(((int64_t)n_users + per_block - 1) / per_block)), \
                           dim3(kThreads), 0, (hipStream_t)stream, part, (int)n_slices, (int64_t)n_users,                \
                           (const T*)U_old, U_out, epi, adam);                                                         \
    }
    TMF_DISPATCH(T, geom, CALL);
#undef CALL
    return check_launch("tmf_wmrb_finish");
}

#define TMF_SLICED_ENTRY_POINTS(SFX, T_)                                                                                  \
    extern "C" int tmf_wmrb_scores3_##SFX(const tmf_slice_lists* lists, const void* U, const void* V, float* sp, float* p, \
                                          int n_components, void* stream) {                                               \
        return wmrb_scores3_impl<T_>(lists, U, V, sp, p, n_components, stream);                                           \
    }                                                                                                                     \
    extern "C" int tmf_wmrb_scores5_##SFX(const int32_t* ids, const int32_t* outs, const int64_t* wg_ptr, int64_t n_wg,    \
                                          int64_t n_users, int64_t n_items, const void* U, const void* V, float* sp,      \
                                          float* p, int n_components, int wgs_per_launch, const int32_t* wstart,          \
                                          int32_t n_windows, int lag, void* workspace, size_t workspace_bytes,            \
                                          void* stream) {                                                                 \
        return wmrb_scores5_impl<T_>(ids, outs, wg_ptr, n_wg, n_users, n_items, U, V, sp, p, n_components, wgs_per_launch, \
                                     wstart, n_windows, lag, workspace, workspace_bytes, stream);                         \
    }                                                                                                                     \
    extern "C" int tmf_wmrb_scores6_##SFX(const int32_t* ids, const int32_t* outs, const int64_t* chunk_ptr, int64_t n_groups, \
                                          int32_t n_slices, int64_t n_users, int64_t n_items, const void* U, const void* V, \
                                          float* sp, float* p, int n_components, void* stream) {                          \
        return wmrb_scores6_impl<T_>(ids, outs, chunk_ptr, n_groups, n_slices, n_users, n_items, U, V, sp, p, n_components, stream); \
    }                                                                                                                     \
    extern "C" int tmf_wmrb_gradu3_##SFX(const tmf_slice_lists* lists, const float* D, const float* delta,                \
                                         const void* V, float* part, int per_slice_launches, int n_components,            \
                                         void* stream) {                                                                  \
        return wmrb_gradu3_impl<T_>(lists, D, delta, V, part, per_slice_launches, n_components, stream);                  \
    }                                                                                                                     \
    extern "C" int tmf_wmrb_gradu4_##SFX(const tmf_slice_lists* lists, const float* D, const float* delta, const void* V,  \
                                         const void* U_old, void* U_out, int n_components, int epi, tmf_adam adam,       \
                                         int32_t users_per_launch, void* workspace, size_t workspace_bytes, void* stream) { \
        return wmrb_gradu4_impl<T_>(lists, D, delta, V, U_old, U_out, n_components, epi, adam, users_per_launch, workspace, \
                                    workspace_bytes, stream);                                                            \
    }                                                                                                                     \
    extern "C" int tmf_wmrb_finish_##SFX(const float* part, int32_t n_slices, int32_t n_users, const void* U_old,         \
                                         void* U_out, int n_components, int epi, tmf_adam adam, void* stream) {           \
        return wmrb_finish_impl<T_>(part, n_slices, n_users, U_old, U_out, n_components, epi, adam, stream);               \
    }

TMF_SLICED_ENTRY_POINTS(f32, float)
TMF_SLICED_ENTRY_POINTS(bf16, __bf16)

extern "C" int tmf_wmrb_scores6_users_per_group(void) { return tmf::kS6Users; }
extern "C" int tmf_wmrb_scores6_supported(int n_components, int bf16, int64_t n_items) { return s6_supported(n_components, bf16, n_items); }
extern "C" int tmf_wmrb_scores5_users_per_workgroup(void) { return tmf::kS5Users; }
extern "C" size_t tmf_wmrb_scores5_workspace_bytes(int64_t n_wg, int32_t n_windows, int wgs_per_launch) {
    if (n_wg <= 0 || n_windows <= 1) return 0;
    return (size_t)s5_launches(n_wg, s5_wgs_per_launch(wgs_per_launch)) * 8 * (size_t)n_windows * tmf::kS5Stride * sizeof(int);
}
extern "C" int tmf_wmrb_scores5_supported(int n_components, int bf16, int64_t n_items) {
    const tmf::RowGeom geom = bf16 ? tmf::row_geom_bf16(n_components) : tmf::row_geom(n_components);
    const int64_t row_bytes = (int64_t)geom.ld * (bf16 ? 2 : 4);
    return geom.G == 32 && row_bytes * tmf::kS5Users <= 128 * 1024 && n_items > 0 && n_items < (1 << 24) &&
           n_items * row_bytes < ((int64_t)1 << 32);
}
```

Before: 1.146 billion.

## Fuse last-slice scoring into hinge kernel and finish into last gradu slice

```diff
diff --git a/include/tmf.h b/include/tmf.h
--- a/include/tmf.h
+++ b/include/tmf.h
@@ -133,10 +133,21 @@
 int tmf_wmrb_hinge2_ordered(const int64_t* rowptr, const float* val, const float* p, const float* sp, int32_t n_users,
                             int32_t n_samples, float c, float* delta, float* D, float* loss_part, const int32_t* user_order,
                             void* stream);
+int tmf_wmrb_hinge2_tail_supported(int n_components, int bf16);
+int tmf_wmrb_hinge2_tail_f32(const tmf_slice_lists* lists, const void* U, const void* V, const float* val, float* sp, float* p,
+                             float c, float* delta, float* D, float* loss_part, const int32_t* group_order, int n_components,
+                             void* stream);
+int tmf_wmrb_hinge2_tail_bf16(const tmf_slice_lists* lists, const void* U, const void* V, const float* val, float* sp, float* p,
+                              float c, float* delta, float* D, float* loss_part, const int32_t* group_order, int n_components,
+                              void* stream);
 int tmf_wmrb_gradu3_f32(const tmf_slice_lists* lists, const float* D, const float* delta, const void* V, float* part,
                         int per_slice_launches, int n_components, void* stream);
 int tmf_wmrb_gradu3_bf16(const tmf_slice_lists* lists, const float* D, const float* delta, const void* V, float* part,
                          int per_slice_launches, int n_components, void* stream);
+int tmf_wmrb_gradu3_finish_f32(const tmf_slice_lists* lists, const float* D, const float* delta, const void* V, float* part,
+                               const void* U_old, void* U_out, int n_components, int epi, tmf_adam adam, void* stream);
+int tmf_wmrb_gradu3_finish_bf16(const tmf_slice_lists* lists, const float* D, const float* delta, const void* V, float* part,
+                                const void* U_old, void* U_out, int n_components, int epi, tmf_adam adam, void* stream);
 int tmf_wmrb_gradu4_supported(int n_components, int bf16);
 size_t tmf_wmrb_gradu4_workspace_bytes(int32_t n_users, int32_t n_slices, int32_t users_per_launch);
 int tmf_wmrb_gradu4_f32(const tmf_slice_lists* lists, const float* D, const float* delta, const void* V, const void* U_old,
diff --git a/teamoflow_amd/_engine.py b/teamoflow_amd/_engine.py
--- a/teamoflow_amd/_engine.py
+++ b/teamoflow_amd/_engine.py
@@ -300,6 +300,24 @@
     if passes.numel() == 0 or int(passes.max()) <= 1:
         return None
     return torch.argsort(passes, descending=True, stable=True).to(torch.int32)
+
+
+TAIL_GROUP = 16
+TAIL_SLICES = 1
+
+
+def hinge_group_order(rowptr_u):
+    if os.environ.get('TMF_HINGE_ORDER', '1') == '0':
+        return None
+    deg = rowptr_u[1:] - rowptr_u[:-1]
+    passes = (deg + (HINGE_CHUNK - 1)) // HINGE_CHUNK
+    if passes.numel() == 0 or int(passes.max()) <= 1:
+        return None
+    pad = (-passes.numel()) % TAIL_GROUP
+    if pad:
+        passes = torch.cat([passes, passes.new_zeros(pad)])
+    worst = passes.view(-1, TAIL_GROUP).max(dim=1)[0]
+    return torch.argsort(worst, descending=True, stable=True).to(torch.int32)
 
 
 class WmrbPlan:
@@ -382,6 +400,8 @@
         self.wbuf = torch.zeros(E, dtype=torch.float32, device=dev)
         self.delta = self.wbuf[:nnz]
         self.hinge_order = hinge_user_order(plan.rowptr_u)
+        self.hinge_group_order = hinge_group_order(plan.rowptr_u) if self.sliced else None
+        self._tail_lists = {}
         self.D = self.wbuf[nnz:].view(m, S)
         self._lists = None
         self.s5 = None
@@ -393,6 +413,16 @@
                                           plan.col_u.data_ptr(), self.pos_off.data_ptr(), m, S, self.n_slices, 0, 0, 0,
                                           (_lib.SLICE_XCD_MAJOR if self.xcd_major else 0) | _lib.SLICE_N_ITEMS_STATED, int(plan.n_items))
         return ctypes.byref(self._lists)
+
+    def range_lists(self, plan, slice_begin, slice_count):
+        key = (slice_begin, slice_count)
+        if key not in self._tail_lists:
+            m, S = self.R.shape
+            self._tail_lists[key] = _lib.SliceLists(self.R.data_ptr(), self.slice_off.data_ptr(), plan.rowptr_u.data_ptr(),
+                                                    plan.col_u.data_ptr(), self.pos_off.data_ptr(), m, S, self.n_slices, slice_begin,
+                                                    slice_count, 0, (_lib.SLICE_XCD_MAJOR if self.xcd_major else 0) | _lib.SLICE_N_ITEMS_STATED,
+                                                    int(plan.n_items))
+        return ctypes.byref(self._tail_lists[key])
 
     def window_lists(self, plan, slice_begin, slice_count, item_base):
         m, S = self.R.shape
@@ -744,6 +774,14 @@
     _row_pass_finish(lib, p.seg_i, st.slab, st.V, V_out, r, item_epi, adam, s, st.sfx)
 
 
+def tail_slices(st, ns):
+    if os.environ.get('TMF_FUSED_TAIL', '1') == '0' or st.row_stationary:
+        return 0
+    if not _lib.load_library().tmf_wmrb_hinge2_tail_supported(st.r, int(st.dtype is torch.bfloat16)):
+        return 0
+    return max(0, min(int(os.environ.get('TMF_TAIL_SLICES', TAIL_SLICES)), ns))
+
+
 def _wmrb_user_pass_sliced(lib, st, adam, c, prof=None, user_epi=_lib.EPI_ADAM, U_out=None):
     p, w, r = st.plan, st.wplan, st.r
     i32 = ctypes.c_int32
@@ -758,6 +796,7 @@
         if prof:
             prof.stop(name)
     s5, s6 = getattr(w, 's5', None), getattr(w, 's6', None)
+    k = tail_slices(st, ns) if s5 is None and s6 is None else 0
     if s6 is not None:
         timed('wmrb_scores', lambda: getattr(lib, 'tmf_wmrb_scores6' + st.sfx)(
             _lib.ptr(s6.ids), _lib.ptr(s6.outs), _lib.ptr(s6.chunk_ptr), s6.n_groups, i32(s6.n_slices), m, p.n_items, _lib.ptr(st.U),
@@ -767,16 +806,29 @@
             _lib.ptr(s5.ids), _lib.ptr(s5.outs), _lib.ptr(s5.wg_ptr), s5.n_wg, m, p.n_items, _lib.ptr(st.U), _lib.ptr(st.V),
             _lib.ptr(st.sp), _lib.ptr(st.pk), r, s5.wgs_per_launch, _lib.ptr(s5.wstart) if s5.paced else None, i32(s5.n_windows),
             s5.lag, _lib.ptr(s5.sync) if s5.paced else None, s5.sync.numel() * 4, s))
+    elif k:
+        if k < ns:
+            timed('wmrb_scores', lambda: getattr(lib, 'tmf_wmrb_scores3' + st.sfx)(
+                w.range_lists(p, 0, ns - k), _lib.ptr(st.U), _lib.ptr(st.V), _lib.ptr(st.sp), _lib.ptr(st.pk), r, s))
+        timed('wmrb_hinge', lambda: getattr(lib, 'tmf_wmrb_hinge2_tail' + st.sfx)(
+            w.range_lists(p, ns - k, k), _lib.ptr(st.U), _lib.ptr(st.V), _lib.ptr(p.val_u), _lib.ptr(st.sp), _lib.ptr(st.pk), c,
+            _lib.ptr(w.delta), _lib.ptr(w.D), _lib.ptr(st.loss_part), _lib.ptr(w.hinge_group_order), r, s))
     else:
         timed('wmrb_scores', lambda: getattr(lib, 'tmf_wmrb_scores3' + st.sfx)(lists, _lib.ptr(st.U), _lib.ptr(st.V), _lib.ptr(st.sp),
                                                                                 _lib.ptr(st.pk), r, s))
-    timed('wmrb_hinge', lambda: lib.tmf_wmrb_hinge2_ordered(_lib.ptr(p.rowptr_u), _lib.ptr(p.val_u), _lib.ptr(st.pk), _lib.ptr(st.sp),
-                                                            i32(m), i32(S), c, _lib.ptr(w.delta), _lib.ptr(w.D), _lib.ptr(st.loss_part),
-                                                            _lib.ptr(w.hinge_order), s))
+    if not k:
+        timed('wmrb_hinge', lambda: lib.tmf_wmrb_hinge2_ordered(_lib.ptr(p.rowptr_u), _lib.ptr(p.val_u), _lib.ptr(st.pk), _lib.ptr(st.sp),
+                                                                i32(m), i32(S), c, _lib.ptr(w.delta), _lib.ptr(w.D), _lib.ptr(st.loss_part),
+                                                                _lib.ptr(w.hinge_order), s))
     if st.row_stationary:
         timed('wmrb_gradu', lambda: getattr(lib, 'tmf_wmrb_gradu4' + st.sfx)(
             lists, _lib.ptr(w.D), _lib.ptr(w.delta), _lib.ptr(st.V), _lib.ptr(st.U), _lib.ptr(st.U_nxt if U_out is None else U_out),
             r, user_epi, adam, i32(st.users_per_launch), _lib.ptr(st.g4_sync), st.g4_sync.numel() * 4, s))
+        return
+    if st.gradu_launches == 0 and os.environ.get('TMF_FUSED_TAIL', '1') != '0':
+        timed('wmrb_gradu', lambda: getattr(lib, 'tmf_wmrb_gradu3_finish' + st.sfx)(
+            lists, _lib.ptr(w.D), _lib.ptr(w.delta), _lib.ptr(st.V), _lib.ptr(st.part), _lib.ptr(st.U),
+            _lib.ptr(st.U_nxt if U_out is None else U_out), r, user_epi, adam, s))
         return
     timed('wmrb_gradu', lambda: getattr(lib, 'tmf_wmrb_gradu3' + st.sfx)(
         lists, _lib.ptr(w.D), _lib.ptr(w.delta), _lib.ptr(st.V), _lib.ptr(st.part),
diff --git a/teamoflow_amd/_lib.py b/teamoflow_amd/_lib.py
--- a/teamoflow_amd/_lib.py
+++ b/teamoflow_amd/_lib.py
@@ -90,7 +90,10 @@
     'tmf_wmrb_scores5_f32': (_I, [_P, _P, _P, _L, _L, _L, _P, _P, _P, _P, _I, _I, _P, _I32, _I, _P, _SZ, _P]),
     'tmf_wmrb_hinge2': (_I, [_P, _P, _P, _P, _I32, _I32, _F, _P, _P, _P, _P]),
     'tmf_wmrb_hinge2_ordered': (_I, [_P, _P, _P, _P, _I32, _I32, _F, _P, _P, _P, _P, _P]),
+    'tmf_wmrb_hinge2_tail_supported': (_I, [_I, _I]),
+    'tmf_wmrb_hinge2_tail_f32': (_I, [_SL, _P, _P, _P, _P, _P, _F, _P, _P, _P, _P, _I, _P]),
     'tmf_wmrb_gradu3_f32': (_I, [_SL, _P, _P, _P, _P, _I, _I, _P]),
+    'tmf_wmrb_gradu3_finish_f32': (_I, [_SL, _P, _P, _P, _P, _P, _P, _I, _I, Adam, _P]),
     'tmf_wmrb_gradu4_supported': (_I, [_I, _I]),
     'tmf_wmrb_gradu4_workspace_bytes': (_SZ, [_I32, _I32, _I32]),
     'tmf_wmrb_gradu4_f32': (_I, [_SL, _P, _P, _P, _P, _P, _I, _I, Adam, _I32, _P, _SZ, _P]),
@@ -135,7 +138,7 @@
 }
 
 SIGNATURES.update(_BASE_SIGNATURES)
-for _name in ('tmf_wmrb_scores3', 'tmf_wmrb_scores5', 'tmf_wmrb_scores6', 'tmf_wmrb_gradu3', 'tmf_wmrb_gradu4', 'tmf_wmrb_finish'):
+for _name in ('tmf_wmrb_scores3', 'tmf_wmrb_scores5', 'tmf_wmrb_scores6', 'tmf_wmrb_hinge2_tail', 'tmf_wmrb_gradu3', 'tmf_wmrb_gradu3_finish', 'tmf_wmrb_gradu4', 'tmf_wmrb_finish'):
     SIGNATURES[_name + '_bf16'] = SIGNATURES[_name + '_f32']
 
 _lib = None
diff --git a/teamoflow_amd/csrc/tmf_hinge.h b/teamoflow_amd/csrc/tmf_hinge.h
--- /dev/null
+++ b/teamoflow_amd/csrc/tmf_hinge.h
@@ -0,0 +1,287 @@
+#pragma once
+#include <math.h>
+
+#include "tmf_common.h"
+
+namespace tmf {
+
+constexpr int HK = 256;
+constexpr int HCHUNK = HK - 1;
+constexpr int HPAD = HK + HK / 32;
+constexpr int HSPL = 8;
+constexpr int HWAVES = 1;
+
+struct HingeLds {
+    unsigned long long keys[HK];
+    float ts[HPAD];
+    float pw[HPAD];
+    unsigned int cnt[HK];
+    unsigned char ord[HK];
+};
+
+__device__ __forceinline__ unsigned int orderable(float t) {
+    const unsigned int u = __float_as_uint(t);
+    return u ^ ((u >> 31) ? 0xffffffffu : 0x80000000u);
+}
+
+__device__ __forceinline__ int pad_slot(int i) { return i + (i >> 5); }
+
+template <int STEP>
+__device__ __forceinline__ void search_step(const float* __restrict__ ts, const float (&x)[HSPL], int (&pp)[HSPL]) {
+    constexpr int SP = STEP + (STEP >> 5);
+    constexpr int OFF = (STEP >= 32) ? SP - 2 : STEP - 1;
+    float tv[HSPL];
+#pragma unroll
+    for (int j = 0; j < HSPL; ++j) tv[j] = ts[pp[j] + OFF];
+#pragma unroll
+    for (int j = 0; j < HSPL; ++j) pp[j] += (tv[j] <= x[j]) ? SP : 0;
+}
+
+__device__ __forceinline__ void search_tile(const float* __restrict__ ts, const float (&x)[HSPL], int (&rho)[HSPL], int nfin) {
+    int pp[HSPL];
+#pragma unroll
+    for (int j = 0; j < HSPL; ++j) pp[j] = 0;
+    if (nfin >= 128) search_step<128>(ts, x, pp);
+    if (nfin >= 64) search_step<64>(ts, x, pp);
+    if (nfin >= 32) search_step<32>(ts, x, pp);
+    if (nfin >= 16) search_step<16>(ts, x, pp);
+    search_step<8>(ts, x, pp);
+    search_step<4>(ts, x, pp);
+    search_step<2>(ts, x, pp);
+    search_step<1>(ts, x, pp);
+#pragma unroll
+    for (int j = 0; j < HSPL; ++j) {
+        const int r = pp[j] - pp[j] / 33;
+        rho[j] = r < nfin ? r : nfin;
+    }
+}
+
+__device__ __forceinline__ void load_tile(const float* __restrict__ spu, int s0, int S, int lane, float (&x)[HSPL]) {
+#pragma unroll
+    for (int j = 0; j < HSPL; ++j) {
+        const int s = s0 + lane + 64 * j;
+        x[j] = (s < S) ? spu[s] : __builtin_nanf("");
+    }
+}
+
+inline int hinge_fixbits(int64_t S) {
+    int lg = 0;
+    while (((int64_t)1 << lg) < S) ++lg;
+    return 62 - lg;
+}
+
+__device__ __forceinline__ void hinge_user(int64_t u, int lane, HingeLds& L, const int64_t* __restrict__ rowptr,
+                                           const float* __restrict__ val, const float* __restrict__ p,
+                                           const float* __restrict__ sp, int S, int fixbits, float c,
+                                           float* __restrict__ delta, float* __restrict__ D, float* __restrict__ loss_part) {
+    const int64_t rb = rowptr[u], re = rowptr[u + 1];
+    const float* spu = sp + u * (int64_t)S;
+    float* Du = D + u * (int64_t)S;
+    const int ntiles = (S + 64 * HSPL - 1) / (64 * HSPL);
+
+    float lsum = 0.f;
+    bool wrote = false;
+    for (int64_t cb = rb; cb < re; cb += HCHUNK) {
+        const int len = (int)((re - cb < HCHUNK) ? (re - cb) : HCHUNK);
+        float tq[4];
+        unsigned long long kq[4];
+        int nfin = 0;
+#pragma unroll
+        for (int q = 0; q < 4; ++q) {
+            const int i = lane + 64 * q;
+            float t = INFINITY;
+            if (i < len) {
+                const float a = val[cb + i];
+                if (a > 0.f) t = -(1.0f - p[cb + i]);
+            }
+            tq[q] = t;
+            kq[q] = ((unsigned long long)orderable(t) << 32) | (unsigned int)i;
+            nfin += __popcll(__ballot(t < INFINITY));
+            if (i < len) L.keys[i] = kq[q];
+        }
+        if (nfin == 0) {
+            for (int i = lane; i < len; i += 64) delta[cb + i] = 0.f;
+            continue;
+        }
+        wave_lds_sync();
+        int rank[4] = {0, 0, 0, 0};
+        if (len <= 64) {
+            for (int j = 0; j < len; ++j) rank[0] += (L.keys[j] < kq[0]) ? 1 : 0;
+        } else if (len <= 128) {
+            for (int j = 0; j < len; ++j) {
+                const unsigned long long kj = L.keys[j];
+                rank[0] += (kj < kq[0]) ? 1 : 0;
+                rank[1] += (kj < kq[1]) ? 1 : 0;
+            }
+        } else {
+            for (int j = 0; j < len; ++j) {
+                const unsigned long long kj = L.keys[j];
+#pragma unroll
+                for (int q = 0; q < 4; ++q) rank[q] += (kj < kq[q]) ? 1 : 0;
+            }
+        }
+#pragma unroll
+        for (int q = 0; q < 4; ++q) {
+            const int i = lane + 64 * q;
+            if (i < len) {
+                L.ts[pad_slot(rank[q])] = tq[q];
+                L.ord[rank[q]] = (unsigned char)i;
+            } else if (i < HK) {
+                L.ts[pad_slot(i)] = INFINITY;
+            }
+        }
+        wave_lds_sync();
+        float town[4];
+        int oown[4];
+#pragma unroll
+        for (int q = 0; q < 4; ++q) {
+            const int pos = 4 * lane + q;
+            town[q] = L.ts[pad_slot(pos)];
+            oown[q] = (pos < len) ? (int)L.ord[pos] : -1;
+            L.cnt[pos] = 0u;
+            L.keys[pos] = 0ull;
+        }
+        const float B = fmaxf(fabsf(L.ts[0]), fabsf(L.ts[pad_slot(nfin - 1)]));
+        int eB = 0;
+        (void)frexpf(B, &eB);
+        if (!(B < INFINITY)) eB = 128;
+        const double to_fix = ldexp(1.0, fixbits - eB), from_fix = ldexp(1.0, eB - fixbits);
+        wave_lds_sync();
+        int ctop = 0;
+        double stop = 0.0;
+        unsigned int rpk[4];
+        for (int tp = 0; tp < ntiles; tp += 2) {
+#pragma unroll
+            for (int h = 0; h < 2; ++h) {
+                const int tile = tp + h;
+                if (tile >= ntiles) break;
+                float x[HSPL];
+                int rho[HSPL];
+                load_tile(spu, tile * 64 * HSPL, S, lane, x);
+                search_tile(L.ts, x, rho, nfin);
+#pragma unroll
+                for (int j = 0; j < HSPL; ++j) {
+                    if (rho[j] == nfin) {
+                        ctop += 1;
+                        stop += (double)x[j];
+                    } else if (rho[j] != 0 && fabsf(x[j]) <= B) {
+                        atomicAdd(&L.cnt[rho[j]], 1u);
+                        atomicAdd(&L.keys[rho[j]], (unsigned long long)__double2ll_rn((double)x[j] * to_fix));
+                    }
+                }
+                if (tp == 0) {
+                    rpk[2 * h] = (unsigned)rho[0] | ((unsigned)rho[1] << 8) | ((unsigned)rho[2] << 16) | ((unsigned)rho[3] << 24);
+                    rpk[2 * h + 1] = (unsigned)rho[4] | ((unsigned)rho[5] << 8) | ((unsigned)rho[6] << 16) | ((unsigned)rho[7] << 24);
+                }
+            }
+        }
+#pragma unroll
+        for (int off = 32; off >= 1; off >>= 1) {
+            ctop += __shfl_xor(ctop, off, 64);
+            stop += __shfl_xor(stop, off, 64);
+        }
+        wave_lds_sync();
+        int csuf[4];
+        long long fsuf[4];
+        {
+            int crun = 0;
+            long long frun = 0;
+#pragma unroll
+            for (int q = 3; q >= 0; --q) {
+                const int b = 4 * lane + q + 1;
+                if (b < HK) {
+                    crun += (int)L.cnt[b];
+                    frun += (long long)L.keys[b];
+                }
+                csuf[q] = crun;
+                fsuf[q] = frun;
+            }
+            int cinc = crun;
+            long long finc = frun;
+#pragma unroll
+            for (int off = 1; off < 64; off <<= 1) {
+                const int co = __shfl_down(cinc, off, 64);
+                const long long fo = __shfl_down(finc, off, 64);
+                if (lane + off < 64) {
+                    cinc += co;
+                    finc += fo;
+                }
+            }
+            const int cex = cinc - crun;
+            const long long fex = finc - frun;
+#pragma unroll
+            for (int q = 0; q < 4; ++q) {
+                csuf[q] += cex;
+                fsuf[q] += fex;
+            }
+        }
+        float wown[4];
+#pragma unroll
+        for (int q = 0; q < 4; ++q) {
+            const int pos = 4 * lane + q;
+            float w = 0.f, d = 0.f;
+            if (pos < nfin) {
+                const int cn = csuf[q] + ctop;
+                const float c1 = -town[q];
+                double hs = (double)cn * (double)c1 + ((double)fsuf[q] * from_fix + stop);
+                hs = hs > 0.0 ? hs : 0.0;
+                const float M = c * (float)hs;
+                lsum += logf(1.0f + M);
+                w = c * __frcp_rn(1.0f + M);
+                d = -(w * (float)cn);
+            }
+            wown[q] = w;
+            if (oown[q] >= 0) delta[cb + oown[q]] = d;
+        }
+        {
+            const float l0 = wown[0], l1 = l0 + wown[1], l2 = l1 + wown[2], l3 = l2 + wown[3];
+            float inc = l3;
+#pragma unroll
+            for (int off = 1; off < 64; off <<= 1) {
+                const float o = __shfl_up(inc, off, 64);
+                if (lane >= off) inc += o;
+            }
+            const float ex = __shfl_up(inc, 1, 64);
+            const float base = (lane == 0) ? 0.f : ex;
+            L.pw[pad_slot(4 * lane)] = base;
+            L.pw[pad_slot(4 * lane + 1)] = base + l0;
+            L.pw[pad_slot(4 * lane + 2)] = base + l1;
+            L.pw[pad_slot(4 * lane + 3)] = base + l2;
+        }
+        wave_lds_sync();
+        for (int tp = 0; tp < ntiles; tp += 2) {
+#pragma unroll
+            for (int h = 0; h < 2; ++h) {
+                const int tile = tp + h;
+                if (tile >= ntiles) break;
+                int rho[HSPL];
+                if (ntiles <= 2) {
+#pragma unroll
+                    for (int j = 0; j < HSPL; ++j) rho[j] = (int)((rpk[2 * h + (j >> 2)] >> (8 * (j & 3))) & 0xffu);
+                } else {
+                    float x[HSPL];
+                    load_tile(spu, tile * 64 * HSPL, S, lane, x);
+                    search_tile(L.ts, x, rho, nfin);
+                }
+#pragma unroll
+                for (int j = 0; j < HSPL; ++j) {
+                    const int s = tile * 64 * HSPL + lane + 64 * j;
+                    if (s < S) {
+                        const float dv = L.pw[pad_slot(rho[j])];
+                        if (wrote) Du[s] += dv;
+                        else Du[s] = dv;
+                    }
+                }
+            }
+        }
+        wrote = true;
+        wave_lds_sync();
+    }
+    if (!wrote)
+        for (int s = lane; s < S; s += 64) Du[s] = 0.f;
+#pragma unroll
+    for (int off = 32; off >= 1; off >>= 1) lsum += __shfl_xor(lsum, off, 64);
+    if (lane == 0 && loss_part) loss_part[u] = lsum;
+}
+
+}
diff --git a/teamoflow_amd/csrc/tmf_hinge.hip b/teamoflow_amd/csrc/tmf_hinge.hip
--- a/teamoflow_amd/csrc/tmf_hinge.hip
+++ b/teamoflow_amd/csrc/tmf_hinge.hip
@@ -1,67 +1,6 @@
-#include <math.h>
-
-#include "tmf_common.h"
+#include "tmf_hinge.h"
 
 namespace tmf {
-
-constexpr int HK = 256;
-constexpr int HCHUNK = HK - 1;
-constexpr int HPAD = HK + HK / 32;
-constexpr int HSPL = 8;
-constexpr int HWAVES = 1;
-
-struct HingeLds {
-    unsigned long long keys[HK];
-    float ts[HPAD];
-    float pw[HPAD];
-    unsigned int cnt[HK];
-    unsigned char ord[HK];
-};
-
-__device__ __forceinline__ unsigned int orderable(float t) {
-    const unsigned int u = __float_as_uint(t);
-    return u ^ ((u >> 31) ? 0xffffffffu : 0x80000000u);
-}
-
-__device__ __forceinline__ int pad_slot(int i) { return i + (i >> 5); }
-
-template <int STEP>
-__device__ __forceinline__ void search_step(const float* __restrict__ ts, const float (&x)[HSPL], int (&pp)[HSPL]) {
-    constexpr int SP = STEP + (STEP >> 5);
-    constexpr int OFF = (STEP >= 32) ? SP - 2 : STEP - 1;
-    float tv[HSPL];
-#pragma unroll
-    for (int j = 0; j < HSPL; ++j) tv[j] = ts[pp[j] + OFF];
-#pragma unroll
-    for (int j = 0; j < HSPL; ++j) pp[j] += (tv[j] <= x[j]) ? SP : 0;
-}
-
-__device__ __forceinline__ void search_tile(const float* __restrict__ ts, const float (&x)[HSPL], int (&rho)[HSPL], int nfin) {
-    int pp[HSPL];
-#pragma unroll
-    for (int j = 0; j < HSPL; ++j) pp[j] = 0;
-    if (nfin >= 128) search_step<128>(ts, x, pp);
-    if (nfin >= 64) search_step<64>(ts, x, pp);
-    if (nfin >= 32) search_step<32>(ts, x, pp);
-    if (nfin >= 16) search_step<16>(ts, x, pp);
-    search_step<8>(ts, x, pp);
-    search_step<4>(ts, x, pp);
-    search_step<2>(ts, x, pp);
-    search_step<1>(ts, x, pp);
-#pragma unroll
-    for (int j = 0; j < HSPL; ++j) {
-        const int r = pp[j] - pp[j] / 33;
-        rho[j] = r < nfin ? r : nfin;
-    }
-}
-
-__device__ __forceinline__ void load_tile(const float* __restrict__ spu, int s0, int S, int lane, float (&x)[HSPL]) {
-#pragma unroll
-    for (int j = 0; j < HSPL; ++j) {
-        const int s = s0 + lane + 64 * j;
-        x[j] = (s < S) ? spu[s] : __builtin_nanf("");
-    }
-}
 
 __global__ __launch_bounds__(64 * HWAVES) void k_wmrb_hinge2(
     const int64_t* __restrict__ rowptr, const float* __restrict__ val, const float* __restrict__ p,
@@ -72,215 +11,7 @@
     const int64_t slot = (int64_t)blockIdx.x * HWAVES + wave;
     if (slot >= n_users) return;
     const int64_t u = order ? (int64_t)order[slot] : slot;
-    HingeLds& L = lds_all[wave];
-    const int64_t rb = rowptr[u], re = rowptr[u + 1];
-    const float* spu = sp + u * (int64_t)S;
-    float* Du = D + u * (int64_t)S;
-    const int ntiles = (S + 64 * HSPL - 1) / (64 * HSPL);
-
-    float lsum = 0.f;
-    bool wrote = false;
-    for (int64_t cb = rb; cb < re; cb += HCHUNK) {
-        const int len = (int)((re - cb < HCHUNK) ? (re - cb) : HCHUNK);
-        float tq[4];
-        unsigned long long kq[4];
-        int nfin = 0;
-#pragma unroll
-        for (int q = 0; q < 4; ++q) {
-            const int i = lane + 64 * q;
-            float t = INFINITY;
-            if (i < len) {
-                const float a = val[cb + i];
-                if (a > 0.f) t = -(1.0f - p[cb + i]);
-            }
-            tq[q] = t;
-            kq[q] = ((unsigned long long)orderable(t) << 32) | (unsigned int)i;
-            nfin += __popcll(__ballot(t < INFINITY));
-            if (i < len) L.keys[i] = kq[q];
-        }
-        if (nfin == 0) {
-            for (int i = lane; i < len; i += 64) delta[cb + i] = 0.f;
-            continue;
-        }
-        wave_lds_sync();
-        int rank[4] = {0, 0, 0, 0};
-        if (len <= 64) {
-            for (int j = 0; j < len; ++j) rank[0] += (L.keys[j] < kq[0]) ? 1 : 0;
-        } else if (len <= 128) {
-            for (int j = 0; j < len; ++j) {
-                const unsigned long long kj = L.keys[j];
-                rank[0] += (kj < kq[0]) ? 1 : 0;
-                rank[1] += (kj < kq[1]) ? 1 : 0;
-            }
-        } else {
-            for (int j = 0; j < len; ++j) {
-                const unsigned long long kj = L.keys[j];
-#pragma unroll
-                for (int q = 0; q < 4; ++q) rank[q] += (kj < kq[q]) ? 1 : 0;
-            }
-        }
-#pragma unroll
-        for (int q = 0; q < 4; ++q) {
-            const int i = lane + 64 * q;
-            if (i < len) {
-                L.ts[pad_slot(rank[q])] = tq[q];
-                L.ord[rank[q]] = (unsigned char)i;
-            } else if (i < HK) {
-                L.ts[pad_slot(i)] = INFINITY;
-            }
-        }
-        wave_lds_sync();
-        float town[4];
-        int oown[4];
-#pragma unroll
-        for (int q = 0; q < 4; ++q) {
-            const int pos = 4 * lane + q;
-            town[q] = L.ts[pad_slot(pos)];
-            oown[q] = (pos < len) ? (int)L.ord[pos] : -1;
-            L.cnt[pos] = 0u;
-            L.keys[pos] = 0ull;
-        }
-        const float B = fmaxf(fabsf(L.ts[0]), fabsf(L.ts[pad_slot(nfin - 1)]));
-        int eB = 0;
-        (void)frexpf(B, &eB);
-        if (!(B < INFINITY)) eB = 128;
-        const double to_fix = ldexp(1.0, fixbits - eB), from_fix = ldexp(1.0, eB - fixbits);
-        wave_lds_sync();
-        int ctop = 0;
-        double stop = 0.0;
-        unsigned int rpk[4];
-        for (int tp = 0; tp < ntiles; tp += 2) {
-#pragma unroll
-            for (int h = 0; h < 2; ++h) {
-                const int tile = tp + h;
-                if (tile >= ntiles) break;
-                float x[HSPL];
-                int rho[HSPL];
-                load_tile(spu, tile * 64 * HSPL, S, lane, x);
-                search_tile(L.ts, x, rho, nfin);
-#pragma unroll
-                for (int j = 0; j < HSPL; ++j) {
-                    if (rho[j] == nfin) {
-                        ctop += 1;
-                        stop += (double)x[j];
-                    } else if (rho[j] != 0 && fabsf(x[j]) <= B) {
-                        atomicAdd(&L.cnt[rho[j]], 1u);
-                        atomicAdd(&L.keys[rho[j]], (unsigned long long)__double2ll_rn((double)x[j] * to_fix));
-                    }
-                }
-                if (tp == 0) {
-                    rpk[2 * h] = (unsigned)rho[0] | ((unsigned)rho[1] << 8) | ((unsigned)rho[2] << 16) | ((unsigned)rho[3] << 24);
-                    rpk[2 * h + 1] = (unsigned)rho[4] | ((unsigned)rho[5] << 8) | ((unsigned)rho[6] << 16) | ((unsigned)rho[7] << 24);
-                }
-            }
-        }
-#pragma unroll
-        for (int off = 32; off >= 1; off >>= 1) {
-            ctop += __shfl_xor(ctop, off, 64);
-            stop += __shfl_xor(stop, off, 64);
-        }
-        wave_lds_sync();
-        int csuf[4];
-        long long fsuf[4];
-        {
-            int crun = 0;
-            long long frun = 0;
-#pragma unroll
-            for (int q = 3; q >= 0; --q) {
-                const int b = 4 * lane + q + 1;
-                if (b < HK) {
-                    crun += (int)L.cnt[b];
-                    frun += (long long)L.keys[b];
-                }
-                csuf[q] = crun;
-                fsuf[q] = frun;
-            }
-            int cinc = crun;
-            long long finc = frun;
-#pragma unroll
-            for (int off = 1; off < 64; off <<= 1) {
-                const int co = __shfl_down(cinc, off, 64);
-                const long long fo = __shfl_down(finc, off, 64);
-                if (lane + off < 64) {
-                    cinc += co;
-                    finc += fo;
-                }
-            }
-            const int cex = cinc - crun;
-            const long long fex = finc - frun;
-#pragma unroll
-            for (int q = 0; q < 4; ++q) {
-                csuf[q] += cex;
-                fsuf[q] += fex;
-            }
-        }
-        float wown[4];
-#pragma unroll
-        for (int q = 0; q < 4; ++q) {
-            const int pos = 4 * lane + q;
-            float w = 0.f, d = 0.f;
-            if (pos < nfin) {
-                const int cn = csuf[q] + ctop;
-                const float c1 = -town[q];
-                double hs = (double)cn * (double)c1 + ((double)fsuf[q] * from_fix + stop);
-                hs = hs > 0.0 ? hs : 0.0;
-                const float M = c * (float)hs;
-                lsum += logf(1.0f + M);
-                w = c * __frcp_rn(1.0f + M);
-                d = -(w * (float)cn);
-            }
-            wown[q] = w;
-            if (oown[q] >= 0) delta[cb + oown[q]] = d;
-        }
-        {
-            const float l0 = wown[0], l1 = l0 + wown[1], l2 = l1 + wown[2], l3 = l2 + wown[3];
-            float inc = l3;
-#pragma unroll
-            for (int off = 1; off < 64; off <<= 1) {
-                const float o = __shfl_up(inc, off, 64);
-                if (lane >= off) inc += o;
-            }
-            const float ex = __shfl_up(inc, 1, 64);
-            const float base = (lane == 0) ? 0.f : ex;
-            L.pw[pad_slot(4 * lane)] = base;
-            L.pw[pad_slot(4 * lane + 1)] = base + l0;
-            L.pw[pad_slot(4 * lane + 2)] = base + l1;
-            L.pw[pad_slot(4 * lane + 3)] = base + l2;
-        }
-        wave_lds_sync();
-        for (int tp = 0; tp < ntiles; tp += 2) {
-#pragma unroll
-            for (int h = 0; h < 2; ++h) {
-                const int tile = tp + h;
-                if (tile >= ntiles) break;
-                int rho[HSPL];
-                if (ntiles <= 2) {
-#pragma unroll
-                    for (int j = 0; j < HSPL; ++j) rho[j] = (int)((rpk[2 * h + (j >> 2)] >> (8 * (j & 3))) & 0xffu);
-                } else {
-                    float x[HSPL];
-                    load_tile(spu, tile * 64 * HSPL, S, lane, x);
-                    search_tile(L.ts, x, rho, nfin);
-                }
-#pragma unroll
-                for (int j = 0; j < HSPL; ++j) {
-                    const int s = tile * 64 * HSPL + lane + 64 * j;
-                    if (s < S) {
-                        const float dv = L.pw[pad_slot(rho[j])];
-                        if (wrote) Du[s] += dv;
-                        else Du[s] = dv;
-                    }
-                }
-            }
-        }
-        wrote = true;
-        wave_lds_sync();
-    }
-    if (!wrote)
-        for (int s = lane; s < S; s += 64) Du[s] = 0.f;
-#pragma unroll
-    for (int off = 32; off >= 1; off >>= 1) lsum += __shfl_xor(lsum, off, 64);
-    if (lane == 0 && loss_part) loss_part[u] = lsum;
+    hinge_user(u, lane, lds_all[wave], rowptr, val, p, sp, S, fixbits, c, delta, D, loss_part);
 }
 
 }
@@ -297,9 +28,7 @@
                                        void* stream) {
     if (n_users == 0) return TMF_OK;
     TMF_REQUIRE(rowptr && sp && D && n_users > 0 && S > 0, "wmrb_hinge2: bad arguments");
-    int lg = 0;
-    while (((int64_t)1 << lg) < (int64_t)S) ++lg;
-    const int fixbits = 62 - lg;
+    const int fixbits = hinge_fixbits(S);
     const unsigned blocks = (unsigned)(((int64_t)n_users + HWAVES - 1) / HWAVES);
     hipLaunchKernelGGL(k_wmrb_hinge2, dim3(blocks), dim3(64 * HWAVES), 0, (hipStream_t)stream, rowptr, val, p, sp, (int)S, fixbits,
                        c, (int64_t)n_users, delta, D, loss_part, user_order);
diff --git a/teamoflow_amd/csrc/tmf_wmrb.hip b/teamoflow_amd/csrc/tmf_wmrb.hip
--- a/teamoflow_amd/csrc/tmf_wmrb.hip
+++ b/teamoflow_amd/csrc/tmf_wmrb.hip
@@ -4,6 +4,7 @@
 #include <type_traits>
 
 #include "tmf_common.h"
+#include "tmf_hinge.h"
 
 namespace tmf {
 
@@ -330,6 +331,10 @@
 #define TMF_STREAM_NT 1
 #endif
 constexpr bool kStreamNT = TMF_STREAM_NT;
+#ifndef TMF_GRADU_ZERO_BRANCH
+#define TMF_GRADU_ZERO_BRANCH 0
+#endif
+constexpr bool kGraduZeroBranch = TMF_GRADU_ZERO_BRANCH;
 constexpr int kSliceUsers = 16;
 constexpr int kLongRange = 48;
 
@@ -370,7 +375,12 @@
                 bool want = e < cnt;
                 d[t] = 0.f;
                 if (GRADU && want) { d[t] = wv[t]; want = d[t] != 0.f; }
-                load_raw<G, NV>(raw[t], V, want ? idv[t] : safe, g);
+                if constexpr (GRADU && kGraduZeroBranch && std::is_same<T, float>::value) {
+                    if (want) load_raw<G, NV>(raw[t], V, idv[t], g);
+                    else zero_raw<NV>(raw[t]);
+                } else {
+                    load_raw<G, NV>(raw[t], V, want ? idv[t] : safe, g);
+                }
             }
 #pragma unroll
             for (int t = 0; t < kUnrollW; ++t) {
@@ -458,19 +468,13 @@
 }
 
 template <int G, int NV, typename T, int WAVES>
-__global__ __launch_bounds__(64 * WAVES) void k_wmrb_scores3(SliceLists a, const T* __restrict__ U, const T* __restrict__ V,
-                                                           float* __restrict__ sp, float* __restrict__ p) {
-    extern __shared__ __attribute__((aligned(16))) char smem_raw[];
+__device__ __forceinline__ void scores_group(const SliceLists& a, int64_t sl, int64_t ubeg, int64_t uend, const T* __restrict__ U,
+                                             const T* __restrict__ V, float* __restrict__ sp, float* __restrict__ p, char* smem_raw) {
     constexpr int NG = 64 / G, NGB = NG * WAVES;
     const int tid = threadIdx.x, lane = tid & 63, wave = tid >> 6;
     const int g = lane & (G - 1), gid = wave * NG + lane / G;
     int* ids = slice_stage<G>(smem_raw, gid);
     float* dst = reinterpret_cast<float*>(ids + Stage<G>::tile);
-    int64_t sl, grp;
-    if (!slice_of_block(a, blockIdx.x, sl, grp)) return;
-    const int64_t ubeg = grp * a.upg;
-    const int64_t uend = (ubeg + a.upg < a.n_users) ? ubeg + a.upg : a.n_users;
-    V = window_base<G, NV, T>(V, a.item_base);
     if constexpr (G == 32 && sizeof(Raw<NV, T>) <= 16) {
         if (a.lean) {
             for (int64_t u = ubeg + gid; u < uend; u += NGB) {
@@ -509,9 +513,60 @@
 }
 
 template <int G, int NV, typename T, int WAVES>
+__global__ __launch_bounds__(64 * WAVES) void k_wmrb_scores3(SliceLists a, const T* __restrict__ U, const T* __restrict__ V,
+                                                           float* __restrict__ sp, float* __restrict__ p) {
+    extern __shared__ __attribute__((aligned(16))) char smem_raw[];
+    int64_t sl, grp;
+    if (!slice_of_block(a, blockIdx.x, sl, grp)) return;
+    const int64_t ubeg = grp * a.upg;
+    const int64_t uend = (ubeg + a.upg < a.n_users) ? ubeg + a.upg : a.n_users;
+    scores_group<G, NV, T, WAVES>(a, sl, ubeg, uend, U, window_base<G, NV, T>(V, a.item_base), sp, p, smem_raw);
+}
+
+constexpr int kTailWaves = 4;
+#ifndef TMF_TAIL_OCC
+#define TMF_TAIL_OCC __attribute__((amdgpu_waves_per_eu(4)))
+#endif
+template <int G, int NV, typename T>
+__global__ __launch_bounds__(64 * kTailWaves) TMF_TAIL_OCC void k_wmrb_hinge2_tail(SliceLists a, const T* __restrict__ U, const T* __restrict__ V,
+                                                                    float* sp, float* p, const float* __restrict__ val, int fixbits,
+                                                                    float c, float* delta, float* D, float* loss_part,
+                                                                    const int32_t* __restrict__ order) {
+    extern __shared__ __attribute__((aligned(16))) char smem_raw[];
+    const int64_t grp = order ? (int64_t)order[blockIdx.x] : (int64_t)blockIdx.x;
+    const int64_t ubeg = grp * a.upg;
+    const int64_t uend = (ubeg + a.upg < a.n_users) ? ubeg + a.upg : a.n_users;
+    const T* Vw = window_base<G, NV, T>(V, a.item_base);
+    for (int64_t sl = a.sl0; sl < a.sl0 + a.nsl; ++sl) scores_group<G, NV, T, kTailWaves>(a, sl, ubeg, uend, U, Vw, sp, p, smem_raw);
+    __builtin_amdgcn_fence(__ATOMIC_RELEASE, "agent");
+    __syncthreads();
+    __builtin_amdgcn_fence(__ATOMIC_ACQUIRE, "agent");
+    const int lane = threadIdx.x & 63;
+    const int wave = __builtin_amdgcn_readfirstlane(threadIdx.x >> 6);
+    HingeLds& L = reinterpret_cast<HingeLds*>(smem_raw)[wave];
+    for (int64_t u = ubeg + wave; u < uend; u += kTailWaves)
+        hinge_user(u, lane, L, a.rowptr, val, p, sp, a.S, fixbits, c, delta, D, loss_part);
+}
+
+template <typename T>
+struct GraduFin {
+    const T* U_old;
+    void* U_out;
+    int first;
+    int epi;
+    tmf_adam adam;
+};
+
+#ifndef TMF_FIN_AHEAD
+#define TMF_FIN_AHEAD 12
+#endif
+template <int NV>
+constexpr int kFinAhead = (TMF_FIN_AHEAD / NV > 1) ? TMF_FIN_AHEAD / NV : 1;
+
+template <int G, int NV, typename T, int WAVES, bool FIN = false>
 __global__ __launch_bounds__(64 * WAVES) void k_wmrb_gradu3(SliceLists a, const T* __restrict__ V, const float* __restrict__ D,
-                                                          const float* __restrict__ delta, float* __restrict__ part,
-                                                          int slice_first, int accumulate) {
+                                                          const float* __restrict__ delta, float* part,
+                                                          int slice_first, int accumulate, GraduFin<T> fin) {
     extern __shared__ __attribute__((aligned(16))) char smem_raw[];
     constexpr int NG = 64 / G, NGB = NG * WAVES;
     const int tid = threadIdx.x, lane = tid & 63, wave = tid >> 6;
@@ -519,7 +574,10 @@
     int* ids = slice_stage<G>(smem_raw, gid);
     float* dst = reinterpret_cast<float*>(ids + Stage<G>::tile);
     int64_t sl, grp, layer = 0;
-    if (slice_first < 0) {
+    if (FIN) {
+        sl = slice_first;
+        grp = blockIdx.x;
+    } else if (slice_first < 0) {
         if (!slice_of_block(a, blockIdx.x, sl, grp)) return;
     } else if (accumulate >= 3) {
         layer = blockIdx.x & 7;
@@ -537,12 +595,35 @@
     for (int64_t u = ubeg + gid; u < uend; u += NGB) {
         const int64_t o = u * (a.n_slices + 1) + sl;
         const int nb = a.off[o], ne = a.off[o + 1], pb = a.poff[o], pe = a.poff[o + 1];
+        constexpr int AHEAD = kFinAhead<NV>;
+        Frag<NV> ahead[FIN ? AHEAD : 1];
+        const int nprev = FIN ? (int)sl - fin.first : 0;
+        if constexpr (FIN) {
+#pragma unroll
+            for (int l = 0; l < AHEAD; ++l)
+                if (l < nprev) load_row_f32<G, NV, T, TMF_NT_FIN>(ahead[l], part, (fin.first + l) * a.n_users + u, g);
+        }
         Frag<NV> acc, none;
         zero<NV>(acc);
         const int64_t us = u * (int64_t)a.S, rb = a.rowptr[u];
         slice_list<G, NV, T, true>(ids, dst, a.R + us, nb, ne, V, none, acc, nullptr, D + us, g, a.item_base);
         slice_list<G, NV, T, true>(ids, dst, a.col + rb, pb, pe, V, none, acc, nullptr, delta + rb, g, a.item_base);
-        if (accumulate == 0) {
+        if constexpr (FIN) {
+            if (nprev > 0) {
+                Frag<NV> sum = ahead[0];
+#pragma unroll
+                for (int l = 1; l < AHEAD; ++l)
+                    if (l < nprev) add<NV>(sum, ahead[l]);
+                for (int l = AHEAD; l < nprev; ++l) {
+                    Frag<NV> y;
+                    load_row_f32<G, NV, T, TMF_NT_FIN>(y, part, (fin.first + l) * a.n_users + u, g);
+                    add<NV>(sum, y);
+                }
+                add<NV>(sum, acc);
+                acc = sum;
+            }
+            row_epilogue<G, NV, T>(acc, fin.U_old, fin.U_out, u, g, fin.epi, fin.adam);
+        } else if (accumulate == 0) {
             store_row_f32<G, NV, T>(acc, part, sl * a.n_users + u, g);
         } else {
             const int64_t prow = layer * a.n_users + u;
@@ -868,14 +949,40 @@
 }
 
 template <typename T>
+static int wmrb_hinge2_tail_impl(const tmf_slice_lists* lists, const void* U, const void* V, const float* val, float* sp, float* p,
+                                 float c, float* delta, float* D, float* loss_part, const int32_t* group_order, int n_components,
+                                 void* stream) {
+    SliceLists a;
+    const RowGeom geom = row_geom_of<T>(n_components);
+    if (int rc = check_lists(lists, a, "wmrb_hinge2_tail", geom.G, kTailWaves, (size_t)geom.ld * sizeof(T))) return rc;
+    if (a.n_users == 0) return TMF_OK;
+    if (int rc = check_ids_debug(lists, (hipStream_t)stream)) return rc;
+    TMF_REQUIRE(U && V && sp && D && (lists->col == nullptr || (p && val && delta)), "wmrb_hinge2_tail: null pointer");
+    TMF_REQUIRE(a.sl0 + a.nsl == a.n_slices, "wmrb_hinge2_tail: the slices [%d, +%d) are not the last of %d", a.sl0, a.nsl, a.n_slices);
+    TMF_REQUIRE(a.upg == kSliceUsers, "wmrb_hinge2_tail: %d users per workgroup (rows of %d lanes, TMF_SLICE_USERS) - this launch takes 16",
+                a.upg, geom.G);
+    TMF_REQUIRE_LAUNCH(a.n_groups, 64 * kTailWaves, "wmrb_hinge2_tail");
+    const size_t stage = slice_lds(geom, kTailWaves), hinge = kTailWaves * sizeof(HingeLds);
+    const size_t lds = stage > hinge ? stage : hinge;
+    const int fixbits = hinge_fixbits(a.S);
+#define CALL(G_, NV_)                                                                                                  \
+    hipLaunchKernelGGL((k_wmrb_hinge2_tail<G_, NV_, T>), dim3((unsigned)a.n_groups), dim3(64 * kTailWaves), lds,        \
+                       (hipStream_t)stream, a, (const T*)U, (const T*)V, sp, p, val, fixbits, c, delta, D, loss_part, group_order)
+    TMF_DISPATCH(T, geom, CALL);
+#undef CALL
+    return check_launch("tmf_wmrb_hinge2_tail");
+}
+
+template <typename T>
 static int wmrb_gradu3_impl(const tmf_slice_lists* lists, const float* D, const float* delta, const void* V, float* part,
-                            int per_slice_launches, int n_components, void* stream) {
+                            int per_slice_launches, int n_components, void* stream, const GraduFin<T>* fin = nullptr) {
     SliceLists a;
     const RowGeom geom = row_geom_of<T>(n_components);
     const int waves = slice_waves(lists, geom.G);
     if (int rc = check_lists(lists, a, "wmrb_gradu3", geom.G, waves)) return rc;
     if (a.n_users == 0) return TMF_OK;
-    TMF_REQUIRE(D && V && part && (delta || lists->col == nullptr), "wmrb_gradu3: null pointer");
+    TMF_REQUIRE(D && V && (delta || lists->col == nullptr), "wmrb_gradu3: null pointer");
+    TMF_REQUIRE(part || (fin && a.nsl == 1), "wmrb_gradu3: null pointer");
     const size_t lds = slice_lds(geom, waves);
     TMF_REQUIRE(per_slice_launches >= 0 && per_slice_launches <= 3, "wmrb_gradu3: per_slice_launches=%d", per_slice_launches);
     if (per_slice_launches == 3) {
@@ -884,7 +991,7 @@
             const int accumulate = (sl == a.sl0) ? 3 : 4;
 #define CALLW(G_, NV_, W_)                                                                                                       \
     hipLaunchKernelGGL((k_wmrb_gradu3<G_, NV_, T, W_>), dim3((unsigned)(a.n_groups * 8)), dim3(64 * W_), lds, (hipStream_t)stream, a, \
-                       (const T*)V, D, delta, part, sl, accumulate)
+                       (const T*)V, D, delta, part, sl, accumulate, GraduFin<T>{})
 #define CALL4(G_, NV_) CALLW(G_, NV_, 4)
 #define CALL8(G_, NV_) CALLW(G_, NV_, 8)
             if (waves == 8) { TMF_DISPATCH(T, geom, CALL8); } else { TMF_DISPATCH(T, geom, CALL4); }
@@ -900,7 +1007,7 @@
             const int accumulate = (sl == a.sl0 && per_slice_launches == 1) ? 1 : 2;
 #define CALLW(G_, NV_, W_)                                                                                                   \
     hipLaunchKernelGGL((k_wmrb_gradu3<G_, NV_, T, W_>), dim3((unsigned)a.n_groups), dim3(64 * W_), lds, (hipStream_t)stream, a, \
-                       (const T*)V, D, delta, part, sl, accumulate)
+                       (const T*)V, D, delta, part, sl, accumulate, GraduFin<T>{})
 #define CALL4(G_, NV_) CALLW(G_, NV_, 4)
 #define CALL8(G_, NV_) CALLW(G_, NV_, 8)
             if (waves == 8) { TMF_DISPATCH(T, geom, CALL8); } else { TMF_DISPATCH(T, geom, CALL4); }
@@ -914,13 +1021,13 @@
     const int64_t per_unit = a.n_groups * unit * 64 * waves;
     const int max_units = (int)((((int64_t)1 << 32) - 1) / per_unit);
     TMF_REQUIRE(max_units >= 1, "wmrb_gradu3: %lld user groups exceed one launch", (long long)a.n_groups);
-    const int first = a.sl0, last = a.sl0 + a.nsl;
+    const int first = a.sl0, last = a.sl0 + a.nsl - (fin ? 1 : 0);
     for (int s0 = first; s0 < last; s0 += max_units * unit) {
         a.sl0 = s0;
         a.nsl = (last - s0 < max_units * unit) ? last - s0 : max_units * unit;
 #define CALLW(G_, NV_, W_)                                                                                   \
     hipLaunchKernelGGL((k_wmrb_gradu3<G_, NV_, T, W_>), dim3(slice_grid(a)), dim3(64 * W_), lds, \
-                       (hipStream_t)stream, a, (const T*)V, D, delta, part, -1, 0)
+                       (hipStream_t)stream, a, (const T*)V, D, delta, part, -1, 0, GraduFin<T>{})
 #define CALL4(G_, NV_) CALLW(G_, NV_, 4)
 #define CALL8(G_, NV_) CALLW(G_, NV_, 8)
         if (waves == 8) { TMF_DISPATCH(T, geom, CALL8); } else { TMF_DISPATCH(T, geom, CALL4); }
@@ -928,7 +1035,31 @@
 #undef CALL8
 #undef CALLW
     }
+    if (fin) {
+        TMF_REQUIRE_LAUNCH(a.n_groups, 64 * waves, "wmrb_gradu3 (last slice)");
+        a.sl0 = first;
+        a.nsl = last + 1 - first;
+#define CALLW(G_, NV_, W_)                                                                                               \
+    hipLaunchKernelGGL((k_wmrb_gradu3<G_, NV_, T, W_, true>), dim3((unsigned)a.n_groups), dim3(64 * W_), lds, (hipStream_t)stream, a, \
+                       (const T*)V, D, delta, part, last, 0, *fin)
+#define CALL4(G_, NV_) CALLW(G_, NV_, 4)
+#define CALL8(G_, NV_) CALLW(G_, NV_, 8)
+        if (waves == 8) { TMF_DISPATCH(T, geom, CALL8); } else { TMF_DISPATCH(T, geom, CALL4); }
+#undef CALL4
+#undef CALL8
+#undef CALLW
+    }
     return check_launch("tmf_wmrb_gradu3");
+}
+
+template <typename T>
+static int wmrb_gradu3_finish_impl(const tmf_slice_lists* lists, const float* D, const float* delta, const void* V, float* part,
+                                   const void* U_old, void* U_out, int n_components, int epi, tmf_adam adam, void* stream) {
+    TMF_REQUIRE(U_out && (epi == TMF_EPI_GRAD || U_old), "wmrb_gradu3_finish: null pointer");
+    TMF_REQUIRE(epi == TMF_EPI_ADAM || epi == TMF_EPI_GRAD, "wmrb_gradu3_finish: bad epilogue %d", epi);
+    TMF_REQUIRE(lists != nullptr, "wmrb_gradu3_finish: lists is null");
+    const GraduFin<T> fin{(const T*)U_old, U_out, (int)lists->slice_begin, epi, adam};
+    return wmrb_gradu3_impl<T>(lists, D, delta, V, part, 0, n_components, stream, &fin);
 }
 
 static size_t gradu4_workspace(int64_t n_users, int n_slices, int64_t users_per_launch) {
@@ -1413,10 +1544,21 @@
                                           float* sp, float* p, int n_components, void* stream) {                          \
         return wmrb_scores6_impl<T_>(ids, outs, chunk_ptr, n_groups, n_slices, n_users, n_items, U, V, sp, p, n_components, stream); \
     }                                                                                                                     \
+    extern "C" int tmf_wmrb_hinge2_tail_##SFX(const tmf_slice_lists* lists, const void* U, const void* V, const float* val, \
+                                              float* sp, float* p, float c, float* delta, float* D, float* loss_part,     \
+                                              const int32_t* group_order, int n_components, void* stream) {               \
+        return wmrb_hinge2_tail_impl<T_>(lists, U, V, val, sp, p, c, delta, D, loss_part, group_order, n_components,      \
+                                         stream);                                                                         \
+    }                                                                                                                     \
     extern "C" int tmf_wmrb_gradu3_##SFX(const tmf_slice_lists* lists, const float* D, const float* delta,                \
                                          const void* V, float* part, int per_slice_launches, int n_components,            \
                                          void* stream) {                                                                  \
         return wmrb_gradu3_impl<T_>(lists, D, delta, V, part, per_slice_launches, n_components, stream);                  \
+    }                                                                                                                     \
+    extern "C" int tmf_wmrb_gradu3_finish_##SFX(const tmf_slice_lists* lists, const float* D, const float* delta,         \
+                                                const void* V, float* part, const void* U_old, void* U_out,               \
+                                                int n_components, int epi, tmf_adam adam, void* stream) {                 \
+        return wmrb_gradu3_finish_impl<T_>(lists, D, delta, V, part, U_old, U_out, n_components, epi, adam, stream);      \
     }                                                                                                                     \
     extern "C" int tmf_wmrb_gradu4_##SFX(const tmf_slice_lists* lists, const float* D, const float* delta, const void* V,  \
                                          const void* U_old, void* U_out, int n_components, int epi, tmf_adam adam,       \
@@ -1432,6 +1574,10 @@
 TMF_SLICED_ENTRY_POINTS(f32, float)
 TMF_SLICED_ENTRY_POINTS(bf16, __bf16)
 
+extern "C" int tmf_wmrb_hinge2_tail_supported(int n_components, int bf16) {
+    const tmf::RowGeom geom = bf16 ? tmf::row_geom_bf16(n_components) : tmf::row_geom(n_components);
+    return geom.ld != 0 && geom.G >= 16 && getenv("TMF_SLICE_USERS") == nullptr;
+}
 extern "C" int tmf_wmrb_scores6_users_per_group(void) { return tmf::kS6Users; }
 extern "C" int tmf_wmrb_scores6_supported(int n_components, int bf16, int64_t n_items) { return s6_supported(n_components, bf16, n_items); }
 extern "C" int tmf_wmrb_scores5_users_per_workgroup(void) { return tmf::kS5Users; }
```

After: 999.1 million. -12.8%, worse.
